# LikeLy-Journey/SegmenTron

Measured on AMD Instinct MI355X. Metric: images/sec fwd+bwd DeepLabv3+_xception65 @1025x2049, higher is better.
Workload: dtype bf16; 1 GPU; DeepLabv3+_xception65 train step (fwd + CE loss + bwd + SGD) @1025x2049, batch 2/GPU (BASELINE.json configs[2]); global_batch=2, bn=BN, parallelism=dp1, full_size=True

## Files before the change

### include/segmentron_hip.h

```cpp
#ifndef SEGMENTRON_HIP_H
#define SEGMENTRON_HIP_H
#ifdef __cplusplus
extern "C" {
#endif

const char* seg_last_error(void);
int seg_version(void);

int seg_conv_gemm_fwd(int dtype, const void* x, long ldx, int N, int Hi, int Wi, int C,
                      const void* w, int O, int KH, int KW, int stride, int pad, int dil,
                      int pro_mode, const float* pro_scale, const float* pro_shift,
                      const float* bias, void* y, long ldy, int Ho, int Wo, int out_H, int out_W,
                      int out_s, float* stat_partial, const void* ep_x, long ldep,
                      const float* ep_c0, const float* ep_c1, int tconv, void* stream);
int seg_conv_gemm_tiles_m(int N, int Ho, int Wo);

int seg_conv_gemm_wgrad(int dtype, const void* x, long ldx, int N, int Hi, int Wi, int C,
                        const void* dy, long lddy, int Ho, int Wo, int O, int KH, int KW,
                        int stride, int pad, int dil, int pro_mode, const float* pro_scale,
                        const float* pro_shift, float* partial, int splits, void* stream);
int seg_conv_gemm_stat_rows(int dtype, int N, int Ho, int Wo, int C, int O, int KH, int KW,
                            int stride, int pad, int dil, int tconv, int has_bias, int pro_mode);
int seg_conv_gemm_wgrad_splits(int dtype, int N, int Ho, int Wo, int C, int O, int KH, int KW,
                               int stride, int pad, int dil, int pro_mode);

int seg_dwconv3x3(int dtype, int mode, const void* x, long ldx, int N, int Hi, int Wi, int C,
                  const float* w9c, int w_layout, int stride, int dil, int pro_mode,
                  const float* pro_scale, const float* pro_shift, void* y, long ldy, int Ho, int Wo,
                  float* stat_partial, int grid_y, void* stream);
int seg_dwconv_grid_y(int dtype, int C, int N, int Ho, int Wo, int stride, int dil, int kind);
int seg_dwconv3x3_wgrad_finalize(const float* partial, int R, int C, float* dw_c9, void* stream);
int seg_dwconv3x3_wgrad(int dtype, const void* x, long ldx, int N, int Hi, int Wi, int C,
                        const void* dy, long lddy, int Ho, int Wo, int stride, int dil,
                        int pro_mode, const float* pro_scale, const float* pro_shift,
                        float* partial, int grid_y, void* stream);

int seg_dwconv3x3_bwd_fused(int dtype, const void* dy, long lddy, const void* x, long ldx, int N,
                            int H, int W, int C, const float* w9c, int w_layout, int dil,
                            int pro_mode, const float* pro_scale, const float* pro_shift, void* g,
                            long ldg, float* partial_w, float* partial_bn, int grid_y,
                            void* stream);
int seg_dwconv3x3_bwd_fused_add_ok(int dil);
int seg_dwconv3x3_bwd_fused_add(int dtype, const void* dy, long lddy, const void* x, long ldx, int N,
                                int H, int W, int C, const float* w9c, int w_layout, int pro_mode,
                                const float* pro_scale, const float* pro_shift, const void* res,
                                long ldr, void* g, long ldg, float* partial_w, float* partial_bn,
                                int grid_y, void* stream);

int seg_colsum(const float* in, long R, int L, double* out_d, float* out_f, double* ws,
               void* stream);
int seg_colsum_count(const float* in, long R, int L, double* out_d, double count, double* ws,
                     void* stream);
int seg_bn_finalize(const double* sums, double count, const double* count_dev,
                    const float* gamma, const float* beta, float eps, float momentum, float* running_mean, float* running_var,
                    float* mean, float* invstd, float* scale, float* shift, int C,
                    const float* mean_offset, void* stream);
int seg_bn_finalize_p(const float* partial, long R, double count, const float* gamma,
                      const float* beta, float eps, float momentum, float* running_mean,
                      float* running_var, float* mean, float* invstd, float* scale, float* shift,
                      int C, const float* mean_offset, double* ws, void* stream);
int seg_bn_finalize_small(int dtype, const void* y, long ldy, long M, int C, const float* gamma,
                          const float* beta, float eps, float momentum, float* running_mean,
                          float* running_var, float* mean, float* invstd, float* scale,
                          float* shift, const float* mean_offset, void* stream);
int seg_bn_moments_small(int dtype, const void* y, long ldy, long M, int C, double* moments,
                         void* stream);
int seg_bn_finalize_small_sync(void* p2p, int dtype, const void* y, long ldy, long M, int C,
                               const float* gamma, const float* beta, float eps, float momentum,
                               float* running_mean, float* running_var, float* mean, float* invstd,
                               float* scale, float* shift, const float* mean_offset,
                               double* count_out, void* stream);
int seg_sum_n(int dtype, int n, const void* const* xs, const long* lds, void* y, long ldy, long M,
              int C, void* stream);
int seg_bn_eval_affine(const float* gamma, const float* beta, const float* rm, const float* rv,
                       float eps, float* scale, float* shift, int C, void* stream);
int seg_bn_eval_affine_multi(int n, const float* const* gamma, const float* const* beta,
                             const float* const* rm, const float* const* rv, const float* eps,
                             float* const* out, const int* C, void* stream);
int seg_bn_apply(int dtype, const void* x, long ldx, int mode_x, const float* sx, const float* tx,
                 const void* r, long ldr, int mode_r, const float* sr, const float* tr,
                 const float* chan_mul, long rows_per_n, const void* elem_mul, long ldm,
                 int post_relu, void* y, long ldy, long M, int C, void* stream);
int seg_bn_bwd_grid_y(int dtype, int C, long M);
int seg_bn_bwd_reduce(int dtype, const void* g, long ldg, const void* x, long ldx, int mode,
                      const float* scale, const float* shift, const float* chan_mul,
                      long rows_per_n, const void* elem_mul, long ldm, long M, int C,
                      float* partial, int grid_y, void* stream);
int seg_bn_bwd_small(int dtype, const void* g, long ldg, const void* x, long ldx, void* dx,
                     long lddx, long M, int C, int mode, const float* scale, const float* shift,
                     const float* mean, const float* invstd, const float* gamma,
                     const float* chan_mul, long rows_per_n, const void* elem_mul, long ldm,
                     double count, int training, float* dgamma, float* dbeta, void* stream);
int seg_bn_bwd_finalize(const double* sums, double count, const double* count_dev,
                        const float* mean, const float* invstd, const float* gamma, float* dgamma, float* dbeta, float* c0, float* c1,
                        int C, void* stream);
int seg_bn_bwd_finalize_s(const double* sums, double count, const double* count_dev,
                          const float* mean, const float* invstd, const float* gamma, float* dgamma,
                          float* dbeta, float* c0, float* c1, int C, double grad_scale, void* stream);
int seg_bn_bwd_finalize_p(const float* partial, long R, double count, const float* mean,
                          const float* invstd, const float* gamma, float* dgamma, float* dbeta,
                          float* c0, float* c1, int C, double* ws, void* stream);
int seg_dw_bwd_finalize(const float* partial_bn, int Rb, double count, const float* mean,
                        const float* invstd, const float* gamma, float* dgamma, float* dbeta,
                        float* c0, float* c1, const float* partial_w, int Rw, float* dw_c9, int C,
                        void* stream);
int seg_bn_bwd_apply(int dtype, const void* g, long ldg, const void* x, long ldx, int mode,
                     const float* scale, const float* shift, const float* c0, const float* c1,
                     const float* chan_mul, long rows_per_n, const void* elem_mul, long ldm,
                     void* dx, long lddx, long M, int C, void* stream);

int seg_gn_chunks(long HW);
int seg_gn_moments(int dtype, const void* u, long ldu, const void* v, long ldv, int N, long HW,
                   int C, float* partial, void* stream);
int seg_gn_fwd_finalize(const float* partial, int N, long HW, int C, int G, const float* gamma,
                        const float* beta, double eps, float* mean_rstd, float* coef,
                        void* stream);
int seg_gn_bwd_finalize(const float* partial, int N, long HW, int C, int G,
                        const float* mean_rstd, const float* gamma, float* coef, float* contrib,
                        void* stream);
int seg_gn_affine(int dtype, const void* u, long ldu, const void* v, long ldv, const float* coef,
                  void* out, long ldo, int N, long HW, int C, void* stream);

int seg_fold_weights(int dtype, const float* W, const float* scale, const float* shift, void* Wp,
                     void* WpT, float* bprime, int O, int C, void* stream);
int seg_fold_bwd_rows(int O);
int seg_fold_bwd_reduce(const float* W, const float* dWp, int splits, const float* scale,
                        const float* shift, const float* db, float* dW, float* dsdt, int O, int C,
                        void* stream);
int seg_fold_bwd_finalize(const float* dsdt, int rows, double count, const double* count_dev,
                          const float* mean, const float* invstd, const float* gamma, const float* scale, float* dgamma, float* dbeta,
                          float* c0, float* c1, int C, void* stream);
int seg_fold_bwd_finalize_s(const float* dsdt, int rows, double count, const double* count_dev,
                            const float* mean, const float* invstd, const float* gamma,
                            const float* scale, float* dgamma, float* dbeta, float* c0, float* c1,
                            int C, double grad_scale, void* stream);

int seg_maxpool_fwd(int dtype, const void* x, long ldx, int N, int Hi, int Wi, int C, int k,
                    int stride, int pad, int pro_mode, const float* pro_scale,
                    const float* pro_shift, void* y, long ldy, int Ho, int Wo, void* idx,
                    void* stream);
int seg_maxpool_bwd(int dtype, void* gx, long ldgx, int N, int Hi, int Wi, int C, int k, int stride,
                    int pad, const void* gy, long ldgy, int Ho, int Wo, const void* idx,
                    void* stream);
int seg_adaptive_avgpool_chunks(int H, int W, int o);
int seg_adaptive_avgpool_partial(int dtype, const void* x, long ldx, int N, int H, int W, int C,
                                 int o, float* partial, int chunks, void* stream);
int seg_adaptive_avgpool_bwd(int dtype, void* gx, long ldgx, int N, int H, int W, int C, int o,
                             const void* gy, long ldgy, void* stream);

int seg_bilinear_fwd(int dtype, const void* x, long ldx, int N, int Hi, int Wi, int C,
                     int pro_mode, const float* pro_scale, const float* pro_shift,
                     const float* chan_mul, void* y, long ldy, int Ho, int Wo, int align_corners,
                     void* stream);
int seg_bilinear_bwd(int dtype, void* gx, long ldgx, int N, int Hi, int Wi, int C, const void* gy,
                     long ldgy, int Ho, int Wo, int align_corners, void* stream);
int seg_nearest_add(int dtype, const void* x, long ldx, int mode_x, const float* sx,
                    const float* tx, const void* r, long ldr, int mode_r, const float* sr,
                    const float* tr, int shift, int post_relu, void* y, long ldy, int N, int H,
                    int W, int C, void* stream);
int seg_nearest_sum_bwd(int dtype, const void* g, long ldg, int N, int H, int W, int C, int shift,
                        void* gr, long ldgr, void* stream);
int seg_upsample_to_nchw(int dtype, const void* x, long ldx, int N, int Hi, int Wi, int C,
                         float* out, int Ho, int Wo, int align_corners, void* stream);
int seg_upsample_to_nchw_bwd(int dtype, void* gx, long ldgx, int N, int Hi, int Wi, int C,
                             const float* gy, int Ho, int Wo, int align_corners, void* stream);
int seg_nchw_to_nhwc_pad(int dtype, const float* x, int N, int Cin, int H, int W, void* y,
                         void* stream);

int seg_upsample_ce_blocks(int N, int H, int W);
int seg_upsample_ce_fwd(int dtype, const void* lo, long ld, int N, int Hi, int Wi, int C,
                        const long* target, int H, int W, long ignore_index, int align_corners,
                        double* ws, float* loss_out, void* stream);
int seg_upsample_ce_bwd(int dtype, const void* lo, long ld, int N, int Hi, int Wi, int C,
                        const long* target, int H, int W, long ignore_index, int align_corners,
                        const float* loss_out, const float* grad_out, void* dlo, long lddlo,
                        void* stream);

int seg_dwconv3x3_s2_grid_y(int C, int N, int H, int W);
int seg_dwconv3x3_s2_bwd_fused(int dtype, const void* dy, long lddy, const void* x, long ldx, int N,
                               int H, int W, int C, const float* w_c9, int pro_mode,
                               const float* pro_scale, const float* pro_shift, void* g, long ldg,
                               float* partial_w, float* partial_bn, int grid_y, void* stream);

int seg_sgd_multi_tensor(int ntensors, const void* const* params, const void* const* grads,
                         const void* const* bufs, const long* numel, const int* group,
                         const float* lr_dev, const float* wd_dev, float momentum, int first,
                         void* stream);
int seg_pack_multi(int dtype, int njobs, const void* const* srcs, const void* const* dsts,
                   const int* O, const int* C, const int* transpose, void* stream);

int seg_metric_update_nchw(const float* logits, int N, int C, int H, int W, const long* target,
                           int nclass, long* counters, void* stream);
int seg_metric_update_upsample(int dtype, const void* lo, long ld, int N, int Hi, int Wi, int C,
                               const long* target, int H, int W, int align_corners, int nclass,
                               long* counters, void* stream);

int seg_cca_attention(int dtype, const void* q, long ldq, const void* k, long ldk, int N, int H,
                      int W, int C, float* att, void* stream);
int seg_cca_attention_bwd(int dtype, const void* dout, long lddo, const void* v, long ldv, int N,
                          int H, int W, int C, const float* att, const float* scale, float* de,
                          void* stream);
int seg_cca_map(int dtype, const float* wt, const void* b, long ldb, int N, int H, int W, int C,
                int transposed, const float* gamma, const void* res, long ldres, void* out,
                long ldo, void* raw, long ldraw, void* stream);

int seg_row_softmax(const void* e, int dt_in, long lde, void* a, int dt_out, long lda, long R,
                    int L, int Lp, float sign, void* stream);
int seg_row_softmax_bwd(const void* a, int dt_a, long lda, const void* g, int dt_g, long ldg,
                        void* de, int dt_out, long ldde, long R, int L, int Lp, float sign,
                        void* stream);
int seg_p2p_create(int rank, int world, long slot_bytes, void** handle_out);
int seg_p2p_ipc_handle(void* handle, void* out64);
int seg_p2p_connect(void* handle, const void* handles);
int seg_p2p_all_reduce_f64(void* handle, void* buf, int n, void* stream);
int seg_p2p_all_reduce_f32(void* handle, void* buf, int n, void* stream);
int seg_p2p_status(void* handle);
int seg_p2p_set_timeout(void* handle, double seconds);
int seg_p2p_destroy(void* handle);
int seg_bn_finalize_p_sync(void* p2p, const float* partial, long R, double local_count,
                           const float* gamma, const float* beta, float eps, float momentum,
                           float* running_mean, float* running_var, float* mean, float* invstd,
                           float* scale, float* shift, int C, const float* mean_offset,
                           double* count_out, double* ws, void* stream);
int seg_bn_bwd_finalize_p_sync(void* p2p, const float* partial, long R, const double* count_dev,
                               const float* mean, const float* invstd, const float* gamma,
                               float* dgamma, float* dbeta, float* c0, float* c1, int C,
                               double grad_scale, double* ws, void* stream);
int seg_dw_bwd_finalize_sync(void* p2p, const float* partial_bn, int Rb, const double* count_dev,
                             const float* mean, const float* invstd, const float* gamma,
                             float* dgamma, float* dbeta, float* c0, float* c1,
                             const float* partial_w, int Rw, float* dw_c9, int C,
                             double grad_scale, void* stream);
int seg_fold_bwd_finalize_sync(void* p2p, const float* dsdt, int rows, const double* count_dev,
                               const float* mean, const float* invstd, const float* gamma,
                               const float* scale, float* dgamma, float* dbeta, float* c0,
                               float* c1, int C, double grad_scale, void* stream);

#ifdef __cplusplus
}
#endif
#endif
```

### segmentron_amd/csrc/conv_gemm_args.h

```cpp
#pragma once
#include <hip/hip_runtime.h>

namespace seg {

struct ConvGemmArgs {
  const void* x;
  const void* w;
  void* y;
  const float* pro_scale;
  const float* pro_shift;
  const float* bias;
  float* stat_partial;
  const void* ep_x;
  const float* ep_c0;
  const float* ep_c1;
  long ldx, ldy, ldep;
  int N, Hi, Wi, C, Ho, Wo, O;
  int KH, KW, stride, pad, dil;
  int pro_mode;
  int tconv;
  int M, K;
  int out_H, out_W, out_s;
  int tiles_m, tiles_n;
};

int px256_tiles_m(long M);
int launch_conv_gemm_px256(int dtype, ConvGemmArgs a, hipStream_t stream);
bool conv_gemm_glds_usable(int dtype, const ConvGemmArgs& a);
int launch_conv_gemm_glds(ConvGemmArgs a, hipStream_t stream);
bool conv_gemm_glds_kxk_usable(int dtype, const ConvGemmArgs& a);
int launch_conv_gemm_glds_kxk(ConvGemmArgs a, hipStream_t stream);

int launch_conv_gemm_glds4(const ConvGemmArgs& a, int rows, hipStream_t stream);

int glds_rows_per_tile(long M, int O, bool kxk);
int glds_tiles_m(long M, int O, bool kxk);

bool conv3x3_direct_usable(int dtype, const ConvGemmArgs& a);
int conv3x3_direct_blocks(int N, int H, int W, int C = 32);
int launch_conv3x3_direct(const ConvGemmArgs& a, hipStream_t stream);

}
```

### segmentron_amd/csrc/conv_gemm_glds.hip

```cpp
#include "conv_gemm.h"
#include "conv_gemm_args.h"
#include "gemm_glds.h"

namespace seg {


template <bool EP, bool STATS, bool KXK = false, int IMS = 4>
__global__ __launch_bounds__(GL_THREADS, 2) void conv_gemm_glds_kernel(const ConvGemmArgs a) {
  typedef bf16_t T;
  constexpr int VEC = 8;
  extern __shared__ __attribute__((aligned(16))) unsigned char smem_raw[];
  lds_byte_t* lds = (lds_byte_t*)smem_raw;

  const int tid = threadIdx.x, lane = tid & 63;
  const int wave = __builtin_amdgcn_readfirstlane(tid >> 6);
  const int wm = wave >> 2, wn = wave & 3;
  const int L = xcd_remap(blockIdx.x, a.tiles_m * a.tiles_n);
  const int tile_m = L / a.tiles_n, tile_n = L - tile_m * a.tiles_n;
  const int m0 = tile_m * (64 * IMS), n0 = tile_n * GL_BN;

  GemmOperand A, B;
  A.base = reinterpret_cast<const unsigned char*>(a.x);
  A.ld_bytes = a.ldx * 2;
  A.rows = a.M;
  B.base = reinterpret_cast<const unsigned char*>(a.w);
  B.ld_bytes = (long)a.K * 2;
  B.rows = a.O;

  f32x16 acc[2][IMS];

  if (KXK) {
    const GlConvA cg = {a.M, a.Hi, a.Wi, a.Ho, a.Wo, a.KW, a.pad, a.dil, a.C / 32};
    gl_mainloop_ring<true, IMS>(A, B, a.K, m0, n0, lds, acc, &cg);
  } else {
    gl_mainloop_ring<false, IMS>(A, B, a.K, m0, n0, lds, acc);
  }

  typedef typename std::conditional<EP, float, T>::type PT;
  constexpr int EP_STRIDE = 64 * (int)sizeof(PT) + 16;
  constexpr int VPR = 64 / VEC;
  unsigned char* ep = smem_raw + wave * 32 * EP_STRIDE;
  T* __restrict__ Y = reinterpret_cast<T*>(a.y);
  const int r32 = lane & 31, hh = lane >> 5;
  const int v = lane & (VPR - 1);
  const int o = n0 + wn * 64 + v * VEC;
  float ssum[VEC], ssq[VEC];
#pragma unroll
  for (int k = 0; k < VEC; ++k) ssum[k] = ssq[k] = 0.f;
  float c0v[VEC], c1v[VEC];
  const bool epc = EP && o < a.O;
  if (epc) {
    load_params<VEC>(a.ep_c0, o, c0v);
    load_params<VEC>(a.ep_c1, o, c1v);
  }
  constexpr int NQ_ALL = (32 * VPR) / 64;
  uint4 xr_all[EP ? IMS : 1][EP ? NQ_ALL : 1];
  if (EP) {
#pragma unroll
    for (int im = 0; im < IMS; ++im)
#pragma unroll
      for (int q = 0; q < NQ_ALL; ++q) {
        const int r = (q * 64 + lane) / VPR;
        const int p = m0 + wm * 32 * IMS + im * 32 + r;
        const long pc = p < a.M ? p : a.M - 1;
        xr_all[im][q] = ldg16(reinterpret_cast<const T*>(a.ep_x) + pc * a.ldep + (epc ? o : 0));
      }
  }
#pragma unroll
  for (int im = 0; im < IMS; ++im) {
#pragma unroll
    for (int jn = 0; jn < 2; ++jn) {
#pragma unroll
      for (int g = 0; g < 4; ++g) {
        const int ch = jn * 32 + 8 * g + 4 * hh;
        float f[4];
#pragma unroll
        for (int k = 0; k < 4; ++k) f[k] = acc[jn][im][4 * g + k];
        HVec<PT>::store(reinterpret_cast<PT*>(ep + r32 * EP_STRIDE) + ch, f);
      }
    }
    __builtin_amdgcn_fence(__ATOMIC_RELEASE, "wavefront");
    __builtin_amdgcn_wave_barrier();
    constexpr int NQ = (32 * VPR) / 64;
    uint4 val[NQ], xr[NQ], vhi[NQ];
#pragma unroll
    for (int q = 0; q < NQ; ++q) {
      const int r = (q * 64 + lane) / VPR;
      if (EP) {
        val[q] = *reinterpret_cast<const uint4*>(ep + r * EP_STRIDE + v * 32);
        vhi[q] = *reinterpret_cast<const uint4*>(ep + r * EP_STRIDE + v * 32 + 16);
      } else {
        val[q] = *reinterpret_cast<const uint4*>(ep + r * EP_STRIDE + v * 16);
      }
      if (EP) xr[q] = xr_all[im][q];
    }
#pragma unroll
    for (int q = 0; q < NQ; ++q) {
      const int r = (q * 64 + lane) / VPR;
      const int p = m0 + wm * 32 * IMS + im * 32 + r;
      if (EP) {
        float f[VEC], xv[VEC];
        Vec<float>::unpack(val[q], f);
        Vec<float>::unpack(vhi[q], f + 4);
        Vec<T>::unpack(xr[q], xv);
        if (epc) {
#pragma unroll
          for (int k = 0; k < VEC; ++k) f[k] = f[k] - c0v[k] - c1v[k] * xv[k];
        }
        val[q] = Vec<T>::pack(f);
      }
      if (STATS && (!EP || p < a.M)) {
        float f[VEC];
        Vec<T>::unpack(val[q], f);
#pragma unroll
        for (int k = 0; k < VEC; ++k) {
          ssum[k] += f[k];
          ssq[k] = fmaf(f[k], f[k], ssq[k]);
        }
      }
      if (p < a.M && o < a.O) stg16(Y + (long)p * a.ldy + o, val[q]);
    }
    __builtin_amdgcn_fence(__ATOMIC_RELEASE, "wavefront");
    __builtin_amdgcn_wave_barrier();
  }
  if (STATS) {
#pragma unroll
    for (int k = 0; k < VEC; ++k) {
#pragma unroll
      for (int m = VPR; m < 64; m <<= 1) {
        ssum[k] += __shfl_xor(ssum[k], m, 64);
        ssq[k] += __shfl_xor(ssq[k], m, 64);
      }
    }
    __syncthreads();
    float* red = reinterpret_cast<float*>(smem_raw);
    if (lane < VPR) {
#pragma unroll
      for (int k = 0; k < VEC; ++k) {
        red[(wm * 2 + 0) * 256 + wn * 64 + v * VEC + k] = ssum[k];
        red[(wm * 2 + 1) * 256 + wn * 64 + v * VEC + k] = ssq[k];
      }
    }
    __syncthreads();
    if (tid < 256) {
      const int oc = n0 + tid;
      if (oc < a.O) {
        float* dst = a.stat_partial + (long)tile_m * 2 * a.O;
        dst[oc] = red[0 * 256 + tid] + red[2 * 256 + tid];
        dst[a.O + oc] = red[1 * 256 + tid] + red[3 * 256 + tid];
      }
    }
  }
}

bool conv_gemm_glds_usable(int dtype, const ConvGemmArgs& a) {
  return dtype == DT_BF16 && a.pro_mode == PRO_NONE && a.bias == nullptr && a.KH == 1 && a.KW == 1 && a.stride == 1 &&
         a.pad == 0 && a.tconv == 0 && a.out_s == 1 && (a.K % 8) == 0 && (a.ldx % 8) == 0 && (a.O % 8) == 0 &&
         (a.ldy % 8) == 0;
}

constexpr int GLDS_FIXED_ROWS = 96;

constexpr long GLDS_W4_MAX_TILES = 512;

static int glds_pick_rows(long M, int O, bool with224) {
  const long tn = (O + GL_BN - 1) / GL_BN;
  int best = 256;
  long best_cost = -1;
  for (int bm = 256; bm >= 192; bm -= 32) {
    const long tiles = ((M + bm - 1) / bm) * tn;
    if (bm == 224 && (!with224 || tiles > GLDS_W4_MAX_TILES)) continue;
    const long cost = ((tiles + 255) / 256) * (bm + GLDS_FIXED_ROWS);
    if (best_cost < 0 || cost < best_cost) {
      best_cost = cost;
      best = bm;
    }
  }
  return best;
}

int glds_rows_per_tile(long M, int O, bool kxk) { return glds_pick_rows(M, O, !kxk); }

int glds_tiles_m(long M, int O, bool kxk) {
  const int bm = glds_rows_per_tile(M, O, kxk);
  return (int)((M + bm - 1) / bm);
}

template <bool EP, bool STATS, bool KXK, int IMS>
static int launch_glds_inst(const ConvGemmArgs& a, hipStream_t stream) {
  static const int once = [] {
    return (int)hipFuncSetAttribute(
        reinterpret_cast<const void*>(&conv_gemm_glds_kernel<EP, STATS, KXK, IMS>),
        hipFuncAttributeMaxDynamicSharedMemorySize, GL_LDS_BYTES);
  }();
  if (once != 0) {
    set_error("conv_gemm_glds: cannot reserve %d bytes of LDS", GL_LDS_BYTES);
    return 2;
  }
  const dim3 grid(a.tiles_m * a.tiles_n), block(GL_THREADS);
  hipLaunchKernelGGL((conv_gemm_glds_kernel<EP, STATS, KXK, IMS>), grid, block, GL_LDS_BYTES,
                     stream, a);
  return check_launch(KXK ? "conv_gemm_fwd (glds KxK)" : "conv_gemm_fwd (glds)");
}

template <bool EP, bool STATS, bool KXK>
static int launch_glds_rows(ConvGemmArgs a, hipStream_t stream) {
  const int bm = glds_pick_rows(a.M, a.O, !KXK && !(EP && !STATS));
  a.tiles_m = (a.M + bm - 1) / bm;
  a.tiles_n = (a.O + GL_BN - 1) / GL_BN;
  if constexpr (!KXK) {
    if (bm == 224) return launch_conv_gemm_glds4(a, bm, stream);
  }
  if (bm == 256) return launch_glds_inst<EP, STATS, KXK, 4>(a, stream);
  if (bm == 192) return launch_glds_inst<EP, STATS, KXK, 3>(a, stream);
  set_error("conv_gemm_glds: no %d-row tile on the eight-wave kernel", bm);
  return 2;
}

int launch_conv_gemm_glds(ConvGemmArgs a, hipStream_t stream) {
  if (a.ep_x != nullptr && a.stat_partial != nullptr)
    return launch_glds_rows<true, true, false>(a, stream);
  if (a.ep_x != nullptr) return launch_glds_rows<true, false, false>(a, stream);
  if (a.stat_partial != nullptr) return launch_glds_rows<false, true, false>(a, stream);
  return launch_glds_rows<false, false, false>(a, stream);
}

bool conv_gemm_glds_kxk_usable(int dtype, const ConvGemmArgs& a) {
  return dtype == DT_BF16 && a.pro_mode == PRO_NONE && a.bias == nullptr && a.ep_x == nullptr &&
         a.KH * a.KW > 1 && a.stride == 1 && a.tconv == 0 && a.out_s == 1 && (a.C % 32) == 0 &&
         (a.ldx % 8) == 0 && (a.O % 8) == 0 && (a.ldy % 8) == 0 &&
         (long)a.N * a.Hi * a.Wi < (1L << 31);
}

int launch_conv_gemm_glds_kxk(ConvGemmArgs a, hipStream_t stream) {
  if (a.stat_partial != nullptr) return launch_glds_rows<false, true, true>(a, stream);
  return launch_glds_rows<false, false, true>(a, stream);
}

}
```

### segmentron_amd/csrc/conv_gemm_wgrad_args.h

```cpp
#pragma once
#include <hip/hip_runtime.h>

namespace seg {

struct WgradArgs {
  const void* x;
  const void* dy;
  float* partial;
  const float* pro_scale;
  const float* pro_shift;
  long ldx, lddy;
  int N, Hi, Wi, C, Ho, Wo, O;
  int KH, KW, stride, pad, dil;
  int pro_mode;
  int M, K;
  int tiles_o, tiles_k, splits;
  int chunk;
};

bool conv_wgrad_glds_usable(int dtype, const WgradArgs& a);
int conv_wgrad_glds_splits(long M, int O, int K);
int launch_conv_wgrad_glds(WgradArgs a, hipStream_t stream);

bool conv3x3_wgrad_direct_usable(int dtype, int C, int O, int KH, int KW, int stride, int pad,
                                 int dil, long M, long ldx, long lddy);
int conv3x3_direct_blocks(int N, int H, int W, int C = 32);
int launch_conv3x3_wgrad_direct(const void* x, long ldx, const void* dy, long lddy, int N, int H,
                                int W, int O, int pro_mode, const float* pro_scale,
                                const float* pro_shift, float* partial, hipStream_t stream);

}
```

### segmentron_amd/csrc/conv_gemm_wgrad_glds.hip

```cpp
#include "conv_gemm.h"
#include "conv_gemm_wgrad_args.h"
#include "gemm_glds.h"

namespace seg {

constexpr int WG_BM = 128, WG_BN = 128, WG_BK = 64;
constexpr int WG_THREADS = 512;
constexpr int WG_SUB = 16 * 1024, WG_SLOT = 32 * 1024, WG_LDS = 4 * WG_SLOT;

typedef unsigned long long u64_t;

__device__ __forceinline__ u64_t tr_read(unsigned addr) {
  u64_t r;
  asm volatile("ds_read_b64_tr_b16 %0, %1" : "=v"(r) : "v"(addr) : "memory");
  return r;
}
template <int OFF>
__device__ __forceinline__ u64_t tr_read_off(unsigned addr) {
  u64_t r;
  asm volatile("ds_read_b64_tr_b16 %0, %1 offset:%2" : "=v"(r) : "v"(addr), "n"(OFF) : "memory");
  return r;
}

struct WgFrags { u64_t a[2], b[2][2]; };

__device__ __forceinline__ bf16x8 wg_join(u64_t lo, u64_t hi) {
  typedef u64_t u64x2 __attribute__((ext_vector_type(2)));
  u64x2 v = {lo, hi};
  return __builtin_bit_cast(bf16x8, v);
}

template <bool KXK>
__global__ __launch_bounds__(WG_THREADS, 2) void conv_wgrad_glds_kernel(const WgradArgs a) {
  extern __shared__ __attribute__((aligned(16))) unsigned char smem_raw[];
  lds_byte_t* lds = (lds_byte_t*)smem_raw;
  const int tid = threadIdx.x, lane = tid & 63;
  const int wave = __builtin_amdgcn_readfirstlane(tid >> 6);
  const int wo = wave >> 1, wc = wave & 1;
  const int tiles = a.tiles_o * a.tiles_k;
  const int L = xcd_remap(blockIdx.x, tiles * a.splits);
  const int tile = L % tiles, split = L / tiles;
  const int o0 = (tile / a.tiles_k) * WG_BM, c0 = (tile % a.tiles_k) * WG_BN;
  const int p0 = split * a.chunk;
  const int p1 = min(a.M, p0 + a.chunk);
  const int nslot = (p1 - p0 + WG_BK - 1) / WG_BK;

  const unsigned char* zero = reinterpret_cast<const unsigned char*>(g_gl_zero);
  const int rr = lane >> 4;
  const int c16 = ((lane & 15) - 4 * rr) & 15;
  const bool ch_dy = o0 + c16 * 8 < a.O, ch_x = c0 + c16 * 8 < (KXK ? a.K : a.C);
  const unsigned char* src[4];
  int prow[2];
  int kdh = 0, kdw = 0, kc0 = c0, pn[2] = {0, 0}, ph[2] = {0, 0}, pw[2] = {0, 0};
  if (KXK) {
    const int tap = c0 / a.C;
    kc0 = c0 - tap * a.C;
    const int kh = tap / a.KW;
    kdh = kh * a.dil - a.pad;
    kdw = (tap - kh * a.KW) * a.dil - a.pad;
  }
#pragma unroll
  for (int j = 0; j < 2; ++j) {
    prow[j] = p0 + (wave * 2 + j) * 4 + rr;
    src[j] = reinterpret_cast<const unsigned char*>(a.dy) +
             ((long)prow[j] * a.lddy + o0 + c16 * 8) * 2;
    src[2 + j] = reinterpret_cast<const unsigned char*>(a.x) +
                 ((long)prow[j] * a.ldx + c0 + c16 * 8) * 2;
    if (KXK) {
      pw[j] = prow[j] % a.Wo;
      const int t = prow[j] / a.Wo;
      ph[j] = t % a.Ho;
      pn[j] = t / a.Ho;
    }
  }
  const long inc_dy = (long)WG_BK * a.lddy * 2, inc_x = (long)WG_BK * a.ldx * 2;
  auto issue = [&](int slot) {
    lds_byte_t* base = lds + (slot & 3) * WG_SLOT + (wave * 2) * 1024;
#pragma unroll
    for (int j = 0; j < 2; ++j) {
      const bool rok = prow[j] + slot * WG_BK < p1;
      const unsigned char* pd = (rok && ch_dy) ? src[j] : zero;
      const unsigned char* px = (rok && ch_x) ? src[2 + j] : zero;
      if (KXK) {
        const int hi = ph[j] + kdh, wi = pw[j] + kdw;
        const bool ok = rok && ch_x && hi >= 0 && hi < a.Hi && wi >= 0 && wi < a.Wi;
        px = ok ? reinterpret_cast<const unsigned char*>(a.x) +
                      ((((long)pn[j] * a.Hi + hi) * a.Wi + wi) * a.ldx + kc0 + c16 * 8) * 2
                : zero;
        pw[j] += WG_BK;
        if (pw[j] >= a.Wo) {
          pw[j] -= a.Wo;
          if (++ph[j] == a.Ho) { ph[j] = 0; ++pn[j]; }
        }
      }
      src[j] += inc_dy;
      src[2 + j] += inc_x;
      __builtin_amdgcn_global_load_lds((glb_byte_t*)pd, base + j * 1024, 16, 0, 0);
      __builtin_amdgcn_global_load_lds((glb_byte_t*)px, base + j * 1024 + WG_SUB, 16, 0, 0);
    }
  };
  issue(0); issue(1); issue(2); issue(3);

  const int g = lane >> 4, i = lane & 15;
  auto lane_base = [&](int cb) {
    const int q = cb * 4 + (g & 1) * 2 + ((i & 3) >> 1);
    const int cpos = (q + 4 * (i >> 2)) & 15;
    return (g >> 1) * 2048 + (i >> 2) * 256 + cpos * 16 + (i & 1) * 8;
  };
  const unsigned lds0 = (unsigned)(unsigned long)lds;
  const unsigned addr_a = lds0 + lane_base(wo);
  const unsigned addr_b0 = lds0 + WG_SUB + lane_base(wc * 2);
  const unsigned addr_b1 = lds0 + WG_SUB + lane_base(wc * 2 + 1);
  auto read = [&](WgFrags& f, int slot, auto step) {
    constexpr int S = decltype(step)::value;
    const unsigned off = (slot & 3) * WG_SLOT;
    f.a[0] = tr_read_off<S * 4096>(addr_a + off);
    f.a[1] = tr_read_off<S * 4096 + 1024>(addr_a + off);
    f.b[0][0] = tr_read_off<S * 4096>(addr_b0 + off);
    f.b[0][1] = tr_read_off<S * 4096 + 1024>(addr_b0 + off);
    f.b[1][0] = tr_read_off<S * 4096>(addr_b1 + off);
    f.b[1][1] = tr_read_off<S * 4096 + 1024>(addr_b1 + off);
  };
  typedef std::integral_constant<int, 0> S0;
  typedef std::integral_constant<int, 1> S1;
  typedef std::integral_constant<int, 2> S2;
  typedef std::integral_constant<int, 3> S3;
  f32x16 acc[2];
#pragma unroll
  for (int e = 0; e < 16; ++e) acc[0][e] = acc[1][e] = 0.f;
  auto mma = [&](const WgFrags& f) {
    const bf16x8 fa = wg_join(f.a[0], f.a[1]);
    acc[0] = __builtin_amdgcn_mfma_f32_32x32x16_bf16(fa, wg_join(f.b[0][0], f.b[0][1]), acc[0], 0,
                                                     0, 0);
    acc[1] = __builtin_amdgcn_mfma_f32_32x32x16_bf16(fa, wg_join(f.b[1][0], f.b[1][1]), acc[1], 0,
                                                     0, 0);
  };
#define WG_WAIT_FRAGS(f, cnt)                                                                  \
  asm volatile("s_waitcnt " cnt                                                               \
               : "+v"(f.a[0]), "+v"(f.a[1]), "+v"(f.b[0][0]), "+v"(f.b[0][1]), "+v"(f.b[1][0]), \
                 "+v"(f.b[1][1])                                                               \
               :                                                                               \
               : "memory")
  WgFrags f0, f1;
  GL_WAIT_VM(12);
  __builtin_amdgcn_s_barrier();
  read(f0, 0, S0{});
  for (int j = 0; j < nslot; ++j) {
    read(f1, j, S1{});
    WG_WAIT_FRAGS(f0, "lgkmcnt(6)");
    mma(f0);
    read(f0, j, S2{});
    WG_WAIT_FRAGS(f1, "lgkmcnt(6)");
    mma(f1);
    read(f1, j, S3{});
    WG_WAIT_FRAGS(f0, "lgkmcnt(6)");
    mma(f0);
    WG_WAIT_FRAGS(f1, "vmcnt(8) lgkmcnt(0)");
    __builtin_amdgcn_s_barrier();
    issue(j + 4);
    read(f0, j + 1, S0{});
    mma(f1);
  }
  asm volatile("s_waitcnt vmcnt(0) lgkmcnt(0)" ::: "memory");
#undef WG_WAIT_FRAGS

  float* __restrict__ P = a.partial + (long)split * a.O * a.K;
  const int r32 = lane & 31, hh = lane >> 5;
#pragma unroll
  for (int jb = 0; jb < 2; ++jb) {
    const int c = c0 + (wc * 2 + jb) * 32 + r32;
#pragma unroll
    for (int e = 0; e < 16; ++e) {
      const int o = o0 + wo * 32 + (e & 3) + 8 * (e >> 2) + 4 * hh;
      if (o < a.O && c < a.K) P[(long)o * a.K + c] = acc[jb][e];
    }
  }
}

bool conv_wgrad_glds_usable(int dtype, const WgradArgs& a) {
  const bool common = dtype == DT_BF16 && a.pro_mode == PRO_NONE && a.stride == 1 &&
                      (a.O % 8) == 0 && (a.ldx % 8) == 0 && (a.lddy % 8) == 0 && a.M >= 2048;
  if (!common) return false;
  if (a.KH == 1 && a.KW == 1)
    return a.pad == 0 && (a.C % 8) == 0 && ((long)a.O * a.C >= 128 * 128 || a.M >= 32768);
  return (a.C % 128) == 0 && a.Wo >= WG_BK && a.O >= 128 &&
         (long)a.N * a.Hi * a.Wi < (1L << 31);
}

int conv_wgrad_glds_splits(long M, int O, int K) {
  const int tiles = ((O + WG_BM - 1) / WG_BM) * ((K + WG_BN - 1) / WG_BN);
  long want = (256 + tiles / 2) / tiles;
  if (want * tiles > 282) want = 256 / tiles;
  const long maxs = (M + 8 * WG_BK - 1) / (8 * WG_BK);
  if (want > maxs) want = maxs;
  if (want < 1) want = 1;
  return (int)want;
}

int launch_conv_wgrad_glds(WgradArgs a, hipStream_t stream) {
  a.tiles_o = (a.O + WG_BM - 1) / WG_BM;
  a.tiles_k = (a.K + WG_BN - 1) / WG_BN;
  const int slots = (a.M + WG_BK - 1) / WG_BK;
  a.chunk = ((slots + a.splits - 1) / a.splits) * WG_BK;
  static const int once = [] {
    int rc = (int)hipFuncSetAttribute(reinterpret_cast<const void*>(&conv_wgrad_glds_kernel<false>),
                                      hipFuncAttributeMaxDynamicSharedMemorySize, WG_LDS);
    rc |= (int)hipFuncSetAttribute(reinterpret_cast<const void*>(&conv_wgrad_glds_kernel<true>),
                                   hipFuncAttributeMaxDynamicSharedMemorySize, WG_LDS);
    return rc;
  }();
  if (once != 0) {
    set_error("conv_wgrad_glds: cannot reserve %d bytes of LDS", WG_LDS);
    return 2;
  }
  const dim3 grid(a.tiles_o * a.tiles_k * a.splits), block(WG_THREADS);
  if (a.KH * a.KW > 1)
    hipLaunchKernelGGL(conv_wgrad_glds_kernel<true>, grid, block, WG_LDS, stream, a);
  else
    hipLaunchKernelGGL(conv_wgrad_glds_kernel<false>, grid, block, WG_LDS, stream, a);
  return check_launch("conv_gemm_wgrad (glds)");
}

}
```

### segmentron_amd/csrc/dwconv.hip

```cpp
#include "common.h"
#include "dwconv_tiled.h"
#include "dwconv_slide.h"
#include <cstdlib>
#include <type_traits>

namespace seg {

constexpr bool g_dw_row = true;

constexpr int DW_TW = 4;
constexpr int DW_THREADS = 256;
enum { MODE_FWD = 0, MODE_DGRAD = 1 };

struct DwArgs {
  const void* x;
  const float* w;
  void* y;
  const float* pro_scale;
  const float* pro_shift;
  float* stat_partial;
  long ldx, ldy;
  int N, Hi, Wi, C;
  int Ho, Wo;
  int stride, pad, dil;
// ... 395 lines not shown
    const int b = 1 << l;
    const double u = (double)CV / (double)(((CV + b - 1) / b) * b);
    if (u > bu + 1e-9) { bu = u; best = l; }
  }
  return best;
}

}

extern "C" int seg_dwconv_grid_y(int dtype, int C, int N, int Ho, int Wo, int stride, int dil,
                                 int kind) {
  using namespace seg;
  const int tiled_stride = kind == 0 ? stride : 1;
  if ((kind == 0 || kind == 1) && dw_slide_supported(stride, dil, C))
    return dw_slide_rows(C, N, Ho, Wo);
  if ((kind == 0 || stride == 1) && dw_tiled_supported(tiled_stride, dil))
    return dw_tiled_grid_y(dtype, C, N, Ho, Wo, kind);
  if (kind == 0 && stride == 2 && dil == 1)
    return dw_tiled_s2_grid_y(dtype, C, N, Ho, Wo);
  if (g_dw_row && (kind == 0 || kind == 1) && dw_row_supported(stride, dil) && C % 4 == 0)
    return dw_row_grid_y(dtype, C, N, Ho, Wo, dil);
  const int vec = dtype == DT_BF16 ? 8 : 4;
  const int CV = C / vec;
  const int l = pick_cvb_log2(CV);
  const int spb = DW_THREADS >> l;
  const long strips = (long)N * Ho * ((Wo + DW_TW - 1) / DW_TW);
  const int gx = (CV + (1 << l) - 1) >> l;
  long gy = (strips + spb - 1) / spb;
  long cap = 1536 / gx;
  if (cap < 1) cap = 1;
  if (gy > cap) gy = cap;
  return (int)gy;
}
extern "C" int seg_dwconv3x3(int dtype, int mode, const void* x, long ldx, int N, int Hi, int Wi,
                             int C, const float* w9c, int w_layout, int stride, int dil, int pro_mode,
                             const float* pro_scale, const float* pro_shift, void* y, long ldy,
                             int Ho, int Wo, float* stat_partial, int grid_y, void* stream) {
  using namespace seg;
  const int vec = dtype == DT_BF16 ? 8 : 4;
  SEG_REQUIRE(dtype == DT_F32 || dtype == DT_BF16, "dwconv3x3: bad dtype %d", dtype);
  SEG_REQUIRE(C % vec == 0 && ldx % vec == 0 && ldy % vec == 0,
              "dwconv3x3: C/ldx/ldy must be multiples of %d", vec);
  SEG_REQUIRE(((pro_mode & PRO_AFFINE) == 0) || (pro_scale && pro_shift),
              "dwconv3x3: affine prologue without scale/shift");
  SEG_REQUIRE(mode == MODE_FWD || stat_partial == nullptr, "dwconv3x3: stats only in forward");
  SEG_REQUIRE(grid_y >= 1, "dwconv3x3: grid_y must be >= 1");
  if (mode == MODE_FWD && dw_slide_supported(stride, dil, C)) {
    SEG_REQUIRE(Ho == Hi && Wo == Wi, "dwconv3x3: stride 1 keeps the size");
    return launch_dw_slide_fwd(dtype, x, ldx, N, Hi, Wi, C, w9c, w_layout, pro_mode, pro_scale,
                               pro_shift, y, ldy, stat_partial, grid_y, (hipStream_t)stream);
  }
  if (mode == MODE_FWD && dw_tiled_supported(stride, dil)) {
    SEG_REQUIRE(Ho == Hi && Wo == Wi, "dwconv3x3: stride 1 keeps the size");
    return launch_dw_tiled(dtype, x, ldx, N, Hi, Wi, C, w9c, w_layout, dil, pro_mode, pro_scale,
                           pro_shift, y, ldy, stat_partial, grid_y, (hipStream_t)stream);
  }
  if (mode == MODE_FWD && stride == 2 && dil == 1) {
    SEG_REQUIRE(Ho == (Hi + 1) / 2 && Wo == (Wi + 1) / 2, "dwconv3x3: stride-2 output size");
    SEG_REQUIRE((long)N * Hi * Wi < (1L << 31), "dwconv3x3: tensor exceeds 32-bit pixel offsets");
    return launch_dw_tiled_s2(dtype, x, ldx, N, Hi, Wi, C, w9c, w_layout, pro_mode, pro_scale,
                              pro_shift, y, ldy, stat_partial, grid_y, (hipStream_t)stream);
  }
  SEG_REQUIRE(w_layout == 0, "dwconv3x3: the strip kernels take tap-major [9][C] weights");
  if (g_dw_row && mode == MODE_FWD && dw_row_supported(stride, dil) && C % 4 == 0) {
    SEG_REQUIRE(Ho == Hi && Wo == Wi, "dwconv3x3: stride 1 keeps the size");
    return launch_dw_row_fwd(dtype, x, ldx, N, Hi, Wi, C, w9c, dil, pro_mode, pro_scale, pro_shift,
                             y, ldy, stat_partial, grid_y, (hipStream_t)stream);
  }
  DwArgs a;
  a.x = x; a.w = w9c; a.y = y; a.pro_scale = pro_scale; a.pro_shift = pro_shift;
  a.stat_partial = stat_partial; a.ldx = ldx; a.ldy = ldy;
  a.N = N; a.Hi = Hi; a.Wi = Wi; a.C = C; a.Ho = Ho; a.Wo = Wo;
  a.stride = stride; a.pad = dil; a.dil = dil; a.pro_mode = pro_mode;
  const int kvec = vec;
  a.CV = C / kvec; a.cvb_log2 = pick_cvb_log2(a.CV);
  a.strips = (long)N * Ho * ((Wo + DW_TW - 1) / DW_TW);
  const int gx = (a.CV + (1 << a.cvb_log2) - 1) >> a.cvb_log2;
  SEG_REQUIRE(grid_y >= 1, "dwconv3x3: grid_y must be >= 1");
  const dim3 grid(gx, grid_y);
  const size_t lds = stat_partial ? (size_t)DW_THREADS * 2 * kvec * sizeof(float) : 0;
  hipStream_t st = (hipStream_t)stream;
  SEG_REQUIRE(a.strips < (1L << 31), "dwconv3x3: too many strips");
  SEG_REQUIRE((long)N * Hi * Wi * ldx < (1L << 31), "dwconv3x3: tensor exceeds 32-bit offsets");
#define SEG_DW_LAUNCH(TT, MM) \
  hipLaunchKernelGGL((dwconv_kernel<TT, MM>), grid, dim3(DW_THREADS), lds, st, a)
  if (dtype == DT_BF16) {
    if (mode == MODE_FWD) SEG_DW_LAUNCH(bf16_t, MODE_FWD); else SEG_DW_LAUNCH(bf16_t, MODE_DGRAD);
  } else {
    if (mode == MODE_FWD) SEG_DW_LAUNCH(float, MODE_FWD); else SEG_DW_LAUNCH(float, MODE_DGRAD);
  }
#undef SEG_DW_LAUNCH
  return check_launch("dwconv3x3");
}

extern "C" int seg_dwconv3x3_wgrad(int dtype, const void* x, long ldx, int N, int Hi, int Wi,
                                   int C, const void* dy, long lddy, int Ho, int Wo, int stride,
                                   int dil, int pro_mode, const float* pro_scale,
                                   const float* pro_shift, float* partial, int grid_y,
                                   void* stream) {
  using namespace seg;
  const int vec = dtype == DT_BF16 ? 8 : 4;
  SEG_REQUIRE(dtype == DT_F32 || dtype == DT_BF16, "dwconv3x3_wgrad: bad dtype %d", dtype);
  SEG_REQUIRE(C % vec == 0 && ldx % vec == 0 && lddy % vec == 0,
              "dwconv3x3_wgrad: C/ldx/lddy must be multiples of %d", vec);
  SEG_REQUIRE(grid_y >= 1, "dwconv3x3_wgrad: grid_y must be >= 1");
  if (dw_tiled_supported(stride, dil)) {
    SEG_REQUIRE(Ho == Hi && Wo == Wi, "dwconv3x3_wgrad: stride 1 keeps the size");
    return launch_dw_wgrad_tiled(dtype, x, ldx, N, Hi, Wi, C, dy, lddy, dil, pro_mode, pro_scale,
                                 pro_shift, partial, grid_y, (hipStream_t)stream);
  }
  DwWgradArgs a;
  a.x = x; a.dy = dy; a.partial = partial; a.pro_scale = pro_scale; a.pro_shift = pro_shift;
  a.ldx = ldx; a.lddy = lddy; a.N = N; a.Hi = Hi; a.Wi = Wi; a.C = C; a.Ho = Ho; a.Wo = Wo;
  a.stride = stride; a.pad = dil; a.dil = dil; a.pro_mode = pro_mode;
  a.CV = C / vec; a.cvb_log2 = pick_cvb_log2(a.CV);
  a.strips = (long)N * Ho * ((Wo + DW_TW - 1) / DW_TW);
  const int gx = (a.CV + (1 << a.cvb_log2) - 1) >> a.cvb_log2;
  SEG_REQUIRE(grid_y >= 1, "dwconv3x3_wgrad: grid_y must be >= 1");
  const dim3 grid(gx, grid_y);
  const size_t lds = (size_t)DW_THREADS * 3 * vec * sizeof(float);
  hipStream_t st = (hipStream_t)stream;
  SEG_REQUIRE(a.strips < (1L << 31), "dwconv3x3_wgrad: too many strips");
  if (dtype == DT_BF16)
    hipLaunchKernelGGL((dwconv_wgrad_kernel<bf16_t>), grid, dim3(DW_THREADS), lds, st, a);
  else
    hipLaunchKernelGGL((dwconv_wgrad_kernel<float>), grid, dim3(DW_THREADS), lds, st, a);
  return check_launch("dwconv3x3_wgrad");
}

extern "C" int seg_dwconv3x3_bwd_fused_add_ok(int dil) { return dil == 1 ? 1 : 0; }

extern "C" int seg_dwconv3x3_bwd_fused_add(int dtype, const void* dy, long lddy, const void* x,
                                           long ldx, int N, int H, int W, int C, const float* w9c,
                                           int w_layout, int pro_mode, const float* pro_scale,
                                           const float* pro_shift, const void* res, long ldr,
                                           void* g, long ldg, float* partial_w, float* partial_bn,
                                           int grid_y, void* stream) {
  using namespace seg;
  SEG_REQUIRE(dtype == DT_F32 || dtype == DT_BF16, "dwconv3x3_bwd_fused_add: bad dtype %d", dtype);
  const int tvec = dtype == DT_BF16 ? 8 : 4;
  SEG_REQUIRE(C % tvec == 0 && ldx % tvec == 0 && lddy % tvec == 0 && ldg % tvec == 0 &&
                  ldr % 4 == 0 && res != nullptr,
              "dwconv3x3_bwd_fused_add: C/ld must be multiples of %d, res non-null", tvec);
  SEG_REQUIRE(((pro_mode & PRO_AFFINE) == 0) || (pro_scale && pro_shift),
              "dwconv3x3_bwd_fused_add: affine prologue without scale/shift");
  SEG_REQUIRE(grid_y >= 1 && partial_w != nullptr, "dwconv3x3_bwd_fused_add: bad grid/partials");
  if (dw_slide_supported(1, 1, C))
    return launch_dw_slide_bwd(dtype, dy, lddy, x, ldx, N, H, W, C, w9c, w_layout, pro_mode,
                               pro_scale, pro_shift, g, ldg, partial_w, partial_bn, grid_y,
                               (hipStream_t)stream, res, ldr);
  return launch_dw_bwd_tiled(dtype, dy, lddy, x, ldx, N, H, W, C, w9c, w_layout, 1, pro_mode,
                             pro_scale, pro_shift, g, ldg, partial_w, partial_bn, grid_y,
                             (hipStream_t)stream, res, ldr);
}

extern "C" int seg_dwconv3x3_bwd_fused(int dtype, const void* dy, long lddy, const void* x,
                                       long ldx, int N, int H, int W, int C, const float* w9c,
                                       int w_layout, int dil, int pro_mode, const float* pro_scale,
                                       const float* pro_shift, void* g, long ldg,
                                       float* partial_w, float* partial_bn, int grid_y,
                                       void* stream) {
  using namespace seg;
  const int vec = 4;
  SEG_REQUIRE(dtype == DT_F32 || dtype == DT_BF16, "dwconv3x3_bwd_fused: bad dtype %d", dtype);
  SEG_REQUIRE(C % vec == 0 && ldx % vec == 0 && lddy % vec == 0 && ldg % vec == 0,
              "dwconv3x3_bwd_fused: C/ld must be multiples of %d", vec);
  SEG_REQUIRE(((pro_mode & PRO_AFFINE) == 0) || (pro_scale && pro_shift),
              "dwconv3x3_bwd_fused: affine prologue without scale/shift");
  SEG_REQUIRE(grid_y >= 1 && partial_w != nullptr, "dwconv3x3_bwd_fused: bad grid/partials");
  if (dw_slide_supported(1, dil, C))
    return launch_dw_slide_bwd(dtype, dy, lddy, x, ldx, N, H, W, C, w9c, w_layout, pro_mode,
                               pro_scale, pro_shift, g, ldg, partial_w, partial_bn, grid_y,
                               (hipStream_t)stream);
  if (dw_tiled_supported(1, dil)) {
    const int tvec = dtype == DT_BF16 ? 8 : 4;
    SEG_REQUIRE(C % tvec == 0 && ldx % tvec == 0 && lddy % tvec == 0 && ldg % tvec == 0,
                "dwconv3x3_bwd_fused: C/ld must be multiples of %d", tvec);
    return launch_dw_bwd_tiled(dtype, dy, lddy, x, ldx, N, H, W, C, w9c, w_layout, dil, pro_mode,
                               pro_scale, pro_shift, g, ldg, partial_w, partial_bn, grid_y,
                               (hipStream_t)stream);
  }
  SEG_REQUIRE(w_layout == 0, "dwconv3x3_bwd_fused: the strip kernel takes tap-major weights");
  if (g_dw_row && dw_row_supported(1, dil))
    return launch_dw_row_bwd(dtype, dy, lddy, x, ldx, N, H, W, C, w9c, dil, pro_mode, pro_scale,
                             pro_shift, g, ldg, partial_w, partial_bn, grid_y, (hipStream_t)stream);
  DwBwdArgs a;
  a.dy = dy; a.x = x; a.g = g; a.w = w9c; a.pro_scale = pro_scale; a.pro_shift = pro_shift;
  a.partial_w = partial_w; a.partial_bn = partial_bn;
  a.lddy = lddy; a.ldx = ldx; a.ldg = ldg; a.N = N; a.H = H; a.W = W; a.C = C; a.dil = dil;
  a.pro_mode = pro_mode; a.CV = C / vec; a.cvb_log2 = pick_cvb_log2(a.CV);
  a.strips = (long)N * H * ((W + DW_TW - 1) / DW_TW);
  SEG_REQUIRE(a.strips < (1L << 31), "dwconv3x3_bwd_fused: too many strips");
  SEG_REQUIRE((long)N * H * W * lddy < (1L << 31), "dwconv3x3_bwd_fused: 32-bit offsets");
  const int gx = (a.CV + (1 << a.cvb_log2) - 1) >> a.cvb_log2;
  const dim3 grid(gx, grid_y);
  const size_t lds = (size_t)DW_THREADS * 3 * vec * sizeof(float);
  hipStream_t st = (hipStream_t)stream;
  if (dtype == DT_BF16)
    hipLaunchKernelGGL((dwconv_bwd_fused_kernel<bf16_t>), grid, dim3(DW_THREADS), lds, st, a);
  else
    hipLaunchKernelGGL((dwconv_bwd_fused_kernel<float>), grid, dim3(DW_THREADS), lds, st, a);
  return check_launch("dwconv3x3_bwd_fused");
}

extern "C" int seg_dwconv3x3_wgrad_finalize(const float* partial, int R, int C, float* dw_c9,
                                            void* stream) {
  using namespace seg;
  SEG_REQUIRE(R >= 1 && C >= 1, "dwconv3x3_wgrad_finalize: bad R/C");
  return launch_dw_wgrad_finalize(partial, R, C, dw_c9, (hipStream_t)stream);
}
```

### segmentron_amd/csrc/dwconv_slide.h

```cpp
#pragma once
#include <hip/hip_runtime.h>

namespace seg {
bool dw_slide_supported(int stride, int dil, int C);
int dw_slide_rows(int C, int N, int H, int W);
int launch_dw_slide_fwd(int dtype, const void* x, long ldx, int N, int H, int W, int C,
                        const float* w, int w_layout, int pro_mode, const float* sc,
                        const float* sh, void* y, long ldy, float* stat_partial, int rows,
                        hipStream_t st);
int launch_dw_slide_bwd(int dtype, const void* dy, long lddy, const void* x, long ldx, int N, int H,
                        int W, int C, const float* w, int w_layout, int pro_mode, const float* sc,
                        const float* sh, void* g, long ldg, float* partial_w, float* partial_bn,
                        int rows, hipStream_t st, const void* res = nullptr, long ldr = 0);
}
```

### segmentron_amd/csrc/dwconv_slide.hip

```cpp
#include <type_traits>
#include "common.h"
#include "dwconv_slide.h"

namespace seg {

constexpr int SL_THREADS = 256, SL_CQ = 16, SL_WL = 16;
constexpr int SL_DEPTH_F = 2, SL_OCC_F = 4, SL_DEPTH_B = 2;
#define SL_SCHED_BARRIER() __builtin_amdgcn_sched_barrier(0)

struct DwSlideArgs {
  const void* x;
  const void* dy;
  const void* res;
  void* y;
  const float* w;
  int w_layout;
  const float* sc; const float* sh;
  float* partial;
  float* partial_bn;
  long ldx, lddy, ldy, ldr;
  int N, H, W, C, pro_mode, rs, nstrips, nwblk, ncblk;
};

struct SlBlock { int n, strip, wblk, cblk, prow; };
__device__ __forceinline__ SlBlock sl_block(const DwSlideArgs& a) {
  const int nblk = a.ncblk * a.nwblk * a.nstrips * a.N;
  int L = xcd_remap(blockIdx.x, nblk);
  SlBlock b;
  b.cblk = L % a.ncblk;
  L /= a.ncblk;
  b.prow = L;
  b.wblk = L % a.nwblk;
  L /= a.nwblk;
  b.strip = L % a.nstrips;
  b.n = L / a.nstrips;
  return b;
}

typedef float f32x2 __attribute__((ext_vector_type(2)));
typedef short s16x2 __attribute__((ext_vector_type(2)));
struct Q4 { f32x2 lo, hi; };
__device__ __forceinline__ Q4 q4_zero() { Q4 q; q.lo = q.hi = (f32x2){0.f, 0.f}; return q; }
__device__ __forceinline__ void q4_fma(Q4& acc, const Q4& a, const Q4& b) {
  acc.lo = __builtin_elementwise_fma(a.lo, b.lo, acc.lo);
  acc.hi = __builtin_elementwise_fma(a.hi, b.hi, acc.hi);
}
template <typename T> struct SlIO;
template <> struct SlIO<bf16_t> {
  typedef uint2 raw_t;
  static constexpr int BYTES = 8;
  __device__ static __forceinline__ Q4 unpack(const raw_t& r) {
    Q4 q;
    q.lo = (f32x2){__uint_as_float(r.x << 16), __uint_as_float(r.x & 0xFFFF0000u)};
    q.hi = (f32x2){__uint_as_float(r.y << 16), __uint_as_float(r.y & 0xFFFF0000u)};
    return q;
  }
  __device__ static __forceinline__ raw_t relu_raw(const raw_t& r) {
    const s16x2 z = {0, 0};
    raw_t o;
    o.x = __builtin_bit_cast(unsigned, __builtin_elementwise_max(__builtin_bit_cast(s16x2, r.x), z));
    o.y = __builtin_bit_cast(unsigned, __builtin_elementwise_max(__builtin_bit_cast(s16x2, r.y), z));
    return o;
  }
  static constexpr bool RAW_RELU = true;
  __device__ static __forceinline__ raw_t pack(const Q4& q) {
    return make_uint2(pack_bf16x2(q.lo.x, q.lo.y), pack_bf16x2(q.hi.x, q.hi.y));
  }
};
template <> struct SlIO<float> {
  typedef uint4 raw_t;
  static constexpr int BYTES = 16;
  __device__ static __forceinline__ Q4 unpack(const raw_t& r) {
    Q4 q;
    q.lo = (f32x2){__uint_as_float(r.x), __uint_as_float(r.y)};
    q.hi = (f32x2){__uint_as_float(r.z), __uint_as_float(r.w)};
    return q;
  }
  __device__ static __forceinline__ raw_t relu_raw(const raw_t& r) { return r; }
  static constexpr bool RAW_RELU = false;
  __device__ static __forceinline__ raw_t pack(const Q4& q) {
    return make_uint4(__float_as_uint(q.lo.x), __float_as_uint(q.lo.y), __float_as_uint(q.hi.x),
                      __float_as_uint(q.hi.y));
  }
};
template <typename R>
__device__ __forceinline__ R sl_ld(const unsigned char* __restrict__ base, unsigned off) {
  return *reinterpret_cast<const R*>(base + off);
}
template <typename R>
__device__ __forceinline__ void sl_st(unsigned char* __restrict__ base, unsigned off, const R& v) {
  *reinterpret_cast<R*>(base + off) = v;
}

__device__ __forceinline__ void sl_load_taps(const DwSlideArgs& a, int c, Q4 (&wt)[9]) {
  float f[36];
  if (a.w_layout & 1) {
    const float4* p = reinterpret_cast<const float4*>(a.w + (long)c * 9);
#pragma unroll
    for (int j = 0; j < 9; ++j) {
      const float4 v = p[j];
      f[4 * j] = v.x; f[4 * j + 1] = v.y; f[4 * j + 2] = v.z; f[4 * j + 3] = v.w;
    }
#pragma unroll
    for (int k = 0; k < 9; ++k) {
      const int tap = (a.w_layout & 2) ? 8 - k : k;
      wt[k].lo = (f32x2){(a.w_layout & 2) ? f[8 - k] : f[k], (a.w_layout & 2) ? f[9 + 8 - k] : f[9 + k]};
      wt[k].hi = (f32x2){(a.w_layout & 2) ? f[18 + 8 - k] : f[18 + k],
                         (a.w_layout & 2) ? f[27 + 8 - k] : f[27 + k]};
      (void)tap;
    }
  } else {
#pragma unroll
    for (int k = 0; k < 9; ++k) {
      const int tap = (a.w_layout & 2) ? 8 - k : k;
      const float4 v = *reinterpret_cast<const float4*>(a.w + (long)tap * a.C + c);
      wt[k].lo = (f32x2){v.x, v.y};
      wt[k].hi = (f32x2){v.z, v.w};
    }
  }
}

template <int MODE, bool RELU_DONE>
__device__ __forceinline__ void sl_act(Q4& q, const Q4& sc, const Q4& sh) {
  const f32x2 z = {0.f, 0.f}, six = {6.f, 6.f};
  if (MODE & PRO_AFFINE) {
    q.lo = __builtin_elementwise_fma(q.lo, sc.lo, sh.lo);
    q.hi = __builtin_elementwise_fma(q.hi, sc.hi, sh.hi);
  }
  if ((MODE & PRO_RELU) && !RELU_DONE) {
    q.lo = __builtin_elementwise_max(q.lo, z);
    q.hi = __builtin_elementwise_max(q.hi, z);
  }
  if (MODE & PRO_CLAMP6) {
    q.lo = __builtin_elementwise_min(q.lo, six);
    q.hi = __builtin_elementwise_min(q.hi, six);
  }
}

struct SlThread {
  int c, w, r0, r1, rlast;
  bool live, lm, rm;
  unsigned off_m, off_0, off_p;
  bool edge, first, last;
  unsigned off_e;
  int bp_up, bp_dn;
};
template <int ESIZE>
__device__ __forceinline__ SlThread sl_thread(const DwSlideArgs& a, const SlBlock& b, long ld) {
  const int tid = threadIdx.x, cq = tid & (SL_CQ - 1), wl = tid >> 4;
  SlThread t;
  const int cfull = (b.cblk * SL_CQ + cq) * 4, wfull = b.wblk * SL_WL + wl;
  t.c = min(cfull, a.C - 4);
  t.w = min(wfull, a.W - 1);
  t.live = wfull < a.W && cfull < a.C;
  t.lm = t.w >= 1;
  t.rm = t.w + 1 < a.W;
  t.r0 = b.strip * a.rs;
  t.r1 = min(a.H, t.r0 + a.rs);
  t.rlast = min(t.r1, a.H - 1);
  t.off_m = (unsigned)((max(t.w - 1, 0) * ld + t.c) * ESIZE);
  t.off_0 = (unsigned)((t.w * ld + t.c) * ESIZE);
  t.off_p = (unsigned)((min(t.w + 1, a.W - 1) * ld + t.c) * ESIZE);
  const int lane = tid & 63, col = lane >> 4;
  t.first = col == 0;
  t.last = col == 3;
  t.edge = t.first || t.last;
  t.off_e = t.first ? t.off_m : (t.last ? t.off_p : 0xFFFFFFFFu);
  t.bp_up = ((lane - 16) & 63) * 4;
  t.bp_dn = ((lane + 16) & 63) * 4;
  return t;
}

typedef unsigned int sl_u32x2 __attribute__((ext_vector_type(2)));
// ... 22 lines not shown
}
template <typename R> __device__ __forceinline__ R sl_bperm(int addr, const R& v);
template <> __device__ __forceinline__ uint2 sl_bperm<uint2>(int addr, const uint2& v) {
  return make_uint2((unsigned)__builtin_amdgcn_ds_bpermute(addr, (int)v.x),
                    (unsigned)__builtin_amdgcn_ds_bpermute(addr, (int)v.y));
}
template <> __device__ __forceinline__ uint4 sl_bperm<uint4>(int addr, const uint4& v) {
  return make_uint4((unsigned)__builtin_amdgcn_ds_bpermute(addr, (int)v.x),
                    (unsigned)__builtin_amdgcn_ds_bpermute(addr, (int)v.y),
                    (unsigned)__builtin_amdgcn_ds_bpermute(addr, (int)v.z),
                    (unsigned)__builtin_amdgcn_ds_bpermute(addr, (int)v.w));
}
__device__ __forceinline__ uint2 sl_sel(bool c, const uint2& a, const uint2& b) {
  return make_uint2(c ? a.x : b.x, c ? a.y : b.y);
}
__device__ __forceinline__ uint4 sl_sel(bool c, const uint4& a, const uint4& b) {
  return make_uint4(c ? a.x : b.x, c ? a.y : b.y, c ? a.z : b.z, c ? a.w : b.w);
}
template <typename R>
__device__ __forceinline__ void sl_neighbours(const SlThread& t, const R (&raw)[3], R& left, R& right) {
  const R up = sl_bperm<R>(t.bp_up, raw[0]), dn = sl_bperm<R>(t.bp_dn, raw[0]);
  left = sl_sel(t.first, raw[1], up);
  right = sl_sel(t.last, raw[1], dn);
}

template <typename T, int MODE, bool XCHG>
__global__ __launch_bounds__(SL_THREADS, SL_OCC_F) void dwconv_slide_fwd_kernel(const DwSlideArgs a) {
  using IO = SlIO<T>;
  using raw_t = typename IO::raw_t;
  constexpr int ES = sizeof(T);
  constexpr bool RAWRELU = IO::RAW_RELU && MODE == PRO_RELU;
  const int tid = threadIdx.x, cq = tid & (SL_CQ - 1);
  const SlBlock b = sl_block(a);
  const SlThread t = sl_thread<ES>(a, b, a.ldx);
  const int r0 = t.r0, r1 = t.r1;

  Q4 wt[9], sc, sh;
  sc = sh = q4_zero();
  const unsigned char* __restrict__ Xb = reinterpret_cast<const unsigned char*>(a.x) +
                                         (long)b.n * a.H * a.W * a.ldx * ES;
  unsigned char* __restrict__ Yb = reinterpret_cast<unsigned char*>(a.y) +
                                   (long)b.n * a.H * a.W * a.ldy * ES;
  const long xpitch = (long)a.W * a.ldx * ES, ypitch = (long)a.W * a.ldy * ES;
  const unsigned rowbytes = (unsigned)xpitch;
  const unsigned yoff = t.live ? (unsigned)((t.w * a.ldy + t.c) * ES) : 0xFFFFFFFFu;

  auto issue = [&](int r, raw_t (&raw)[3]) {
    const unsigned char* __restrict__ row = Xb + (long)min(max(r, 0), t.rlast) * xpitch;
    if (XCHG) {
      raw[0] = sl_ld<raw_t>(row, t.off_0);
      raw[1] = sl_ld_edge<raw_t>(row, rowbytes, t.off_e);
    } else {
      raw[0] = sl_ld<raw_t>(row, t.off_0);
      raw[1] = sl_ld<raw_t>(row, t.off_m);
      raw[2] = sl_ld<raw_t>(row, t.off_p);
    }
  };
  auto commit = [&](int r, const raw_t (&raw)[3], Q4 (&row)[3], auto check) {
    constexpr bool CHECK = decltype(check)::value;
    const bool rv = !CHECK || (r >= 0 && r < a.H);
    raw_t r3[3];
    r3[1] = raw[0];
    if (XCHG) {
      sl_neighbours<raw_t>(t, raw, r3[0], r3[2]);
    } else {
      r3[0] = raw[1];
      r3[2] = raw[2];
    }
#pragma unroll
    for (int k = 0; k < 3; ++k) {
      row[k] = IO::unpack(RAWRELU ? IO::relu_raw(r3[k]) : r3[k]);
      sl_act<MODE, RAWRELU>(row[k], sc, sh);
      if (CHECK && !rv) row[k] = q4_zero();
    }
  };
  Q4 ssum = q4_zero(), ssq = q4_zero();
  auto compute = [&](int ro, const Q4 (&ra)[3], const Q4 (&rb)[3], const Q4 (&rc)[3]) {
    Q4 acc = q4_zero();
#pragma unroll
    for (int kw = 0; kw < 3; ++kw) q4_fma(acc, ra[kw], wt[kw]);
#pragma unroll
    for (int kw = 0; kw < 3; ++kw) q4_fma(acc, rb[kw], wt[3 + kw]);
#pragma unroll
    for (int kw = 0; kw < 3; ++kw) q4_fma(acc, rc[kw], wt[6 + kw]);
    sl_st_row<raw_t>(Yb + (long)ro * ypitch, (unsigned)ypitch, yoff, IO::pack(acc));
    ssum.lo += acc.lo; ssum.hi += acc.hi;
    q4_fma(ssq, acc, acc);
  };

  constexpr int D = SL_DEPTH_F, U = (D % 3 == 0) ? D : 3 * D;
  Q4 win[3][3];
  raw_t ring[D][3];
#pragma unroll
  for (int j = 0; j < D; ++j) issue(r0 - 1 + j, ring[j]);
  sl_load_taps(a, t.c, wt);
  if (MODE & PRO_AFFINE) {
    const float4 s4 = *reinterpret_cast<const float4*>(a.sc + t.c);
    const float4 t4 = *reinterpret_cast<const float4*>(a.sh + t.c);
    sc.lo = (f32x2){s4.x, s4.y}; sc.hi = (f32x2){s4.z, s4.w};
    sh.lo = (f32x2){t4.x, t4.y}; sh.hi = (f32x2){t4.z, t4.w};
  }
#pragma unroll
  for (int kh = 0; kh < 3; ++kh) {
    if (!t.lm) wt[kh * 3] = q4_zero();
    if (!t.rm) wt[kh * 3 + 2] = q4_zero();
  }
  commit(r0 - 1, ring[0], win[0], std::true_type{});
  issue(r0 - 1 + D, ring[0]);
  commit(r0, ring[1 % D], win[1], std::false_type{});
  issue(r0 + D, ring[1 % D]);
  int ro = r0;
  for (; ro + U < r1; ro += U) {
#pragma unroll
    for (int k = 0; k < U; ++k) {
      commit(ro + k + 1, ring[(k + 2) % D], win[(k + 2) % 3], std::false_type{});
      issue(ro + k + 1 + D, ring[(k + 2) % D]);
      SL_SCHED_BARRIER();
      compute(ro + k, win[k % 3], win[(k + 1) % 3], win[(k + 2) % 3]);
      SL_SCHED_BARRIER();
    }
  }
#pragma unroll
  for (int k = 0; k < U; ++k) {
    if (ro + k < r1) {
      commit(ro + k + 1, ring[(k + 2) % D], win[(k + 2) % 3], std::true_type{});
      issue(ro + k + 1 + D, ring[(k + 2) % D]);
      compute(ro + k, win[k % 3], win[(k + 1) % 3], win[(k + 2) % 3]);
    }
  }

  if (a.partial != nullptr) {
    __shared__ float red[4][SL_CQ][8];
    float v[8] = {ssum.lo.x, ssum.lo.y, ssum.hi.x, ssum.hi.y, ssq.lo.x, ssq.lo.y, ssq.hi.x, ssq.hi.y};
#pragma unroll
    for (int i = 0; i < 8; ++i) {
      v[i] = t.live ? v[i] : 0.f;
      v[i] += __shfl_xor(v[i], 16, 64);
      v[i] += __shfl_xor(v[i], 32, 64);
    }
    if ((tid & 63) < SL_CQ) {
#pragma unroll
      for (int i = 0; i < 8; ++i) red[tid >> 6][cq][i] = v[i];
    }
    __syncthreads();
    if (tid < SL_CQ * 8) {
      const int q = tid >> 3, k = tid & 7;
      const float tot = red[0][q][k] + red[1][q][k] + red[2][q][k] + red[3][q][k];
      const int ch = (b.cblk * SL_CQ + q) * 4 + (k & 3);
      if (ch < a.C) a.partial[((long)b.prow * 2 + (k >> 2)) * a.C + ch] = tot;
    }
  }
}

template <typename T, int MODE, bool RES, bool XCHG>
__global__ __launch_bounds__(SL_THREADS, 2) void dwconv_slide_bwd_kernel(const DwSlideArgs a) {
  using IO = SlIO<T>;
  using raw_t = typename IO::raw_t;
  constexpr int ES = sizeof(T);
  const int tid = threadIdx.x, cq = tid & (SL_CQ - 1);
  const SlBlock b = sl_block(a);
  const SlThread t = sl_thread<ES>(a, b, a.lddy);
  const int r0 = t.r0, r1 = t.r1;

  Q4 wt[9], sc, sh;
  sc = sh = q4_zero();
  const long img = (long)b.n * a.H * a.W;
  const unsigned char* __restrict__ Db = reinterpret_cast<const unsigned char*>(a.dy) + img * a.lddy * ES;
  const unsigned char* __restrict__ Xb = reinterpret_cast<const unsigned char*>(a.x) + img * a.ldx * ES;
  const unsigned char* __restrict__ Rb =
      RES ? reinterpret_cast<const unsigned char*>(a.res) + img * a.ldr * ES : nullptr;
  unsigned char* __restrict__ Gb = reinterpret_cast<unsigned char*>(a.y) + img * a.ldy * ES;
  const long dpitch = (long)a.W * a.lddy * ES, xpitch = (long)a.W * a.ldx * ES;
  const long rpitch = (long)a.W * a.ldr * ES, gpitch = (long)a.W * a.ldy * ES;
  const unsigned rowbytes = (unsigned)dpitch;
  const unsigned xoff = (unsigned)((t.w * a.ldx + t.c) * ES), roff = (unsigned)((t.w * a.ldr + t.c) * ES);
  const unsigned goff = t.live ? (unsigned)((t.w * a.ldy + t.c) * ES) : 0xFFFFFFFFu;

  auto issue = [&](int r, raw_t (&raw)[3]) {
    const unsigned char* __restrict__ row = Db + (long)min(max(r, 0), t.rlast) * dpitch;
    if (XCHG) {
      raw[0] = sl_ld<raw_t>(row, t.off_0);
      raw[1] = sl_ld_edge<raw_t>(row, rowbytes, t.off_e);
    } else {
      raw[0] = sl_ld<raw_t>(row, t.off_0);
      raw[1] = sl_ld<raw_t>(row, t.off_m);
      raw[2] = sl_ld<raw_t>(row, t.off_p);
    }
  };
  auto issue_x = [&](int r, raw_t& xr, raw_t& rr) {
    const int rcl = min(r, r1 - 1);
    xr = sl_ld<raw_t>(Xb + (long)rcl * xpitch, xoff);
    if (RES) rr = sl_ld<raw_t>(Rb + (long)rcl * rpitch, roff);
  };
  auto commit = [&](int r, const raw_t (&raw)[3], Q4 (&row)[3], auto check) {
    constexpr bool CHECK = decltype(check)::value;
    const bool rv = !CHECK || (r >= 0 && r < a.H);
    raw_t r3[3];
    r3[1] = raw[0];
    if (XCHG) {
      sl_neighbours<raw_t>(t, raw, r3[0], r3[2]);
    } else {
      r3[0] = raw[1];
      r3[2] = raw[2];
    }
#pragma unroll
    for (int k = 0; k < 3; ++k) {
      row[k] = IO::unpack(r3[k]);
      if (CHECK && !rv) row[k] = q4_zero();
    }
  };
  Q4 accw[9], s1 = q4_zero(), s2 = q4_zero();
#pragma unroll
  for (int k = 0; k < 9; ++k) accw[k] = q4_zero();

  auto compute = [&](int ro, const raw_t& xraw, const raw_t& rraw, const Q4 (&ra)[3],
                     const Q4 (&rb)[3], const Q4 (&rcw)[3]) {
    const Q4 xr = IO::unpack(xraw);
    Q4 xa = xr;
    sl_act<MODE, false>(xa, sc, sh);
    Q4 g = q4_zero();
#pragma unroll
    for (int bq = 0; bq < 3; ++bq) { q4_fma(g, ra[bq], wt[8 - bq]); q4_fma(accw[8 - bq], ra[bq], xa); }
#pragma unroll
    for (int bq = 0; bq < 3; ++bq) { q4_fma(g, rb[bq], wt[5 - bq]); q4_fma(accw[5 - bq], rb[bq], xa); }
#pragma unroll
    for (int bq = 0; bq < 3; ++bq) { q4_fma(g, rcw[bq], wt[2 - bq]); q4_fma(accw[2 - bq], rcw[bq], xa); }
    if (MODE & PRO_RELU) {
      auto on = [&](float v) { return v > 0.f && (!(MODE & PRO_CLAMP6) || v < 6.f); };
      g.lo.x = on(xa.lo.x) ? g.lo.x : 0.f; g.lo.y = on(xa.lo.y) ? g.lo.y : 0.f;
      g.hi.x = on(xa.hi.x) ? g.hi.x : 0.f; g.hi.y = on(xa.hi.y) ? g.hi.y : 0.f;
    }
    if (RES) {
      const Q4 rr = IO::unpack(rraw);
      Q4 o;
      o.lo = g.lo + rr.lo;
      o.hi = g.hi + rr.hi;
      sl_st_row<raw_t>(Gb + (long)ro * gpitch, (unsigned)gpitch, goff, IO::pack(o));
    } else {
      sl_st_row<raw_t>(Gb + (long)ro * gpitch, (unsigned)gpitch, goff, IO::pack(g));
    }
    s1.lo += g.lo; s1.hi += g.hi;
    q4_fma(s2, g, xr);
  };

  constexpr int D = SL_DEPTH_B, U = (D % 3 == 0) ? D : 3 * D;
  Q4 win[3][3];
  raw_t ring[D][3], xring[D], rring[D];
#pragma unroll
  for (int j = 0; j < D; ++j) {
    issue(r0 - 1 + j, ring[j]);
    rring[j] = xring[j] = sl_ld<raw_t>(Xb + (long)min(r0 + j, r1 - 1) * xpitch, xoff);
    if (RES) rring[j] = sl_ld<raw_t>(Rb + (long)min(r0 + j, r1 - 1) * rpitch, roff);
  }
  sl_load_taps(a, t.c, wt);
  if (MODE & PRO_AFFINE) {
    const float4 s4 = *reinterpret_cast<const float4*>(a.sc + t.c);
    const float4 t4 = *reinterpret_cast<const float4*>(a.sh + t.c);
    sc.lo = (f32x2){s4.x, s4.y}; sc.hi = (f32x2){s4.z, s4.w};
    sh.lo = (f32x2){t4.x, t4.y}; sh.hi = (f32x2){t4.z, t4.w};
  }
#pragma unroll
  for (int kh = 0; kh < 3; ++kh) {
    if (!t.lm) wt[kh * 3 + 2] = q4_zero();
    if (!t.rm) wt[kh * 3] = q4_zero();
  }
  commit(r0 - 1, ring[0], win[0], std::true_type{});
  issue(r0 - 1 + D, ring[0]);
  commit(r0, ring[1 % D], win[1], std::false_type{});
  issue(r0 + D, ring[1 % D]);
  int ro = r0;
  for (; ro + U < r1; ro += U) {
#pragma unroll
    for (int k = 0; k < U; ++k) {
      commit(ro + k + 1, ring[(k + 2) % D], win[(k + 2) % 3], std::false_type{});
      issue(ro + k + 1 + D, ring[(k + 2) % D]);
      const raw_t xraw = xring[k % D], rraw = rring[k % D];
      issue_x(ro + k + D, xring[k % D], rring[k % D]);
      SL_SCHED_BARRIER();
      compute(ro + k, xraw, rraw, win[k % 3], win[(k + 1) % 3], win[(k + 2) % 3]);
      SL_SCHED_BARRIER();
    }
  }
#pragma unroll
  for (int k = 0; k < U; ++k) {
    if (ro + k < r1) {
      commit(ro + k + 1, ring[(k + 2) % D], win[(k + 2) % 3], std::true_type{});
      issue(ro + k + 1 + D, ring[(k + 2) % D]);
      const raw_t xraw = xring[k % D], rraw = rring[k % D];
      issue_x(ro + k + D, xring[k % D], rring[k % D]);
      compute(ro + k, xraw, rraw, win[k % 3], win[(k + 1) % 3], win[(k + 2) % 3]);
    }
  }

  float v[44];
#pragma unroll
  for (int k = 0; k < 9; ++k) {
    const int kw = k % 3;
    const bool keep = t.live && (kw != 2 || t.lm) && (kw != 0 || t.rm);
    v[k * 4] = keep ? accw[k].lo.x : 0.f; v[k * 4 + 1] = keep ? accw[k].lo.y : 0.f;
    v[k * 4 + 2] = keep ? accw[k].hi.x : 0.f; v[k * 4 + 3] = keep ? accw[k].hi.y : 0.f;
  }
  v[36] = s1.lo.x; v[37] = s1.lo.y; v[38] = s1.hi.x; v[39] = s1.hi.y;
  v[40] = s2.lo.x; v[41] = s2.lo.y; v[42] = s2.hi.x; v[43] = s2.hi.y;
#pragma unroll
  for (int i = 36; i < 44; ++i) v[i] = t.live ? v[i] : 0.f;
#pragma unroll
  for (int i = 0; i < 44; ++i) {
    v[i] += __shfl_xor(v[i], 16, 64);
    v[i] += __shfl_xor(v[i], 32, 64);
  }
  __shared__ float red[4][SL_CQ][44];
  if ((tid & 63) < SL_CQ) {
#pragma unroll
    for (int i = 0; i < 44; ++i) red[tid >> 6][cq][i] = v[i];
  }
  __syncthreads();
  for (int e = tid; e < SL_CQ * 44; e += SL_THREADS) {
    const int q = e / 44, k = e - q * 44;
    const float tot = red[0][q][k] + red[1][q][k] + red[2][q][k] + red[3][q][k];
    const int ch = (b.cblk * SL_CQ + q) * 4 + (k & 3), r = k >> 2;
    if (ch < a.C) {
      if (r < 9) a.partial[((long)b.prow * 9 + r) * a.C + ch] = tot;
      else if (a.partial_bn != nullptr) a.partial_bn[((long)b.prow * 2 + (r - 9)) * a.C + ch] = tot;
    }
  }
}

bool dw_slide_supported(int stride, int dil, int C) { return stride == 1 && dil == 1 && C % 4 == 0; }

static void slide_geom(DwSlideArgs& a, int N, int H, int W, int C) {
  a.ncblk = (C / 4 + SL_CQ - 1) / SL_CQ;
  a.nwblk = (W + SL_WL - 1) / SL_WL;
  long ns = (H + 21) / 43;
  const long per_strip = (long)N * a.nwblk * a.ncblk;
  const long want = (400 + per_strip - 1) / per_strip;
  if (ns < want) ns = want;
  if (ns > H / 8) ns = H / 8;
  const long cap = 1024 / ((long)N * a.nwblk);
  if (ns > cap) ns = cap;
  if (ns < 1) ns = 1;
  a.rs = (int)((H + ns - 1) / ns);
  a.nstrips = (H + a.rs - 1) / a.rs;
}

int dw_slide_rows(int C, int N, int H, int W) {
  DwSlideArgs a;
  slide_geom(a, N, H, W, C);
  return N * a.nstrips * a.nwblk;
}

static bool slide_exchange(const DwSlideArgs& a, int esize) {
  return (long)a.N * a.H * a.W * a.C * esize >= (30L << 20);
}
template <typename T>
static void slide_launch_fwd(const DwSlideArgs& a, dim3 grid, hipStream_t st) {
  const bool xc = slide_exchange(a, (int)sizeof(T));
  switch (a.pro_mode) {
#define SL_CASE(M)                                                                                  \
  case M:                                                                                           \
    if (xc) hipLaunchKernelGGL((dwconv_slide_fwd_kernel<T, M, true>), grid, dim3(SL_THREADS), 0, st, a);  \
    else hipLaunchKernelGGL((dwconv_slide_fwd_kernel<T, M, false>), grid, dim3(SL_THREADS), 0, st, a);    \
    break;
    SL_CASE(0) SL_CASE(1) SL_CASE(2) SL_CASE(3) SL_CASE(5) SL_CASE(7)
#undef SL_CASE
    default: break;
  }
}
template <typename T, bool RES>
static void slide_launch_bwd(const DwSlideArgs& a, dim3 grid, hipStream_t st) {
  const bool xc = slide_exchange(a, (int)sizeof(T));
  switch (a.pro_mode) {
#define SL_CASE(M)                                                                                       \
  case M:                                                                                                \
    if (xc) hipLaunchKernelGGL((dwconv_slide_bwd_kernel<T, M, RES, true>), grid, dim3(SL_THREADS), 0, st, a);  \
    else hipLaunchKernelGGL((dwconv_slide_bwd_kernel<T, M, RES, false>), grid, dim3(SL_THREADS), 0, st, a);    \
    break;
    SL_CASE(0) SL_CASE(1) SL_CASE(2) SL_CASE(3) SL_CASE(5) SL_CASE(7)
#undef SL_CASE
    default: break;
  }
}
static bool slide_mode_ok(int m) { return m == 0 || m == 1 || m == 2 || m == 3 || m == 5 || m == 7; }

int launch_dw_slide_fwd(int dtype, const void* x, long ldx, int N, int H, int W, int C,
                        const float* w, int w_layout, int pro_mode, const float* sc,
                        const float* sh, void* y, long ldy, float* stat_partial, int rows,
                        hipStream_t st) {
  DwSlideArgs a;
  a.x = x; a.dy = nullptr; a.res = nullptr; a.y = y; a.w = w; a.w_layout = w_layout;
  a.sc = sc; a.sh = sh; a.partial = stat_partial; a.partial_bn = nullptr;
  a.ldx = ldx; a.lddy = 0; a.ldy = ldy; a.ldr = 0;
  a.N = N; a.H = H; a.W = W; a.C = C; a.pro_mode = pro_mode;
  slide_geom(a, N, H, W, C);
  SEG_REQUIRE(slide_mode_ok(pro_mode), "dwconv (slide): unsupported prologue mode %d", pro_mode);
  SEG_REQUIRE(C % 4 == 0 && ldx % 4 == 0 && ldy % 4 == 0,
              "dwconv (slide): C/ldx/ldy must be multiples of 4");
  SEG_REQUIRE(stat_partial == nullptr || rows == N * a.nstrips * a.nwblk,
              "dwconv (slide): %d partial rows, the launch writes %d (seg_dwconv_grid_y)", rows,
              N * a.nstrips * a.nwblk);
  const dim3 grid((unsigned)((long)a.ncblk * a.nwblk * a.nstrips * N));
  if (dtype == DT_BF16) slide_launch_fwd<bf16_t>(a, grid, st);
  else slide_launch_fwd<float>(a, grid, st);
  return check_launch("dwconv3x3 (slide)");
}

int launch_dw_slide_bwd(int dtype, const void* dy, long lddy, const void* x, long ldx, int N, int H,
                        int W, int C, const float* w, int w_layout, int pro_mode, const float* sc,
                        const float* sh, void* g, long ldg, float* partial_w, float* partial_bn,
                        int rows, hipStream_t st, const void* res, long ldr) {
  DwSlideArgs a;
  a.x = x; a.dy = dy; a.res = res; a.y = g; a.w = w; a.w_layout = w_layout & 1;
  a.sc = sc; a.sh = sh; a.partial = partial_w; a.partial_bn = partial_bn;
  a.ldx = ldx; a.lddy = lddy; a.ldy = ldg; a.ldr = ldr;
  a.N = N; a.H = H; a.W = W; a.C = C; a.pro_mode = pro_mode;
  slide_geom(a, N, H, W, C);
  SEG_REQUIRE(slide_mode_ok(pro_mode), "dwconv bwd (slide): unsupported prologue mode %d", pro_mode);
  SEG_REQUIRE(C % 4 == 0 && ldx % 4 == 0 && lddy % 4 == 0 && ldg % 4 == 0 &&
                  (res == nullptr || ldr % 4 == 0),
              "dwconv bwd (slide): C/ldx/lddy/ldg/ldr must be multiples of 4");
  SEG_REQUIRE(rows == N * a.nstrips * a.nwblk,
              "dwconv bwd (slide): %d partial rows, the launch writes %d (seg_dwconv_grid_y)", rows,
              N * a.nstrips * a.nwblk);
  const dim3 grid((unsigned)((long)a.ncblk * a.nwblk * a.nstrips * N));
  if (dtype == DT_BF16) {
    if (res) slide_launch_bwd<bf16_t, true>(a, grid, st);
    else slide_launch_bwd<bf16_t, false>(a, grid, st);
  } else {
    if (res) slide_launch_bwd<float, true>(a, grid, st);
    else slide_launch_bwd<float, false>(a, grid, st);
  }
  return check_launch("dwconv3x3_bwd_fused (slide)");
}

}
```

### segmentron_amd/functional.py

```python
import contextlib
import dataclasses
import os
import weakref

import torch
import torch.distributed as dist
import torch.nn as nn

from . import hip_ops as K
from . import parallel
from .hip_ops import PRO_AFFINE, PRO_NONE, PRO_RELU


class BNState:
    __slots__ = ("gamma", "beta", "mean", "invstd", "scale", "shift", "count", "training", "group")

    def __init__(self, gamma, beta, mean, invstd, scale, shift, count, training, group=None):
        self.gamma, self.beta = gamma, beta
        self.mean, self.invstd, self.scale, self.shift = mean, invstd, scale, shift
        self.count, self.training, self.group = count, training, group


RELU, RELU6 = 1, 5


class Act:
    __slots__ = ("t", "bn", "relu")

    def __init__(self, t, bn=None, relu=False):
        self.t, self.bn, self.relu = t, bn, relu

    @property
    def pro(self):
        mode = (PRO_AFFINE if self.bn is not None else PRO_NONE) | int(self.relu)
        if self.bn is None:
            return (mode, None, None)
        return (mode, self.bn.scale, self.bn.shift)

    @property
    def params(self):
        if self.bn is None:
            return None, None
        return self.bn.gamma, self.bn.beta

    def with_relu(self):
        return Act(self.t, self.bn, self.relu or True)

    @property
    def shape(self):
        return self.t.shape


_sync_group = parallel.sync_group


class GradFork:
    __slots__ = ("g",)

    def __init__(self):
        self.g = None

    def take(self):
        g, self.g = self.g, None
        return g


def uses_batch_stats(bn):
    return not getattr(bn, "frozen", False) and (bn.training or bn.running_mean is None)


def finish_bn(bn, partial, count, mean_offset=None, y=None):
    use_batch = uses_batch_stats(bn)
    if not use_batch:
        scale, shift = eval_affine(bn)
        invstd = mean = None
        if torch.is_grad_enabled():
            mean = bn.running_mean
            invstd = torch.rsqrt(bn.running_var + bn.eps)
        return BNState(bn.weight, bn.bias, mean, invstd, scale, shift, count, False)
    if count <= 1 and _sync_group(bn) is None:
        raise ValueError("Expected more than 1 value per channel when training, got count=%d"
                         % count)
    group = _sync_group(bn)
    cnt = float(count)
    momentum = bn.momentum if bn.momentum is not None else 0.1
    track = bn.training and getattr(bn, "track_running_stats", False) \
        and bn.running_mean is not None
    rm, rv = (bn.running_mean, bn.running_var) if track else (None, None)
    if track:
        note_running_stats_changed()
    if group is None and y is not None and count <= K.SMALL_BN_ROWS:
        mean, invstd, scale, shift = K.bn_finalize_small(y, bn.weight, bn.bias, bn.eps, momentum,
                                                         rm, rv, mean_offset)
    elif group is None:
        mean, invstd, scale, shift = K.bn_finalize_p(partial, cnt, bn.weight, bn.bias, bn.eps,
                                                     momentum, rm, rv, mean_offset)
    else:
        C = partial.shape[-1]
        naive = parallel.is_naive_sync(bn)
        if naive:
            rm = rv = None
        box = parallel.mailbox(group)
        small = y is not None and count * dist.get_world_size(group) <= K.SMALL_BN_ROWS
        if box is not None and small:
            mean, invstd, scale, shift, cnt = K.bn_finalize_small_sync(
                box, y, bn.weight, bn.bias, bn.eps, momentum, rm, rv, mean_offset)
        elif box is not None:
            mean, invstd, scale, shift, cnt = K.bn_finalize_p_sync(
                box, partial, cnt, bn.weight, bn.bias, bn.eps, momentum, rm, rv, mean_offset)
        elif small:
            sums, cnt = parallel.allreduce_moments(K.bn_moments_small(y), group)
            mean, invstd, scale, shift = K.bn_finalize(sums, cnt, bn.weight, bn.bias, bn.eps,
                                                       momentum, rm, rv, mean_offset)
        else:
            sums, cnt = parallel.allreduce_forward_sums(partial.view(partial.shape[0], 2 * C),
                                                        cnt, group)
            mean, invstd, scale, shift = K.bn_finalize(sums, cnt, bn.weight, bn.bias, bn.eps,
                                                       momentum, rm, rv, mean_offset)
        if naive and track:
            mo = mean if mean_offset is None else mean + mean_offset
            parallel.naive_running_update(bn, mo, invstd)
            track = False
    if track and bn.num_batches_tracked is not None:
        if _COUNTER_SCOPE[0] > 0:
            _PENDING_COUNTERS.append(bn.num_batches_tracked)
        else:
            bn.num_batches_tracked.add_(1)
    return BNState(bn.weight, bn.bias, mean, invstd, scale, shift, cnt, True, group)


_PENDING_COUNTERS = []
_COUNTER_SCOPE = [0]


class bn_counter_scope:
    def __enter__(self):
        _COUNTER_SCOPE[0] += 1
        return self

    def __exit__(self, exc_type, exc, tb):
        _COUNTER_SCOPE[0] -= 1
        if _COUNTER_SCOPE[0] == 0:
            flush_bn_counters()
        return False


def flush_bn_counters():
    if _PENDING_COUNTERS:
        torch._foreach_add_(_PENDING_COUNTERS, 1)
        del _PENDING_COUNTERS[:]


def _sync_bwd_finalize(partial, bn):
    box = parallel.mailbox(bn.group)
    scale = parallel.grad_scale(bn.group)
    if box is not None and isinstance(bn.count, torch.Tensor):
        return K.bn_bwd_finalize_p_sync(box, partial, bn.count, bn.mean, bn.invstd, bn.gamma, scale)
    sums = parallel.allreduce_backward_sums(K.colsum(partial), bn.group)
    return K.bn_bwd_finalize(sums, bn.count, bn.mean, bn.invstd, bn.gamma, scale)


def bn_input_backward(g, x, bn, relu, chan_mul=None, inplace=False, elem_mul=None):
    mode = (PRO_AFFINE if bn is not None else PRO_NONE) | int(relu)
    if bn is None:
        if not relu and chan_mul is None and elem_mul is None:
            return g, None, None
        dx = K.bn_bwd_apply(g, x, (mode, None, None), chan_mul=chan_mul,
                            out=g if inplace else None, elem_mul=elem_mul)
        return dx, None, None
    pro = (mode, bn.scale, bn.shift)
    if (bn.group is None and not isinstance(bn.count, torch.Tensor) and bn.mean is not None
            and bn.count <= K.SMALL_BN_ROWS and g.dim() == 4
            and g.shape[0] * g.shape[1] * g.shape[2] <= K.SMALL_BN_ROWS):
        return K.bn_bwd_small(g, x, pro, bn.count, bn.mean, bn.invstd, bn.gamma, chan_mul,
                              elem_mul, bn.training, out=g if inplace else None)
    partial = K.bn_bwd_reduce_partial(g, x, pro, chan_mul, elem_mul)
    if bn.group is None:
        dgamma, dbeta, c0, c1 = K.bn_bwd_finalize_p(partial, bn.count, bn.mean, bn.invstd,
                                                    bn.gamma)
    else:
        dgamma, dbeta, c0, c1 = _sync_bwd_finalize(partial, bn)
    if not bn.training:
        c0 = c1 = None
    dx = K.bn_bwd_apply(g, x, pro, c0, c1, chan_mul, out=g if inplace else None,
                        elem_mul=elem_mul)
    return dx, dgamma, dbeta


_WCACHE = {}
_EPOCH = [1]


def _scope():
    return _EPOCH[0] if (torch.cuda.is_available() and torch.cuda.is_current_stream_capturing()) \
        else 0


def _hit(ent, param, scope):
    return (ent is not None and ent[0] == param._version and ent[1] == param.data_ptr()
            and ent[2]() is param and ent[4] == scope)


def cached_pack(param, kind, builder):
    key = (id(param), kind)
    ent = _WCACHE.get(key)
    scope = _scope()
    if _hit(ent, param, scope):
        return ent[3]
    val = builder()
    _WCACHE[key] = (param._version, param.data_ptr(), weakref.ref(param), val, scope)
    _note_miss()
    return val


_MISSES = [0]


# ... 14 lines not shown


@contextlib.contextmanager
def restrict_pack_plan(params):
    prev = _PLAN_FILTER[0]
    _PLAN_FILTER[0] = {id(p) for p in params}
    try:
        yield
    finally:
        _PLAN_FILTER[0] = prev
_PARAM_ALIAS = {}


def packed_pointwise(param, transpose, dtype):
    param = _PARAM_ALIAS.get(id(param), param)
    key = (id(param), ("pw", bool(transpose), dtype))
    scope = _scope()
    ent = _WCACHE.get(key)
    if _hit(ent, param, scope):
        return ent[3]
    _PACK_PLAN[(id(param), bool(transpose), dtype)] = weakref.ref(param)
    todo = []
    for (pid, tr, dt), ref in list(_PACK_PLAN.items()):
        p = ref()
        if p is None or id(p) != pid:
            del _PACK_PLAN[(pid, tr, dt)]
            continue
        if dt != dtype or p.device != param.device:
            continue
        if _PLAN_FILTER[0] is not None and pid not in _PLAN_FILTER[0] and p is not param:
            continue
        if _hit(_WCACHE.get((pid, ("pw", tr, dt))), p, scope):
            continue
        todo.append((p, tr))
    outs = K.pack_multi([(p.detach().view(p.shape[0], p.shape[1]), tr) for p, tr in todo], dtype)
    for (p, tr), val in zip(todo, outs):
        _WCACHE[(id(p), ("pw", tr, dtype))] = (p._version, p.data_ptr(), weakref.ref(p), val, scope)
        _note_miss()
    return _WCACHE[key][3]


_EVAL_PLAN = {}
EVAL_AFFINE_MAX_C = 2048


_STATS_EPOCH = [0]


def note_running_stats_changed():
    _STATS_EPOCH[0] += 1


def _eval_versions(bn):
    ts = (bn.weight, bn.bias, bn.running_mean, bn.running_var)
    return tuple(-1 if t is None else t._version for t in ts) \
        + tuple(0 if t is None else t.data_ptr() for t in ts) \
        + tuple(0 if t is None else id(t) for t in ts) \
        + (float(bn.eps), 0 if getattr(bn, "frozen", False) else _STATS_EPOCH[0])


def eval_affine(bn):
    key = (id(bn), "eval_affine")
    scope = _scope()

    def hit(m, k):
        ent = _WCACHE.get(k)
        return ent is not None and ent[0] == _eval_versions(m) and ent[2]() is m and ent[4] == scope \
            and ent[1] == m.running_mean.data_ptr()

    if hit(bn, key):
        return _WCACHE[key][3]
    if bn.running_mean.numel() > EVAL_AFFINE_MAX_C:
        val = K.bn_eval_affine(bn.weight, bn.bias, bn.running_mean, bn.running_var, bn.eps)
        _WCACHE[key] = (_eval_versions(bn), bn.running_mean.data_ptr(), weakref.ref(bn), val, scope)
        return val
    _EVAL_PLAN[id(bn)] = weakref.ref(bn)
    todo = []
    for mid, ref in list(_EVAL_PLAN.items()):
        m = ref()
        if m is None or id(m) != mid or m.running_mean is None:
            del _EVAL_PLAN[mid]
            continue
        if m is not bn:
            if m.running_mean.device != bn.running_mean.device or uses_batch_stats(m):
                continue
            if _PLAN_FILTER[0] is not None and (m.weight is None or id(m.weight) not in _PLAN_FILTER[0]):
                continue
            if hit(m, (mid, "eval_affine")):
                continue
        todo.append(m)
    outs = K.bn_eval_affine_multi([(m.weight, m.bias, m.running_mean, m.running_var, m.eps)
                                   for m in todo])
    for m, val in zip(todo, outs):
        _WCACHE[(id(m), "eval_affine")] = (_eval_versions(m), m.running_mean.data_ptr(),
                                           weakref.ref(m), val, scope)
        _note_miss()
    return _WCACHE[key][3]


def pack_conv_weight(w, cx, dtype):
    O, Cw, KH, KW = w.shape
    if KH == 1 and KW == 1 and cx == Cw:
        return w.detach().reshape(O, Cw).to(dtype)
    p = w.detach().permute(0, 2, 3, 1)
    if cx != Cw:
        p = torch.nn.functional.pad(p, (0, cx - Cw))
    return p.reshape(O, KH * KW * cx).to(dtype).contiguous()


def pack_conv_weight_dgrad(w, opad, dtype):
    O, Cw, KH, KW = w.shape
    if KH == 1 and KW == 1 and opad == O:
        out = torch.empty((Cw, O), dtype=dtype, device=w.device)
        out.copy_(w.detach().reshape(O, Cw).t())
        return out
    p = w.detach().flip(2, 3).permute(1, 2, 3, 0)
    if opad != O:
        p = torch.nn.functional.pad(p, (0, opad - O))
    return p.reshape(Cw, KH * KW * opad).to(dtype).contiguous()


def pack_conv_weight_tconv(w, opad, dtype):
    O, Cw, KH, KW = w.shape
    p = w.detach().permute(1, 2, 3, 0)
    if opad != O:
        p = torch.nn.functional.pad(p, (0, opad - O))
    return p.reshape(Cw, KH * KW * opad).to(dtype).contiguous()


def pack_dw_weight(w, flipped=False):
    C = w.shape[0]
    t = w.detach().reshape(C, 9)
    if flipped:
        t = t.flip(1)
    out = torch.empty((9, C), dtype=torch.float32, device=w.device)
    out.copy_(t.t())
    return out


def _round_up(v, m):
    return (v + m - 1) // m * m


class ConvSpec:

    def __init__(self, act, stride=1, pad=0, dil=1, out=None, want_stats=True):
        self.bn_in, self.relu = act.bn, act.relu
        self.pro = act.pro
        self.stride, self.pad, self.dil = stride, pad, dil
        self.out, self.want_stats = out, want_stats
        self.partial = None
        self.drop_bias = False
        self.fork = None


class _ConvFn(torch.autograd.Function):

    @staticmethod
    def forward(ctx, x, in_gamma, in_beta, weight, bias, spec):
        O, Cw, KH, KW = weight.shape
        cx, dt = x.shape[-1], x.dtype
        if KH == 1 and KW == 1 and cx == Cw and weight.dtype == torch.float32:
            wp = packed_pointwise(weight, False, dt)
        else:
            wp = cached_pack(weight, ("fwd", cx, dt), lambda: pack_conv_weight(weight, cx, dt))
        y, spec.partial = K.conv_gemm(x, wp, O, KH, KW, spec.stride, spec.pad, spec.dil, spec.pro,
                                      None if spec.drop_bias else bias, spec.out, spec.want_stats)
        spec.out = None
        ctx.spec = spec
        ctx.save_for_backward(x, weight)
        ctx.has_bias = bias is not None
        return y

    @staticmethod
    def backward(ctx, dy):
        x, weight = ctx.saved_tensors
        s = ctx.spec
        O, Cw, KH, KW = weight.shape
        vec = K.vec_of(x.dtype)
        N, Ho, Wo, _ = dy.shape
        if O % vec != 0 or K.nhwc(dy)[4] % vec != 0:
            dyp = torch.zeros((N, Ho, Wo, _round_up(O, vec)), dtype=dy.dtype, device=dy.device)
            dyp[..., :O] = dy
            dy_full, dy = dyp, dyp[..., :O]
        else:
            dy_full = dy
        Cx = x.shape[-1]
        Ow = dy_full.shape[-1]
        dWp = K.conv_wgrad(x, dy_full, Ow, KH, KW, s.stride, s.pad, s.dil, s.pro)[:O]
        if KH == 1 and KW == 1 and Cx == Cw:
            dW = dWp.view(O, Cw, 1, 1)
        else:
            dW = dWp.view(O, KH, KW, Cx)[..., :Cw].permute(0, 3, 1, 2).contiguous()
        dbias = None
        if ctx.has_bias and s.drop_bias:
            dbias = torch.zeros(O, dtype=torch.float32, device=dy.device)
        elif ctx.has_bias:
            dbias = K.bn_bwd_reduce(dy_full, dy_full, (PRO_NONE, None, None))[:O].float()
        dx = dgamma = dbeta = None
        if ctx.needs_input_grad[0]:
            Op, dt = dy_full.shape[-1], x.dtype
            if KH == 1 and KW == 1 and Op == O and weight.dtype == torch.float32:
                wt = packed_pointwise(weight, True, dt)
            else:
                wt = cached_pack(weight, ("dgrad", Op, dt),
                                 lambda: pack_conv_weight_dgrad(weight, Op, dt))
            res = None
            if s.fork is not None and s.fork.g is not None:
                res = s.fork.take()
            if s.stride == 1 and res is not None and KH == 1 and KW == 1 and s.bn_in is None \
                    and not s.relu and Cw % K.vec_of(dt) == 0 and res.dtype == dt:
                g, _ = K.conv_gemm(dy_full, wt, Cw, 1, 1, 1, 0, 1,
                                   ep=(res, _const(Cw, x.device, 0.0), _const(Cw, x.device, -1.0)))
                res = None
            elif s.stride == 1:
                g, _ = K.conv_gemm(dy_full, wt, Cw, KH, KW, 1, s.dil * (KH - 1) - s.pad, s.dil)
            elif KH == 1 and KW == 1 and s.pad == 0:
                g, _ = K.conv_gemm(dy_full, wt, Cw, 1, 1, 1, 0, 1,
                                   scatter=(x.shape[1], x.shape[2], s.stride))
            else:
                wt = cached_pack(weight, ("tconv", Op, dt),
                                 lambda: pack_conv_weight_tconv(weight, Op, dt))
                g, _ = K.conv_gemm(dy_full, wt, Cw, KH, KW, s.stride, s.pad, s.dil,
                                   tconv_out_hw=(x.shape[1], x.shape[2]))
            dx, dgamma, dbeta = bn_input_backward(g, x, s.bn_in, s.relu, inplace=True)
            if res is not None:
                dx = dx + res
        elif s.fork is not None:
            s.fork.g = None
        return dx, dgamma, dbeta, dW, dbias, None


_ONES = {}


def _const(c, device, value):
    key = (c, str(device), float(value))
    if key not in _ONES:
        _ONES[key] = torch.full((c,), float(value), dtype=torch.float32, device=device)
    return _ONES[key]


def _ones(c, device):
    return _const(c, device, 1.0)


class _FoldConvFn(torch.autograd.Function):

    @staticmethod
    def forward(ctx, x, in_gamma, in_beta, weight, spec):
        O, C = weight.shape[0], weight.shape[1]
        bn = spec.bn_in
        w2d = weight.detach().view(O, C)
        wp, wpt, bp = K.fold_weights(w2d, bn.scale, bn.shift, x.dtype,
                                     want_transpose=ctx.needs_input_grad[0])
        spec.mean_offset = bp
        bias = None if spec.drop_const else bp
        y, spec.partial = K.conv_gemm(x, wp, O, 1, 1, spec.stride, 0, 1, None, bias, spec.out,
                                      spec.want_stats)
        spec.out = None
        ctx.spec = spec
        ctx.wpt = wpt
        ctx.save_for_backward(x, weight)
        return y

    @staticmethod
    def backward(ctx, dy):
        x, weight = ctx.saved_tensors
        s = ctx.spec
        bn = s.bn_in
        O, C = weight.shape[0], weight.shape[1]
        if K.nhwc(dy)[4] % K.vec_of(dy.dtype) != 0:
            dy = dy.contiguous()
        dwp = K.conv_wgrad(x, dy, O, 1, 1, s.stride, 0, 1, None, raw_partial=True)
        db = None
        if not s.drop_const:
            db = K.bn_bwd_reduce(dy, dy, (PRO_NONE, None, None))[:O].float()
        dW, dsdt = K.fold_bwd_reduce(weight.detach().view(O, C), dwp, bn.scale, bn.shift, db)
        box = parallel.mailbox(bn.group) if bn.group is not None else None
        if box is not None and isinstance(bn.count, torch.Tensor):
            dgamma, dbeta, c0, c1 = K.fold_bwd_finalize_sync(
                box, dsdt, bn.count, bn.mean, bn.invstd, bn.gamma, bn.scale,
                parallel.grad_scale(bn.group))
        else:
            if bn.group is not None:
                dsdt = K.colsum(dsdt, f64=False)
                parallel.allreduce_backward_sums(dsdt, bn.group)
            dgamma, dbeta, c0, c1 = K.fold_bwd_finalize(
                dsdt, bn.count, bn.mean, bn.invstd, bn.gamma, bn.scale,
                parallel.grad_scale(bn.group) if bn.group is not None else 1.0)
        dx = None
        if ctx.needs_input_grad[0]:
            if s.stride == 1:
                dx, _ = K.conv_gemm(dy, ctx.wpt, C, 1, 1, 1, 0, 1,
                                    ep=(x, c0, c1) if bn.training else None)
            else:
                g, _ = K.conv_gemm(dy, ctx.wpt, C, 1, 1, 1, 0, 1,
                                   scatter=(x.shape[1], x.shape[2], s.stride))
                if bn.training:
                    ones = _ones(C, x.device)
                    dx = K.bn_bwd_apply(g, x, (PRO_AFFINE, ones, ones), c0, c1, out=g)
                else:
                    dx = g
        return dx, dgamma, dbeta, dW.view_as(weight), None


class _DwFn(torch.autograd.Function):

    @staticmethod
    def forward(ctx, x, in_gamma, in_beta, weight, spec):
        if K.dw_tiled(spec.stride, spec.dil):
            w = weight.detach()
        else:
            w = cached_pack(weight, "dw", lambda: pack_dw_weight(weight))
        y, spec.partial = K.dwconv(x, w, spec.stride, spec.dil, spec.pro, spec.out,
                                   spec.want_stats)
        spec.out = None
        ctx.spec = spec
        ctx.save_for_backward(x, weight)
        return y

    @staticmethod
    def backward(ctx, dy):
        x, weight = ctx.saved_tensors
        s = ctx.spec
        C = weight.shape[0]
        if K.nhwc(dy)[4] % K.vec_of(dy.dtype) != 0:
            dy = dy.contiguous()
        dx = dgamma = dbeta = None
        tiled = K.dw_tiled(s.stride, s.dil)
        big = x.numel() * x.element_size() >= (40 << 20)
        strided = s.stride == 2 and s.dil == 1 and C % 4 == 0 and weight.dtype == torch.float32
        if ctx.needs_input_grad[0] and ((s.stride == 1 and (tiled or big or s.dil > 2)) or strided):
            bn = s.bn_in
            box = parallel.mailbox(bn.group) if (bn is not None and bn.group is not None) else None
            both = bn is not None and (strided or tiled) and \
                (bn.group is None or (box is not None and isinstance(bn.count, torch.Tensor)))
            if strided:
                g, dW, pb = K.dwconv_bwd_fused_s2(x, dy, weight.detach().contiguous(), s.pro,
                                                  want_bn=bn is not None, raw_dw=both)
            elif tiled:
                res = None
                if bn is None and s.fork is not None and s.fork.g is not None \
                        and K.dwconv_bwd_fused_add_ok(x, s.dil):
                    res = s.fork.take()
                    if res.dtype != x.dtype or tuple(res.shape) != tuple(x.shape):
                        s.fork.g, res = res, None
                g, dW, pb = K.dwconv_bwd_fused(x, dy, weight.detach(), s.dil, s.pro,
                                               want_bn=bn is not None, torch_layout=True,
                                               raw_dw=both, res=res)
            else:
                w9c = cached_pack(weight, "dw", lambda: pack_dw_weight(weight))
                g, dW9c, pb = K.dwconv_bwd_fused(x, dy, w9c, s.dil, s.pro, want_bn=bn is not None)
                dW = dW9c.t().reshape(C, 1, 3, 3).contiguous()
            if bn is None:
                dx = g
            else:
                if both and pb.shape[0] <= 1024 and bn.group is None:
                    dgamma, dbeta, c0, c1, dW = K.dw_bwd_finalize(pb, dW, bn.count, bn.mean,
                                                                  bn.invstd, bn.gamma)
                elif both and pb.shape[0] <= 1024:
                    dgamma, dbeta, c0, c1, dW = K.dw_bwd_finalize_sync(
                        box, pb, dW, bn.count, bn.mean, bn.invstd, bn.gamma,
                        parallel.grad_scale(bn.group))
                elif both:
                    dW = K.dw_wgrad_finalize(dW, C)
                    if bn.group is None:
                        dgamma, dbeta, c0, c1 = K.bn_bwd_finalize_p(pb, bn.count, bn.mean,
                                                                    bn.invstd, bn.gamma)
                    else:
                        dgamma, dbeta, c0, c1 = _sync_bwd_finalize(pb, bn)
                elif bn.group is None:
                    dgamma, dbeta, c0, c1 = K.bn_bwd_finalize_p(pb, bn.count, bn.mean, bn.invstd,
                                                                bn.gamma)
                else:
                    dgamma, dbeta, c0, c1 = _sync_bwd_finalize(pb, bn)
                if not bn.training:
                    c0 = c1 = None
                dx = K.bn_bwd_apply(g, x, (PRO_AFFINE, bn.scale, bn.shift), c0, c1, out=g)
        else:
            tiled = K.dw_tiled(s.stride, s.dil)
            if tiled:
                dW = K.dwconv_wgrad(x, dy, s.stride, s.dil, s.pro, torch_layout=True)
            else:
                dW9c = K.dwconv_wgrad(x, dy, s.stride, s.dil, s.pro)
                dW = dW9c.t().reshape(C, 1, 3, 3).contiguous()
            if ctx.needs_input_grad[0]:
                if tiled:
                    w = weight.detach()
                elif s.stride == 1:
                    w = cached_pack(weight, "dw_flip", lambda: pack_dw_weight(weight, True))
                else:
                    w = cached_pack(weight, "dw", lambda: pack_dw_weight(weight))
                g = K.dwconv_dgrad(dy, w, s.stride, s.dil, (x.shape[1], x.shape[2]))
                dx, dgamma, dbeta = bn_input_backward(g, x, s.bn_in, s.relu, inplace=True)
        if s.fork is not None and s.fork.g is not None and dx is not None:
            dx = dx + s.fork.take()
        return dx, dgamma, dbeta, dW, None


class ApplySpec:
    def __init__(self, a, r=None, chan_mul=None, post_relu=False, out=None, elem_mul=None,
                 fork=None):
        self.elem_mul = elem_mul
        self.fork = fork
        self.bn_x, self.relu_x, self.pro_x = a.bn, a.relu, a.pro
        if r is not None:
            self.bn_r, self.relu_r, self.pro_r = r.bn, r.relu, r.pro
        else:
            self.bn_r, self.relu_r, self.pro_r = None, False, None
        self.chan_mul, self.post_relu, self.out = chan_mul, post_relu, out


class _ApplyFn(torch.autograd.Function):

    @staticmethod
    def forward(ctx, x, gx, bx, r, gr, br, spec):
        y = K.bn_apply(x, spec.pro_x, r, spec.pro_r, spec.chan_mul, spec.post_relu, spec.out,
                       spec.elem_mul)
        spec.out = None
        ctx.spec = spec
        ctx.has_r = r is not None
        if spec.post_relu:
            ctx.save_for_backward(x, r, y)
        else:
            ctx.save_for_backward(x, r)
        return y

    @staticmethod
    def backward(ctx, g):
        s = ctx.spec
        if s.post_relu:
            x, r, y = ctx.saved_tensors
            g = K.bn_bwd_apply(g, y, (PRO_RELU, None, None))
        else:
            x, r = ctx.saved_tensors
        dx, dgx, dbx = bn_input_backward(g, x, s.bn_x, s.relu_x, s.chan_mul, inplace=False,
                                         elem_mul=s.elem_mul)
        dr = dgr = dbr = None
        if ctx.has_r and ctx.needs_input_grad[3]:
            if s.fork is not None and s.bn_r is None and not s.relu_r:
                s.fork.g = g
            else:
                dr, dgr, dbr = bn_input_backward(g, r, s.bn_r, s.relu_r, None, inplace=False)
        return dx, dgx, dbx, dr, dgr, dbr, None


class AddUpSpec:
    def __init__(self, a, r, shift, post_relu, out=None):
        self.bn_x, self.relu_x, self.pro_x = a.bn, a.relu, a.pro
        self.bn_r, self.relu_r, self.pro_r = r.bn, r.relu, r.pro
        self.shift, self.post_relu, self.out = shift, post_relu, out


class _AddUpFn(torch.autograd.Function):

    @staticmethod
    def forward(ctx, x, gx, bx, r, gr, br, spec):
        y = K.nearest_add(x, spec.pro_x, r, spec.pro_r, spec.shift, spec.post_relu, spec.out)
        spec.out = None
        ctx.spec = spec
        if spec.post_relu:
            ctx.save_for_backward(x, r, y)
        else:
            ctx.save_for_backward(x, r)
        return y

    @staticmethod
    def backward(ctx, g):
        s = ctx.spec
        if s.post_relu:
            x, r, y = ctx.saved_tensors
            g = K.bn_bwd_apply(g, y, (PRO_RELU, None, None))
        else:
            x, r = ctx.saved_tensors
        dx = dgx = dbx = dr = dgr = dbr = None
        if ctx.needs_input_grad[3]:
            g_r = K.nearest_sum_bwd(g, s.shift)
            dr, dgr, dbr = bn_input_backward(g_r, r, s.bn_r, s.relu_r, inplace=True)
        if ctx.needs_input_grad[0]:
            dx, dgx, dbx = bn_input_backward(g, x, s.bn_x, s.relu_x, inplace=False)
        return dx, dgx, dbx, dr, dgr, dbr, None
# ... 269 lines not shown


def fork(t, n):
    if n <= 1 or not (torch.is_grad_enabled() and t.requires_grad):
        return (t,) * n
    return _ForkFn.apply(t, n)


def _scaled(t, gamma32, residual=None):
    C = t.shape[-1]
    sc = gamma32.expand(C).contiguous()
    zero = torch.zeros(C, dtype=torch.float32, device=t.device)
    return K.bn_apply(t, (PRO_AFFINE, sc, zero), residual, None if residual is None
                      else (PRO_NONE, None, None))


def _dot(a, b):
    C = a.shape[-1]
    return K.bn_bwd_reduce(a, b, (PRO_NONE, None, None))[C:2 * C].sum().float().view(1)


class _PAMFn(torch.autograd.Function):

    @staticmethod
    def forward(ctx, q, k, v, x, gamma):
        N, H, W, C = x.shape
        P, dt = H * W, x.dtype
        vec = K.vec_of(dt)
        Pp = _round_up(P, vec)
        g32 = gamma.detach().float().contiguous()
        raw = torch.empty((N, H, W, C), dtype=dt, device=x.device)
        atts = []
        for n in range(N):
            kp = torch.zeros((Pp, k.shape[-1]), dtype=dt, device=x.device)
            kp[:P] = k[n].reshape(P, -1)
            e = K.gemm_nt(q[n].reshape(P, -1).contiguous(), kp)
            a = K.row_softmax(e, P, dt)
            vt = torch.zeros((C, Pp), dtype=dt, device=x.device)
            vt[:, :P] = v[n].reshape(P, C).t()
            raw[n] = K.gemm_nt(a, vt).view(H, W, C)
            atts.append(a)
        ctx.save_for_backward(q, k, v, raw, g32, *atts)
        return _scaled(raw, g32, x)

    @staticmethod
    def backward(ctx, dout):
        q, k, v, raw, g32 = ctx.saved_tensors[:5]
        atts = ctx.saved_tensors[5:]
        N, H, W, C = raw.shape
        P, dt = H * W, raw.dtype
        Pp = atts[0].shape[1]
        dout = dout.contiguous()
        dgamma = _dot(dout, raw) if ctx.needs_input_grad[4] else None
        do = _scaled(dout, g32)
        dq, dk, dv = torch.empty_like(q), torch.empty_like(k), torch.empty_like(v)
        for n in range(N):
            a, don = atts[n], do[n].reshape(P, C)
            dv[n] = K.gemm_tn(a, don)[:P].to(dt).view(H, W, C)
            vp = torch.zeros((Pp, C), dtype=dt, device=raw.device)
            vp[:P] = v[n].reshape(P, C)
            de = K.row_softmax_bwd(a, K.gemm_nt(don, vp), P, dt)
            kt = torch.zeros((k.shape[-1], Pp), dtype=dt, device=raw.device)
            kt[:, :P] = k[n].reshape(P, -1).t()
            dq[n] = K.gemm_nt(de, kt).view(H, W, -1)
            dk[n] = K.gemm_tn(de, q[n].reshape(P, -1).contiguous())[:P].to(dt).view(H, W, -1)
        return dq, dk, dv, dout, dgamma


class _CAMFn(torch.autograd.Function):

    @staticmethod
    def forward(ctx, x, gamma):
        N, H, W, C = x.shape
        P, dt = H * W, x.dtype
        g32 = gamma.detach().float().contiguous()
        raw = torch.empty_like(x)
        atts = []
        for n in range(N):
            xn = x[n].reshape(P, C).contiguous()
            a = K.row_softmax(K.gemm_tn(xn, xn), C, dt, sign=-1.0)
            raw[n] = K.gemm_nt(xn, a).view(H, W, C)
            atts.append(a)
        ctx.save_for_backward(x, raw, g32, *atts)
        return _scaled(raw, g32, x)

    @staticmethod
    def backward(ctx, dout):
        x, raw, g32 = ctx.saved_tensors[:3]
        atts = ctx.saved_tensors[3:]
        N, H, W, C = x.shape
        P, dt = H * W, x.dtype
        dout = dout.contiguous()
        dgamma = _dot(dout, raw) if ctx.needs_input_grad[1] else None
        do = _scaled(dout, g32)
        dx = torch.empty_like(x)
        for n in range(N):
            a, xn, don = atts[n], x[n].reshape(P, C).contiguous(), do[n].reshape(P, C)
            de = K.row_softmax_bwd(a, K.gemm_tn(don, xn), C, torch.float32, sign=-1.0)
            sym = (de + de.t()).to(dt)
            g1 = K.gemm_nt(don, a.t().contiguous()).view(1, H, W, C)
            g2 = K.gemm_nt(xn, sym).view(1, H, W, C)
            K.bn_apply(g1, None, g2, None, out=dx[n:n + 1])
        dx = K.bn_apply(dx, None, dout, None)
        return dx, dgamma


def position_attention(q, k, v, x, gamma):
    return _PAMFn.apply(q, k, v, x, gamma)


def channel_attention(x, gamma):
    return _CAMFn.apply(x, gamma)


_NO_FOLD = os.environ.get("SEG_NO_FOLD") == "1"


class _GroupNormFn(torch.autograd.Function):

    @staticmethod
    def forward(ctx, y, weight, bias, groups, eps, out):
        N, H, W, C = y.shape
        mean_rstd, coef = K.gn_fwd_finalize(K.gn_moments(y), H * W, groups, weight, bias, eps)
        ctx.save_for_backward(y, weight, mean_rstd)
        ctx.groups, ctx.has_bias = groups, bias is not None
        return K.gn_affine(y, None, coef, out=out)

    @staticmethod
    def backward(ctx, dz):
        y, weight, mean_rstd = ctx.saved_tensors
        N, H, W, C = y.shape
        if dz.dtype != y.dtype:
            dz = dz.to(y.dtype)
        if not _sum_n_operand_ok(dz, K.vec_of(y.dtype)):
            dz = dz.contiguous()
        coef, contrib = K.gn_bwd_finalize(K.gn_moments(dz, y), H * W, ctx.groups, mean_rstd, weight)
        dx = K.gn_affine(dz, y, coef) if ctx.needs_input_grad[0] else None
        dw = db = None
        if weight is not None and (ctx.needs_input_grad[1] or ctx.needs_input_grad[2]):
            sums = K.colsum(contrib.view(N, 2 * C), f64=False)
            dw = sums[:C].to(weight.dtype) if ctx.needs_input_grad[1] else None
            db = sums[C:].to(weight.dtype) if ctx.has_bias and ctx.needs_input_grad[2] else None
        return dx, dw, db, None, None, None


def is_group_norm(norm):
    return isinstance(norm, torch.nn.GroupNorm)


def group_norm(y, gn, out=None):
    return Act(_GroupNormFn.apply(y, gn.weight, gn.bias, gn.num_groups, gn.eps, out))


def conv_bn(act, conv, bn=None, out=None, fork=None):
    x = act.t
    gn = bn if is_group_norm(bn) else None
    if gn is not None:
        bn = None
    batch_stats = bn is not None and uses_batch_stats(bn)
    spec = ConvSpec(act, conv.stride[0], conv.padding[0], conv.dilation[0],
                    None if gn is not None else out, want_stats=batch_stats)
    g, b = act.params
    foldable = (act.bn is not None and not act.relu and conv.kernel_size == (1, 1)
                and conv.padding[0] == 0 and conv.bias is None and not _NO_FOLD)
    if not foldable and (act.bn is not None or act.relu) and conv.out_channels >= 256:
        act = Act(materialize(act))
        x = act.t
        spec = ConvSpec(act, conv.stride[0], conv.padding[0], conv.dilation[0], out,
                        want_stats=batch_stats)
        g, b = act.params
    if foldable:
        spec.drop_const = batch_stats
        y = _FoldConvFn.apply(x, g, b, conv.weight, spec)
        offset = spec.mean_offset if batch_stats else None
    else:
        spec.drop_bias = batch_stats and conv.bias is not None
        spec.fork = fork
        y = _ConvFn.apply(x, g, b, conv.weight, conv.bias, spec)
        offset = conv.bias.detach() if spec.drop_bias else None
    if gn is not None:
        return group_norm(y, gn, out)
    if bn is None:
        return Act(y)
    N, Ho, Wo, _ = y.shape
    return Act(y, finish_bn(bn, spec.partial, N * Ho * Wo, offset, y=y))


def dwconv_bn(act, conv, bn, out=None, fork=None):
    gn = bn if is_group_norm(bn) else None
    spec = ConvSpec(act, conv.stride[0], conv.padding[0], conv.dilation[0],
                    None if gn is not None else out,
                    want_stats=gn is None and uses_batch_stats(bn))
    spec.fork = fork
    assert conv.padding[0] == conv.dilation[0] and conv.kernel_size[0] == 3
    g, b = act.params
    y = _DwFn.apply(act.t, g, b, conv.weight, spec)
    if gn is not None:
        return group_norm(y, gn, out)
    N, Ho, Wo, _ = y.shape
    return Act(y, finish_bn(bn, spec.partial, N * Ho * Wo, y=y))


def materialize(act, residual=None, chan_mul=None, post_relu=False, out=None, elem_mul=None,
                force=False, fork=None):
    if act.bn is None and not act.relu and residual is None and chan_mul is None and out is None \
            and not post_relu and elem_mul is None and not force:
        return act.t
    spec = ApplySpec(act, residual, chan_mul, post_relu, out, elem_mul, fork)
    gx, bx = act.params
    if residual is None:
        return _ApplyFn.apply(act.t, gx, bx, None, None, None, spec)
    gr, br = residual.params
    return _ApplyFn.apply(act.t, gx, bx, residual.t, gr, br, spec)


def add_upsampled(act, up, shift, post_relu=False, out=None):
    gx, bx = act.params
    gr, br = up.params
    return _AddUpFn.apply(act.t, gx, bx, up.t, gr, br, AddUpSpec(act, up, shift, post_relu, out))


def bilinear(act, out_hw, chan_mul=None, align_corners=True, out=None):
    spec = ResizeSpec(act, tuple(out_hw), chan_mul, align_corners, out)
    g, b = act.params
    return _BilinearFn.apply(act.t, g, b, spec)


_LAZY_EVAL = [os.environ.get("SEG_LAZY_EVAL_LOGITS") == "1"]


def criss_cross_attention(q, k, v, x, gamma):
    return _CCAFn.apply(q, k, v, x, gamma)


def lazy_eval_logits(enable=None):
    prev = _LAZY_EVAL[0]
    if enable is not None:
        _LAZY_EVAL[0] = bool(enable)
    return prev


def want_lazy_logits(training):
    if training:
        return torch.is_grad_enabled()
    return _LAZY_EVAL[0] and not torch.is_grad_enabled()


def logits_to_nchw(x, out_hw, align_corners=True, lazy=False):
    if lazy and align_corners:
        return LogitsView(x, out_hw, align_corners)
    return _LogitsFn.apply(x, tuple(out_hw), align_corners)


def global_avg_pool(x, keep_fp32=False):
    return _GapFn.apply(x, torch.float32 if keep_fp32 else x.dtype)


def max_pool(act, k, stride, pad):
    g, b = act.params
    return _MaxPoolFn.apply(act.t, g, b, PoolSpec(act, k, stride, pad))


def adaptive_avg_pool(x, o, keep_fp32=False):
    return _AdaptivePoolFn.apply(x, o, torch.float32 if keep_fp32 else x.dtype)


def dropout_mask(shape, p, dtype, device):
    keep = torch.rand(shape, device=device) >= p
    return (keep.to(torch.float32) / (1.0 - p)).to(dtype)


def concat_alias(buf, parts):
    return _CatFn.apply(buf, *parts)


def image_to_nhwc(x, dtype):
    return K.nchw_to_nhwc_pad(x, dtype)
```

### segmentron_amd/hip_ops.py

```python
import torch

from ._lib import LIB

PRO_NONE, PRO_RELU, PRO_AFFINE, PRO_AFFINE_RELU = 0, 1, 2, 3
_DT = {torch.float32: 0, torch.bfloat16: 1}


def vec_of(dtype):
    return 8 if dtype == torch.bfloat16 else 4


_raw_stream = getattr(torch._C, "_cuda_getCurrentRawStream", None)


def _stream():
    if _raw_stream is not None:
        return _raw_stream(torch.cuda.current_device())
    return torch.cuda.current_stream().cuda_stream


def _p(t):
    return 0 if t is None else t.data_ptr()


# ... 114 lines not shown
def gn_bwd_finalize(partial, HW, G, mean_rstd, gamma):
    N, _, _, C = partial.shape
    coef = torch.empty((N, 3, C), dtype=torch.float32, device=partial.device)
    contrib = torch.empty((N, 2, C), dtype=torch.float32, device=partial.device)
    LIB.call("seg_gn_bwd_finalize", _p(partial), N, HW, C, G, _p(mean_rstd), _p(gamma), _p(coef),
             _p(contrib), _stream())
    return coef, contrib


def gn_affine(u, v, coef, out=None):
    N, H, W, C, ldu = nhwc(u)
    ldv = 0 if v is None else nhwc(v)[4]
    if out is None:
        out = torch.empty((N, H, W, C), dtype=u.dtype, device=u.device)
    LIB.call("seg_gn_affine", _DT[u.dtype], _p(u), ldu, _p(v), ldv, _p(coef), _p(out),
             nhwc(out)[4], N, H * W, C, _stream())
    return out


def colsum_count(partial2d, count):
    R, L = partial2d.shape
    dev = partial2d.device
    out = torch.empty(L + 1, dtype=torch.float64, device=dev)
    ws = torch.empty(64 * L, dtype=torch.float64, device=dev) if R > 128 else None
    LIB.call("seg_colsum_count", _p(partial2d), R, L, _p(out), float(count), _p(ws), _stream())
    return out


def conv_wgrad(x, dy, O, KH, KW, stride, pad, dil, pro=None, raw_partial=False):
    N, Hi, Wi, C, ldx = nhwc(x)
    Nd, Ho, Wo, Od, lddy = nhwc(dy)
    assert Nd == N and Od == O
    mode, ps, pt = _pro(pro)
    K = KH * KW * C
    splits = LIB.query("seg_conv_gemm_wgrad_splits", _DT[x.dtype], N, Ho, Wo, C, O, KH, KW,
                       stride, pad, dil, mode)
    partial = torch.empty((splits, O * K), dtype=torch.float32, device=x.device)
    LIB.call("seg_conv_gemm_wgrad", _DT[x.dtype], _p(x), ldx, N, Hi, Wi, C, _p(dy), lddy, Ho, Wo,
             O, KH, KW, stride, pad, dil, mode, _p(ps), _p(pt), _p(partial), splits, _stream())
    if raw_partial:
        return partial
    if splits == 1:
        return partial.view(O, K)
    return colsum(partial, f64=False).view(O, K)


def dw_tiled(stride, dil):
    return stride == 1 and dil in (1, 2)


def _dw_weight_arg(w, C, stride, dil, flip):
    if w.dim() == 4 or (w.dim() == 2 and w.shape == (C, 9) and C != 9):
        if not dw_tiled(stride, dil):
            raise ValueError("depthwise strip kernels need tap-major [9, C] weights")
        return w, 1 | (2 if flip else 0)
    return w, (2 if flip else 0) if dw_tiled(stride, dil) else 0


def dwconv(x, w9c, stride, dil, pro=None, out=None, want_stats=False):
    N, Hi, Wi, C, ldx = nhwc(x)
    Ho, Wo = conv_out_size(Hi, 3, stride, dil, dil), conv_out_size(Wi, 3, stride, dil, dil)
    mode, ps, pt = _pro(pro)
    if out is None:
        out = torch.empty((N, Ho, Wo, C), dtype=x.dtype, device=x.device)
    ldy = nhwc(out)[4]
    w, layout = _dw_weight_arg(w9c, C, stride, dil, False)
    gy = LIB.query("seg_dwconv_grid_y", _DT[x.dtype], C, N, Ho, Wo, stride, dil, 0)
    partial = torch.empty((gy, 2, C), dtype=torch.float32, device=x.device) if want_stats else None
    LIB.call("seg_dwconv3x3", _DT[x.dtype], 0, _p(x), ldx, N, Hi, Wi, C, _p(w), layout, stride,
             dil, mode, _p(ps), _p(pt), _p(out), ldy, Ho, Wo, _p(partial), gy, _stream())
    return out, partial


def dwconv_dgrad(dy, w9c, stride, dil, in_hw, flipped=True):
    N, Ho, Wo, C, lddy = nhwc(dy)
    Hi, Wi = in_hw
    dx = torch.empty((N, Hi, Wi, C), dtype=dy.dtype, device=dy.device)
    gy = LIB.query("seg_dwconv_grid_y", _DT[dy.dtype], C, N, Hi, Wi, stride, dil, 0)
    if stride == 1:
        if w9c.dim() == 4:
            w, layout = w9c, 3
        elif dw_tiled(stride, dil):
            w, layout = w9c, 0 if flipped else 2
        else:
            w, layout = (w9c if flipped else w9c.flip(0).contiguous()), 0
        LIB.call("seg_dwconv3x3", _DT[dy.dtype], 0, _p(dy), lddy, N, Ho, Wo, C, _p(w), layout, 1,
                 dil, PRO_NONE, 0, 0, _p(dx), C, Hi, Wi, 0, gy, _stream())
    else:
        LIB.call("seg_dwconv3x3", _DT[dy.dtype], 1, _p(dy), lddy, N, Ho, Wo, C, _p(w9c), 0, stride,
                 dil, PRO_NONE, 0, 0, _p(dx), C, Hi, Wi, 0, gy, _stream())
    return dx


def dw_wgrad_finalize(pw, C):
    dW = torch.empty((C, 1, 3, 3), dtype=torch.float32, device=pw.device)
    LIB.call("seg_dwconv3x3_wgrad_finalize", _p(pw), pw.shape[0], C, _p(dW), _stream())
    return dW


def dw_bwd_finalize(pb, pw, count, mean, invstd, gamma):
    C = mean.numel()
    out = torch.empty((4, C), dtype=torch.float32, device=mean.device)
    dW = torch.empty((C, 1, 3, 3), dtype=torch.float32, device=mean.device)
    LIB.call("seg_dw_bwd_finalize", _p(pb), pb.shape[0], float(count), _p(mean), _p(invstd),
             _p(gamma), _p(out[0]), _p(out[1]), _p(out[2]), _p(out[3]), _p(pw), pw.shape[0],
             _p(dW), C, _stream())
    return out[0], out[1], out[2], out[3], dW


def dw_bwd_finalize_sync(box, pb, pw, count_dev, mean, invstd, gamma, grad_scale):
    C = mean.numel()
    out = torch.empty((4, C), dtype=torch.float32, device=mean.device)
    dW = torch.empty((C, 1, 3, 3), dtype=torch.float32, device=mean.device)
    LIB.call("seg_dw_bwd_finalize_sync", box.handle, _p(pb), pb.shape[0], _p(count_dev), _p(mean),
             _p(invstd), _p(gamma), _p(out[0]), _p(out[1]), _p(out[2]), _p(out[3]), _p(pw),
             pw.shape[0], _p(dW), C, float(grad_scale), _stream())
    return out[0], out[1], out[2], out[3], dW


def dwconv_bwd_fused_add_ok(x, dil):
    return bool(LIB.query("seg_dwconv3x3_bwd_fused_add_ok", int(dil)))


def dwconv_bwd_fused(x, dy, w, dil, pro=None, want_bn=False, torch_layout=False, raw_dw=False,
                     res=None):
    N, H, W, C, ldx = nhwc(x)
    lddy = nhwc(dy)[4]
    mode, ps, pt = _pro(pro)
    g = torch.empty((N, H, W, C), dtype=x.dtype, device=x.device)
    tiled = dw_tiled(1, dil)
    layout = 1 if w.dim() == 4 else 0
    if layout and not tiled:
        raise ValueError("depthwise strip kernels need tap-major [9, C] weights")
    gy = LIB.query("seg_dwconv_grid_y", _DT[x.dtype], C, N, H, W, 1, dil, 1)
    pw = torch.empty((gy, 9 * C), dtype=torch.float32, device=x.device)
    pb = torch.empty((gy, 2 * C), dtype=torch.float32, device=x.device) if want_bn else None
    if res is not None:
        assert dil == 1 and tuple(res.shape) == (N, H, W, C) and res.dtype == x.dtype
        LIB.call("seg_dwconv3x3_bwd_fused_add", _DT[x.dtype], _p(dy), lddy, _p(x), ldx, N, H, W,
                 C, _p(w), layout, mode, _p(ps), _p(pt), _p(res), nhwc(res)[4], _p(g), C, _p(pw),
                 _p(pb), gy, _stream())
    else:
        LIB.call("seg_dwconv3x3_bwd_fused", _DT[x.dtype], _p(dy), lddy, _p(x), ldx, N, H, W, C,
                 _p(w), layout, dil, mode, _p(ps), _p(pt), _p(g), C, _p(pw), _p(pb), gy, _stream())
    if raw_dw:
        return g, pw, pb
    if torch_layout:
        dW = torch.empty((C, 1, 3, 3), dtype=torch.float32, device=x.device)
        LIB.call("seg_dwconv3x3_wgrad_finalize", _p(pw), gy, C, _p(dW), _stream())
        return g, dW, pb
    return g, colsum(pw, f64=False).view(9, C), pb


def dwconv_bwd_fused_s2(x, dy, w, pro=None, want_bn=False, raw_dw=False):
    N, H, W, C, ldx = nhwc(x)
    Nd, Ho, Wo, Cd, lddy = nhwc(dy)
    assert (Nd, Ho, Wo, Cd) == (N, (H + 1) // 2, (W + 1) // 2, C) and tuple(w.shape) == (C, 1, 3, 3)
    mode, ps, pt = _pro(pro)
    g = torch.empty((N, H, W, C), dtype=x.dtype, device=x.device)
    gy = LIB.query("seg_dwconv3x3_s2_grid_y", C, N, H, W)
    pw = torch.empty((gy, 9 * C), dtype=torch.float32, device=x.device)
    pb = torch.empty((gy, 2 * C), dtype=torch.float32, device=x.device) if want_bn else None
    LIB.call("seg_dwconv3x3_s2_bwd_fused", _DT[x.dtype], _p(dy), lddy, _p(x), ldx, N, H, W, C,
             _p(w), mode, _p(ps), _p(pt), _p(g), C, _p(pw), _p(pb), gy, _stream())
    if raw_dw:
        return g, pw, pb
    dW = torch.empty((C, 1, 3, 3), dtype=torch.float32, device=x.device)
    LIB.call("seg_dwconv3x3_wgrad_finalize", _p(pw), gy, C, _p(dW), _stream())
    return g, dW, pb


def dwconv_wgrad(x, dy, stride, dil, pro=None, torch_layout=False):
    N, Hi, Wi, C, ldx = nhwc(x)
    _, Ho, Wo, _, lddy = nhwc(dy)
    mode, ps, pt = _pro(pro)
    gy = LIB.query("seg_dwconv_grid_y", _DT[x.dtype], C, N, Ho, Wo, stride, dil, 2)
    partial = torch.empty((gy, 9 * C), dtype=torch.float32, device=x.device)
    LIB.call("seg_dwconv3x3_wgrad", _DT[x.dtype], _p(x), ldx, N, Hi, Wi, C, _p(dy), lddy, Ho, Wo,
             stride, dil, mode, _p(ps), _p(pt), _p(partial), gy, _stream())
    if torch_layout:
        out = torch.empty((C, 1, 3, 3), dtype=torch.float32, device=x.device)
        LIB.call("seg_dwconv3x3_wgrad_finalize", _p(partial), gy, C, _p(out), _stream())
        return out
    return colsum(partial, f64=False).view(9, C)


def bn_finalize(sums, count, gamma, beta, eps, momentum, running_mean, running_var,
                mean_offset=None):
    C = sums.numel() // 2
    dev = sums.device
    out = torch.empty((4, C), dtype=torch.float32, device=dev)
    LIB.call("seg_bn_finalize", _p(sums), *_count(count), _p(gamma), _p(beta), float(eps),
             float(momentum), _p(running_mean), _p(running_var), _p(out[0]), _p(out[1]),
             _p(out[2]), _p(out[3]), C, _p(mean_offset), _stream())
    return out[0], out[1], out[2], out[3]


def bn_eval_affine(gamma, beta, rm, rv, eps):
    C = rm.numel()
    out = torch.empty((2, C), dtype=torch.float32, device=rm.device)
    LIB.call("seg_bn_eval_affine", _p(gamma), _p(beta), _p(rm), _p(rv), float(eps), _p(out[0]),
             _p(out[1]), C, _stream())
    return out[0], out[1]


def bn_eval_affine_multi(jobs):
    import ctypes
    n = len(jobs)
    outs = [torch.empty((2, j[2].numel()), dtype=torch.float32, device=j[2].device) for j in jobs]
    vp, fp, ip = ctypes.c_void_p * n, ctypes.c_float * n, ctypes.c_int * n
    LIB.call("seg_bn_eval_affine_multi", n, vp(*[_p(j[0]) for j in jobs]),
             vp(*[_p(j[1]) for j in jobs]), vp(*[_p(j[2]) for j in jobs]),
             vp(*[_p(j[3]) for j in jobs]), fp(*[float(j[4]) for j in jobs]),
             vp(*[o.data_ptr() for o in outs]), ip(*[j[2].numel() for j in jobs]), _stream())
    return [(o[0], o[1]) for o in outs]


def bn_apply(x, pro_x=None, r=None, pro_r=None, chan_mul=None, post_relu=False, out=None,
             elem_mul=None):
    N, H, W, C, ldx = nhwc(x)
    mx, sx, tx = _pro(pro_x)
    mr, sr, tr = _pro(pro_r)
    if out is None:
        out = torch.empty((N, H, W, C), dtype=x.dtype, device=x.device)
    ldy = nhwc(out)[4]
    ldr = nhwc(r)[4] if r is not None else 0
    ldm = nhwc(elem_mul)[4] if elem_mul is not None else 0
    LIB.call("seg_bn_apply", _DT[x.dtype], _p(x), ldx, mx, _p(sx), _p(tx), _p(r), ldr, mr, _p(sr),
             _p(tr), _p(chan_mul), H * W, _p(elem_mul), ldm, int(post_relu), _p(out), ldy,
             N * H * W, C, _stream())
    return out


def sum_n(tensors):
    import ctypes
    ts = list(tensors)
    while len(ts) > 1:
        group, ts = ts[:8], ts[8:]
        N, H, W, C, _ = nhwc(group[0])
        lds = [nhwc(t)[4] for t in group]
        assert all(t.shape == group[0].shape and t.dtype == group[0].dtype for t in group)
        out = torch.empty((N, H, W, C), dtype=group[0].dtype, device=group[0].device)
        n = len(group)
        LIB.call("seg_sum_n", _DT[out.dtype], n, (ctypes.c_void_p * n)(*[t.data_ptr() for t in group]),
                 (ctypes.c_long * n)(*lds), _p(out), C, N * H * W, C, _stream())
        ts.insert(0, out)
    return ts[0]


def nearest_add(x, pro_x, r, pro_r, shift, post_relu=False, out=None):
    N, H, W, C, ldx = nhwc(x)
    Nr, Hr, Wr, Cr, ldr = nhwc(r)
    if (Nr, Hr << shift, Wr << shift, Cr) != (N, H, W, C):
        raise ValueError("nearest_add: %s is not %s upsampled by 2^%d"
                         % (tuple(x.shape), tuple(r.shape), shift))
    mx, sx, tx = _pro(pro_x)
    mr, sr, tr = _pro(pro_r)
    if out is None:
        out = torch.empty((N, H, W, C), dtype=x.dtype, device=x.device)
    LIB.call("seg_nearest_add", _DT[x.dtype], _p(x), ldx, mx, _p(sx), _p(tx), _p(r), ldr, mr,
             _p(sr), _p(tr), shift, int(post_relu), _p(out), nhwc(out)[4], N, H, W, C, _stream())
    return out


def nearest_sum_bwd(g, shift):
    N, H, W, C, ldg = nhwc(g)
    out = torch.empty((N, H >> shift, W >> shift, C), dtype=g.dtype, device=g.device)
    LIB.call("seg_nearest_sum_bwd", _DT[g.dtype], _p(g), ldg, N, H, W, C, shift, _p(out), C,
             _stream())
    return out


def bn_bwd_reduce_partial(g, x, pro, chan_mul=None, elem_mul=None):
    N, H, W, C, ldg = nhwc(g)
    ldx = nhwc(x)[4]
    mode, s, t = _pro(pro)
    M = N * H * W
    gy = LIB.query("seg_bn_bwd_grid_y", _DT[g.dtype], C, M)
    partial = torch.empty((gy, 2 * C), dtype=torch.float32, device=g.device)
    ldm = nhwc(elem_mul)[4] if elem_mul is not None else 0
    LIB.call("seg_bn_bwd_reduce", _DT[g.dtype], _p(g), ldg, _p(x), ldx, mode, _p(s), _p(t),
             _p(chan_mul), H * W, _p(elem_mul), ldm, M, C, _p(partial), gy, _stream())
    return partial


def bn_bwd_small(g, x, pro, count, mean, invstd, gamma, chan_mul=None, elem_mul=None,
                 training=True, out=None):
    N, H, W, C, ldg = nhwc(g)
    ldx = nhwc(x)[4]
    mode, s, t = _pro(pro)
    if out is None:
        out = torch.empty((N, H, W, C), dtype=g.dtype, device=g.device)
    lddx = nhwc(out)[4]
    dgb = torch.empty((2, C), dtype=torch.float32, device=g.device)
    ldm = nhwc(elem_mul)[4] if elem_mul is not None else 0
    LIB.call("seg_bn_bwd_small", _DT[g.dtype], _p(g), ldg, _p(x), ldx, _p(out), lddx, N * H * W, C,
             mode, _p(s), _p(t), _p(mean), _p(invstd), _p(gamma), _p(chan_mul), H * W,
             _p(elem_mul), ldm, float(count), 1 if training else 0, _p(dgb[0]), _p(dgb[1]),
             _stream())
    return out, dgb[0], dgb[1]


def bn_bwd_reduce(g, x, pro, chan_mul=None):
    return colsum(bn_bwd_reduce_partial(g, x, pro, chan_mul), f64=True)


def _ws(R, C, dev):
    return torch.empty(128 * C, dtype=torch.float64, device=dev) if R > 1024 else None


def bn_finalize_p(partial, count, gamma, beta, eps, momentum, running_mean, running_var,
                  mean_offset=None):
    R = partial.shape[0]
    C = partial.numel() // (2 * R)
    out = torch.empty((4, C), dtype=torch.float32, device=partial.device)
    ws = _ws(R, C, partial.device)
    LIB.call("seg_bn_finalize_p", _p(partial), R, float(count), _p(gamma), _p(beta), float(eps),
             float(momentum), _p(running_mean), _p(running_var), _p(out[0]), _p(out[1]),
             _p(out[2]), _p(out[3]), C, _p(mean_offset), _p(ws), _stream())
    return out[0], out[1], out[2], out[3]


SMALL_BN_ROWS = 1024


def bn_finalize_small(y, gamma, beta, eps, momentum, running_mean, running_var, mean_offset=None):
    N, H, W, C, ldy = nhwc(y)
    out = torch.empty((4, C), dtype=torch.float32, device=y.device)
    LIB.call("seg_bn_finalize_small", _DT[y.dtype], _p(y), ldy, N * H * W, C, _p(gamma), _p(beta),
             float(eps), float(momentum), _p(running_mean), _p(running_var), _p(out[0]),
             _p(out[1]), _p(out[2]), _p(out[3]), _p(mean_offset), _stream())
    return out[0], out[1], out[2], out[3]


def bn_moments_small(y):
    N, H, W, C, ldy = nhwc(y)
    out = torch.empty(2 * C + 1, dtype=torch.float64, device=y.device)
    LIB.call("seg_bn_moments_small", _DT[y.dtype], _p(y), ldy, N * H * W, C, _p(out), _stream())
    return out


def bn_finalize_small_sync(box, y, gamma, beta, eps, momentum, running_mean, running_var,
                           mean_offset=None):
    N, H, W, C, ldy = nhwc(y)
    out = torch.empty((4, C), dtype=torch.float32, device=y.device)
    cnt = torch.empty(1, dtype=torch.float64, device=y.device)
    LIB.call("seg_bn_finalize_small_sync", box.handle, _DT[y.dtype], _p(y), ldy, N * H * W, C,
             _p(gamma), _p(beta), float(eps), float(momentum), _p(running_mean), _p(running_var),
             _p(out[0]), _p(out[1]), _p(out[2]), _p(out[3]), _p(mean_offset), _p(cnt), _stream())
    return out[0], out[1], out[2], out[3], cnt


def bn_finalize_p_sync(box, partial, local_count, gamma, beta, eps, momentum, running_mean,
                       running_var, mean_offset=None):
    R = partial.shape[0]
    C = partial.numel() // (2 * R)
    out = torch.empty((4, C), dtype=torch.float32, device=partial.device)
    cnt = torch.empty(1, dtype=torch.float64, device=partial.device)
    ws = _ws(R, C, partial.device)
    LIB.call("seg_bn_finalize_p_sync", box.handle, _p(partial), R, float(local_count), _p(gamma),
             _p(beta), float(eps), float(momentum), _p(running_mean), _p(running_var), _p(out[0]),
             _p(out[1]), _p(out[2]), _p(out[3]), C, _p(mean_offset), _p(cnt), _p(ws), _stream())
    return out[0], out[1], out[2], out[3], cnt


def bn_bwd_finalize_p_sync(box, partial, count_dev, mean, invstd, gamma, grad_scale):
    C = mean.numel()
    out = torch.empty((4, C), dtype=torch.float32, device=mean.device)
    ws = _ws(partial.shape[0], C, mean.device)
    LIB.call("seg_bn_bwd_finalize_p_sync", box.handle, _p(partial), partial.shape[0], _p(count_dev),
             _p(mean), _p(invstd), _p(gamma), _p(out[0]), _p(out[1]), _p(out[2]), _p(out[3]), C,
             float(grad_scale), _p(ws), _stream())
    return out[0], out[1], out[2], out[3]


def bn_bwd_finalize_p(partial, count, mean, invstd, gamma):
    R = partial.shape[0]
    C = mean.numel()
    out = torch.empty((4, C), dtype=torch.float32, device=mean.device)
    ws = _ws(R, C, mean.device)
    LIB.call("seg_bn_bwd_finalize_p", _p(partial), R, float(count), _p(mean), _p(invstd),
             _p(gamma), _p(out[0]), _p(out[1]), _p(out[2]), _p(out[3]), C, _p(ws), _stream())
    return out[0], out[1], out[2], out[3]


def bn_bwd_finalize(sums, count, mean, invstd, gamma, grad_scale=1.0):
    C = mean.numel()
    out = torch.empty((4, C), dtype=torch.float32, device=mean.device)
    LIB.call("seg_bn_bwd_finalize_s", _p(sums), *_count(count), _p(mean), _p(invstd), _p(gamma),
             _p(out[0]), _p(out[1]), _p(out[2]), _p(out[3]), C, float(grad_scale), _stream())
    return out[0], out[1], out[2], out[3]


def bn_bwd_apply(g, x, pro, c0=None, c1=None, chan_mul=None, out=None, elem_mul=None):
    N, H, W, C, ldg = nhwc(g)
    ldx = nhwc(x)[4]
    mode, s, t = _pro(pro)
    if out is None:
        out = torch.empty((N, H, W, C), dtype=g.dtype, device=g.device)
    lddx = nhwc(out)[4]
    ldm = nhwc(elem_mul)[4] if elem_mul is not None else 0
    LIB.call("seg_bn_bwd_apply", _DT[g.dtype], _p(g), ldg, _p(x), ldx, mode, _p(s), _p(t), _p(c0),
             _p(c1), _p(chan_mul), H * W, _p(elem_mul), ldm, _p(out), lddx, N * H * W, C,
             _stream())
    return out


def fold_weights(w2d, scale, shift, dtype, want_transpose=False, want_bias=True):
    O, C = w2d.shape
    dev = w2d.device
    wp = torch.empty((O, C), dtype=dtype, device=dev)
    wpt = torch.empty((C, O), dtype=dtype, device=dev) if want_transpose else None
    bp = torch.empty(O, dtype=torch.float32, device=dev) if want_bias else None
    LIB.call("seg_fold_weights", _DT[dtype], _p(w2d), _p(scale), _p(shift), _p(wp), _p(wpt),
             _p(bp), O, C, _stream())
    return wp, wpt, bp


def fold_bwd_reduce(w2d, dwp, scale, shift, db=None):
    O, C = w2d.shape
    S = 1 if tuple(dwp.shape) == (O, C) else dwp.shape[0]
    assert dwp.numel() == S * O * C and dwp.is_contiguous()
    R = LIB.query("seg_fold_bwd_rows", O)
    if S > 8 and R == 1:
        dwp = colsum(dwp.view(S, O * C), f64=False).view(O, C)
        S = 1
    dW = torch.empty((O, C), dtype=torch.float32, device=w2d.device)
    dsdt = torch.empty((R, 2 * C), dtype=torch.float32, device=w2d.device)
    LIB.call("seg_fold_bwd_reduce", _p(w2d), _p(dwp), S, _p(scale), _p(shift), _p(db), _p(dW),
             _p(dsdt), O, C, _stream())
    return dW, dsdt


def fold_bwd_finalize(dsdt, count, mean, invstd, gamma, scale, grad_scale=1.0):
    C = mean.numel()
    out = torch.empty((4, C), dtype=torch.float32, device=mean.device)
    dsdt = dsdt.view(-1, 2 * C)
    LIB.call("seg_fold_bwd_finalize_s", _p(dsdt), dsdt.shape[0], *_count(count), _p(mean),
             _p(invstd), _p(gamma), _p(scale), _p(out[0]), _p(out[1]), _p(out[2]), _p(out[3]), C,
             float(grad_scale), _stream())
    return out[0], out[1], out[2], out[3]


def fold_bwd_finalize_sync(box, dsdt, count_dev, mean, invstd, gamma, scale, grad_scale):
    C = mean.numel()
    out = torch.empty((4, C), dtype=torch.float32, device=mean.device)
    dsdt = dsdt.view(-1, 2 * C)
    LIB.call("seg_fold_bwd_finalize_sync", box.handle, _p(dsdt), dsdt.shape[0], _p(count_dev),
             _p(mean), _p(invstd), _p(gamma), _p(scale), _p(out[0]), _p(out[1]), _p(out[2]),
             _p(out[3]), C, float(grad_scale), _stream())
    return out[0], out[1], out[2], out[3]


def maxpool(x, k, stride, pad, pro=None):
    N, Hi, Wi, C, ldx = nhwc(x)
    Ho, Wo = (Hi + 2 * pad - k) // stride + 1, (Wi + 2 * pad - k) // stride + 1
    mode, ps, pt = _pro(pro)
    y = torch.empty((N, Ho, Wo, C), dtype=x.dtype, device=x.device)
    idx = torch.empty((N, Ho, Wo, C), dtype=torch.uint8, device=x.device)
    LIB.call("seg_maxpool_fwd", _DT[x.dtype], _p(x), ldx, N, Hi, Wi, C, k, stride, pad, mode,
             _p(ps), _p(pt), _p(y), C, Ho, Wo, _p(idx), _stream())
    return y, idx


def maxpool_bwd(gy, idx, in_hw, k, stride, pad):
    N, Ho, Wo, C, ldgy = nhwc(gy)
    Hi, Wi = in_hw
    gx = torch.empty((N, Hi, Wi, C), dtype=gy.dtype, device=gy.device)
    LIB.call("seg_maxpool_bwd", _DT[gy.dtype], _p(gx), C, N, Hi, Wi, C, k, stride, pad, _p(gy),
             ldgy, Ho, Wo, _p(idx), _stream())
    return gx


def adaptive_avgpool_sums(x, o):
    N, H, W, C, ldx = nhwc(x)
    chunks = LIB.query("seg_adaptive_avgpool_chunks", H, W, o)
    partial = torch.empty((chunks, N * o * o * C), dtype=torch.float32, device=x.device)
    LIB.call("seg_adaptive_avgpool_partial", _DT[x.dtype], _p(x), ldx, N, H, W, C, o, _p(partial),
             chunks, _stream())
    sums = partial[0] if chunks == 1 else colsum(partial, f64=False)
    return sums.view(N, o, o, C)


def adaptive_avgpool_bwd(gy, in_hw):
    N, o, _, C, ldgy = nhwc(gy)
    H, W = in_hw
    gx = torch.empty((N, H, W, C), dtype=gy.dtype, device=gy.device)
    LIB.call("seg_adaptive_avgpool_bwd", _DT[gy.dtype], _p(gx), C, N, H, W, C, o, _p(gy), ldgy,
             _stream())
    return gx


_BIN_AREAS = {}


def adaptive_bin_areas(H, W, o, device):
    key = (H, W, o, str(device))
    if key not in _BIN_AREAS:
        _BIN_AREAS[key] = _adaptive_bin_areas(H, W, o, device)
    return _BIN_AREAS[key]


def _adaptive_bin_areas(H, W, o, device):
    import math
    hs = [math.ceil((i + 1) * H / o) - (i * H) // o for i in range(o)]
    ws = [math.ceil((j + 1) * W / o) - (j * W) // o for j in range(o)]
    return torch.tensor([[float(a * b) for b in ws] for a in hs], device=device)


def bilinear(x, out_hw, pro=None, chan_mul=None, align_corners=True, out=None):
    N, Hi, Wi, C, ldx = nhwc(x)
    Ho, Wo = out_hw
    mode, s, t = _pro(pro)
    if out is None:
        out = torch.empty((N, Ho, Wo, C), dtype=x.dtype, device=x.device)
    ldy = nhwc(out)[4]
    LIB.call("seg_bilinear_fwd", _DT[x.dtype], _p(x), ldx, N, Hi, Wi, C, mode, _p(s), _p(t),
             _p(chan_mul), _p(out), ldy, Ho, Wo, int(align_corners), _stream())
    return out


def bilinear_bwd(gy, in_hw, align_corners=True):
    N, Ho, Wo, C, ldgy = nhwc(gy)
    Hi, Wi = in_hw
    gx = torch.empty((N, Hi, Wi, C), dtype=gy.dtype, device=gy.device)
    LIB.call("seg_bilinear_bwd", _DT[gy.dtype], _p(gx), C, N, Hi, Wi, C, _p(gy), ldgy, Ho, Wo,
             int(align_corners), _stream())
    return gx


def upsample_to_nchw(x, C, out_hw, align_corners=True):
    N, Hi, Wi, _, ldx = nhwc(x)
    Ho, Wo = out_hw
    out = torch.empty((N, C, Ho, Wo), dtype=torch.float32, device=x.device)
    LIB.call("seg_upsample_to_nchw", _DT[x.dtype], _p(x), ldx, N, Hi, Wi, C, _p(out), Ho, Wo,
             int(align_corners), _stream())
    return out


def upsample_to_nchw_bwd(gy, in_hw, dtype, pitch, align_corners=True):
    if not gy.is_cuda or gy.dtype != torch.float32:
        raise RuntimeError("upsample_to_nchw_bwd needs a float32 HIP device tensor")
    N, C, Ho, Wo = gy.shape
    Hi, Wi = in_hw
    gy = gy.contiguous()
    gx = torch.empty((N, Hi, Wi, pitch), dtype=dtype, device=gy.device)
    LIB.call("seg_upsample_to_nchw_bwd", _DT[dtype], _p(gx), pitch, N, Hi, Wi, C, _p(gy), Ho, Wo,
             int(align_corners), _stream())
    return gx


def nchw_to_nhwc_pad(x, dtype):
    if not x.is_cuda:
        raise RuntimeError("segmentron_amd ops need HIP device tensors (no CPU fallback)")
    N, Cin, H, W = x.shape
    x = x.contiguous().float()
    y = torch.empty((N, H, W, vec_of(dtype)), dtype=dtype, device=x.device)
    LIB.call("seg_nchw_to_nhwc_pad", _DT[dtype], _p(x), N, Cin, H, W, _p(y), _stream())
    return y


def upsample_ce_fwd(lo, target, out_hw, ignore_index, align_corners=True):
    N, Hi, Wi, C, ld = nhwc(lo)
    H, W = out_hw
    if not target.is_cuda or target.dtype != torch.int64 or tuple(target.shape) != (N, H, W):
        raise RuntimeError("upsample_ce: target must be an int64 HIP tensor [N, H, W] = %s, got %s"
                           % ((N, H, W), tuple(target.shape)))
    target = target.contiguous()
    blocks = LIB.query("seg_upsample_ce_blocks", N, H, W)
    ws = torch.empty(2 * blocks, dtype=torch.float64, device=lo.device)
    out = torch.empty(2, dtype=torch.float32, device=lo.device)
    LIB.call("seg_upsample_ce_fwd", _DT[lo.dtype], _p(lo), ld, N, Hi, Wi, C, _p(target), H, W,
             int(ignore_index), int(align_corners), _p(ws), _p(out), _stream())
    return out


def upsample_ce_bwd(lo, target, out_hw, ignore_index, loss_out, grad_out, pitch,
                    align_corners=True):
    N, Hi, Wi, C, ld = nhwc(lo)
    H, W = out_hw
    grad_out = grad_out.reshape(1).to(torch.float32).contiguous()
    dlo = torch.empty((N, Hi, Wi, pitch), dtype=lo.dtype, device=lo.device)
    LIB.call("seg_upsample_ce_bwd", _DT[lo.dtype], _p(lo), ld, N, Hi, Wi, C,
             _p(target.contiguous()), H, W, int(ignore_index), int(align_corners), _p(loss_out),
             _p(grad_out), _p(dlo), pitch, _stream())
    return dlo
# ... 130 lines not shown
```

### segmentron_amd/models/backbones/xception.py

```python
import torch
import torch.nn as nn

from ... import functional as F
from ...config import cfg
from ...modules import SeparableConv2d
from .build import BACKBONE_REGISTRY

__all__ = ["Xception65", "XceptionBlock", "xception65"]


class XceptionBlock(nn.Module):

    def __init__(self, channel_list, stride=1, dilation=1, skip_connection_type="conv",
                 relu_first=True, low_feat=False, norm_layer=nn.BatchNorm2d):
        super().__init__()
        assert len(channel_list) == 4
        if skip_connection_type not in ("conv", "sum", "none"):
            raise ValueError("Unsupported skip connection type.")
        self.skip_connection_type = skip_connection_type
        self.relu_first = relu_first
        self.low_feat = low_feat
        c = channel_list
        if skip_connection_type == "conv":
            self.conv = nn.Conv2d(c[0], c[3], 1, stride=stride, bias=False)
            self.bn = norm_layer(c[3])
        self.sep_conv1 = SeparableConv2d(c[0], c[1], dilation=dilation, relu_first=relu_first,
                                         norm_layer=norm_layer)
        self.sep_conv2 = SeparableConv2d(c[1], c[2], dilation=dilation, relu_first=relu_first,
                                         norm_layer=norm_layer)
        self.sep_conv3 = SeparableConv2d(c[2], c[3], dilation=dilation, relu_first=relu_first,
                                         stride=stride, norm_layer=norm_layer)
        self.last_inp_channels = c[3]

    def forward(self, inputs):
        fork = None
        if (self.skip_connection_type == "sum" and self.relu_first and inputs.bn is None
                and not inputs.relu and torch.is_grad_enabled() and inputs.t.requires_grad):
            fork = F.GradFork()
        skip_in = inputs
        if self.skip_connection_type == "conv":
            t = F.fork(inputs.t, 2)
            inputs, skip_in = F.Act(t[0], inputs.bn, inputs.relu), F.Act(t[1], inputs.bn, inputs.relu)
        sc1 = self.sep_conv1(inputs, fork=fork) if fork is not None else self.sep_conv1(inputs)
        sc2 = self.sep_conv2(sc1)
        low = sc2
        if self.low_feat:
            t = F.fork(sc2.t, 2)
            sc2, low = F.Act(t[0], sc2.bn, sc2.relu), F.Act(t[1], sc2.bn, sc2.relu)
        residual = self.sep_conv3(sc2)
        if self.skip_connection_type == "conv":
            shortcut = F.conv_bn(skip_in, self.conv, self.bn)
            outputs = F.Act(F.materialize(residual, residual=shortcut))
        elif self.skip_connection_type == "sum":
            outputs = F.Act(F.materialize(residual, residual=inputs, fork=fork))
        else:
            outputs = residual
        return (outputs, low) if self.low_feat else outputs


class Xception65(nn.Module):

    def __init__(self, norm_layer=nn.BatchNorm2d):
        super().__init__()
        os_ = cfg.MODEL.OUTPUT_STRIDE
        if os_ == 32:
            b3_stride, mid_dil, exit_dil, exit_stride = 2, 1, (1, 1), 2
        elif os_ == 16:
            b3_stride, mid_dil, exit_dil, exit_stride = 2, 1, (1, 2), 1
        elif os_ == 8:
            b3_stride, mid_dil, exit_dil, exit_stride = 1, 2, (2, 4), 1
        else:
            raise NotImplementedError
        self.conv1 = nn.Conv2d(3, 32, 3, stride=2, padding=1, bias=False)
        self.bn1 = norm_layer(32)
        self.relu = nn.ReLU()
        self.conv2 = nn.Conv2d(32, 64, 3, stride=1, padding=1, bias=False)
        self.bn2 = norm_layer(64)
        self.block1 = XceptionBlock([64, 128, 128, 128], stride=2, norm_layer=norm_layer)
        self.block2 = XceptionBlock([128, 256, 256, 256], stride=2, low_feat=True,
                                    norm_layer=norm_layer)
        self.block3 = XceptionBlock([256, 728, 728, 728], stride=b3_stride, low_feat=True,
                                    norm_layer=norm_layer)
        for i in range(4, 20):
            setattr(self, "block%d" % i,
                    XceptionBlock([728] * 4, dilation=mid_dil, skip_connection_type="sum",
                                  norm_layer=norm_layer))
        self.block20 = XceptionBlock([728, 728, 1024, 1024], stride=exit_stride,
                                     dilation=exit_dil[0], norm_layer=norm_layer)
        self.block21 = XceptionBlock([1024, 1536, 1536, 2048], dilation=exit_dil[1],
                                     skip_connection_type="none", relu_first=False,
                                     norm_layer=norm_layer)

    def forward(self, x):
        from ... import compute_dtype
        a = F.Act(F.image_to_nhwc(x, compute_dtype()))
        a = F.conv_bn(a, self.conv1, self.bn1)
        a.relu = True
        a = F.conv_bn(a, self.conv2, self.bn2)
        a.relu = True
        a = self.block1(a)
        a, c1 = self.block2(a)
        a, c2 = self.block3(a)
        for i in range(4, 20):
            a = getattr(self, "block%d" % i)(a)
        c3 = a
        a = self.block20(c3)
        c4 = self.block21(a)
        return c1, c2, c3, c4


@BACKBONE_REGISTRY.register()
def xception65(norm_layer=nn.BatchNorm2d):
    return Xception65(norm_layer=norm_layer)
```

### segmentron_amd/modules/basic.py

```python
from collections import OrderedDict

import torch.nn as nn

from .. import functional as F

__all__ = ["SeparableConv2d", "_ConvBNReLU", "InvertedResidual"]


class SeparableConv2d(nn.Module):

    def __init__(self, inplanes, planes, kernel_size=3, stride=1, dilation=1, relu_first=True,
                 bias=False, norm_layer=nn.BatchNorm2d):
        super().__init__()
        assert kernel_size == 3 and not bias
        self.relu_first = relu_first
        layers = [
            ("depthwise", nn.Conv2d(inplanes, inplanes, kernel_size, stride=stride,
                                    padding=dilation, dilation=dilation, groups=inplanes,
                                    bias=bias)),
            ("bn_depth", norm_layer(inplanes)),
            ("pointwise", nn.Conv2d(inplanes, planes, 1, bias=bias)),
            ("bn_point", norm_layer(planes)),
        ]
        if relu_first:
            layers.insert(0, ("relu", nn.ReLU()))
        else:
            layers.insert(2, ("relu1", nn.ReLU(inplace=True)))
            layers.append(("relu2", nn.ReLU(inplace=True)))
        self.block = nn.Sequential(OrderedDict(layers))

    def forward(self, act, fork=None):
        b = self.block
        if self.relu_first:
            d = F.dwconv_bn(act.with_relu(), b.depthwise, b.bn_depth, fork=fork)
            return F.conv_bn(d, b.pointwise, b.bn_point)
        assert fork is None
        d = F.dwconv_bn(act, b.depthwise, b.bn_depth)
        d.relu = True
        p = F.conv_bn(d, b.pointwise, b.bn_point)
        p.relu = True
        return p


class _ConvBNReLU(nn.Module):

    def __init__(self, in_channels, out_channels, kernel_size, stride=1, padding=0, dilation=1,
                 groups=1, relu6=False, norm_layer=nn.BatchNorm2d):
        super().__init__()
        if groups not in (1, in_channels) or (groups != 1 and in_channels != out_channels):
            raise NotImplementedError("only dense and depthwise convolutions are on the HIP path")
        self.conv = nn.Conv2d(in_channels, out_channels, kernel_size, stride, padding, dilation,
                              groups, bias=False)
        self.bn = norm_layer(out_channels)
        self.relu = nn.ReLU6(True) if relu6 else nn.ReLU(True)
        self.relu6 = relu6
        self.depthwise = groups != 1

    def forward(self, act, out=None):
        if self.depthwise:
            a = F.dwconv_bn(act, self.conv, self.bn, out=out)
        else:
            a = F.conv_bn(act, self.conv, self.bn, out=out)
        a.relu = F.RELU6 if self.relu6 else F.RELU
        return a


class InvertedResidual(nn.Module):

    def __init__(self, in_channels, out_channels, stride, expand_ratio, dilation=1,
                 norm_layer=nn.BatchNorm2d):
        super().__init__()
        assert stride in [1, 2]
        self.use_res_connect = stride == 1 and in_channels == out_channels
        inter = int(round(in_channels * expand_ratio))
        layers = []
        if expand_ratio != 1:
            layers.append(_ConvBNReLU(in_channels, inter, 1, relu6=True, norm_layer=norm_layer))
        layers.extend([
            _ConvBNReLU(inter, inter, 3, stride, dilation, dilation, groups=inter, relu6=True,
                        norm_layer=norm_layer),
            nn.Conv2d(inter, out_channels, 1, bias=False),
            norm_layer(out_channels)])
        self.conv = nn.Sequential(*layers)

    def forward(self, x):
        a = x
        mods = list(self.conv)
        for m in mods[:-2]:
            a = m(a)
        a = F.conv_bn(a, mods[-2], mods[-1])
        if self.use_res_connect:
            return F.Act(F.materialize(a, residual=x))
        return a
```

Baseline: 90.40 images/sec.

## Fuse pointwise BN-fold backward correction into depthwise bwd and group middle-flow wgrads

Adds a dgrad GEMM variant that accumulates the BN-fold dscale/dshift sums in its epilogue and defers the BN correction (c0, c1) to the following depthwise backward kernel, which applies it on the fly. Separately, the pointwise weight gradients of the 48 middle-flow separable convs are batched into one grouped wgrad launch through a per-layer pointer table, with each layer's scale applied as its result is written. Together these are meant to remove one full elementwise pass per separable conv and many small wgrad launches. In exchange they add complex cross-layer state (CorrLink, weight groups) and fallback paths when shape or dtype conditions are not met.

New measurement: 90.39 images/sec (median of 6 runs). No clear change (-0.0%).

```diff
diff --git a/include/segmentron_hip.h b/include/segmentron_hip.h
--- a/include/segmentron_hip.h
+++ b/include/segmentron_hip.h
@@ -46,6 +46,13 @@
                                 const float* pro_scale, const float* pro_shift, const void* res,
                                 long ldr, void* g, long ldg, float* partial_w, float* partial_bn,
                                 int grid_y, void* stream);
+
+int seg_dwconv3x3_bwd_fused_corr(int dtype, const void* dy, long lddy, const void* x, long ldx,
+                                 int N, int H, int W, int C, const float* w9c, int w_layout,
+                                 int pro_mode, const float* pro_scale, const float* pro_shift,
+                                 const void* res, long ldr, const void* d, long ldd,
+                                 const float* c0, const float* c1, void* g, long ldg,
+                                 float* partial_w, float* partial_bn, int grid_y, void* stream);
 
 int seg_colsum(const float* in, long R, int L, double* out_d, float* out_f, double* ws,
                void* stream);
@@ -123,6 +130,11 @@
 
 int seg_fold_weights(int dtype, const float* W, const float* scale, const float* shift, void* Wp,
                      void* WpT, float* bprime, int O, int C, void* stream);
+int seg_conv_gemm_dgrad_sums_rows(long M, int C);
+int seg_conv_gemm_dgrad_sums(const void* dy, long lddy, int M, int O, const void* wt, int C,
+                             const float* scale, const void* x, long ldx, void* y, long ldy,
+                             float* dsdt, int rows, int want_dt, void* stream);
+int seg_conv_wgrad_grouped(const long* table, int L, int M, int O, int C, void* stream);
 int seg_fold_bwd_rows(int O);
 int seg_fold_bwd_reduce(const float* W, const float* dWp, int splits, const float* scale,
                         const float* shift, const float* db, float* dW, float* dsdt, int O, int C,
diff --git a/segmentron_amd/csrc/conv_gemm_args.h b/segmentron_amd/csrc/conv_gemm_args.h
--- a/segmentron_amd/csrc/conv_gemm_args.h
+++ b/segmentron_amd/csrc/conv_gemm_args.h
@@ -22,12 +22,15 @@
   int M, K;
   int out_H, out_W, out_s;
   int tiles_m, tiles_n;
+  int sums_dt;
 };
 
 int px256_tiles_m(long M);
 int launch_conv_gemm_px256(int dtype, ConvGemmArgs a, hipStream_t stream);
 bool conv_gemm_glds_usable(int dtype, const ConvGemmArgs& a);
 int launch_conv_gemm_glds(ConvGemmArgs a, hipStream_t stream);
+int glds_sums_rows_per_tile(long M, int O);
+int launch_conv_gemm_glds_sums(ConvGemmArgs a, hipStream_t stream);
 bool conv_gemm_glds_kxk_usable(int dtype, const ConvGemmArgs& a);
 int launch_conv_gemm_glds_kxk(ConvGemmArgs a, hipStream_t stream);
 
diff --git a/segmentron_amd/csrc/conv_gemm_glds.hip b/segmentron_amd/csrc/conv_gemm_glds.hip
--- a/segmentron_amd/csrc/conv_gemm_glds.hip
+++ b/segmentron_amd/csrc/conv_gemm_glds.hip
@@ -5,7 +5,7 @@
 namespace seg {
 
 
-template <bool EP, bool STATS, bool KXK = false, int IMS = 4>
+template <bool EP, bool STATS, bool KXK = false, int IMS = 4, bool SUMS = false>
 __global__ __launch_bounds__(GL_THREADS, 2) void conv_gemm_glds_kernel(const ConvGemmArgs a) {
   typedef bf16_t T;
   constexpr int VEC = 8;
@@ -49,7 +49,11 @@
   for (int k = 0; k < VEC; ++k) ssum[k] = ssq[k] = 0.f;
   float c0v[VEC], c1v[VEC];
   const bool epc = EP && o < a.O;
-  if (epc) {
+  if (SUMS) {
+#pragma unroll
+    for (int k = 0; k < VEC; ++k) c0v[k] = 0.f;
+    if (epc) load_params<VEC>(a.ep_c0, o, c0v);
+  } else if (epc) {
     load_params<VEC>(a.ep_c0, o, c0v);
     load_params<VEC>(a.ep_c1, o, c1v);
   }
@@ -103,13 +107,23 @@
         Vec<float>::unpack(val[q], f);
         Vec<float>::unpack(vhi[q], f + 4);
         Vec<T>::unpack(xr[q], xv);
-        if (epc) {
+        if (SUMS) {
+          if (p < a.M) {
+#pragma unroll
+            for (int k = 0; k < VEC; ++k) {
+              ssum[k] = fmaf(f[k], xv[k], ssum[k]);
+              ssq[k] += f[k];
+            }
+          }
+#pragma unroll
+          for (int k = 0; k < VEC; ++k) f[k] *= c0v[k];
+        } else if (epc) {
 #pragma unroll
           for (int k = 0; k < VEC; ++k) f[k] = f[k] - c0v[k] - c1v[k] * xv[k];
         }
         val[q] = Vec<T>::pack(f);
       }
-      if (STATS && (!EP || p < a.M)) {
+      if (STATS && !SUMS && (!EP || p < a.M)) {
         float f[VEC];
         Vec<T>::unpack(val[q], f);
 #pragma unroll
@@ -147,7 +161,7 @@
       if (oc < a.O) {
         float* dst = a.stat_partial + (long)tile_m * 2 * a.O;
         dst[oc] = red[0 * 256 + tid] + red[2 * 256 + tid];
-        dst[a.O + oc] = red[1 * 256 + tid] + red[3 * 256 + tid];
+        dst[a.O + oc] = (SUMS && !a.sums_dt) ? 0.f : red[1 * 256 + tid] + red[3 * 256 + tid];
       }
     }
   }
@@ -186,11 +200,11 @@
   return (int)((M + bm - 1) / bm);
 }
 
-template <bool EP, bool STATS, bool KXK, int IMS>
+template <bool EP, bool STATS, bool KXK, int IMS, bool SUMS = false>
 static int launch_glds_inst(const ConvGemmArgs& a, hipStream_t stream) {
   static const int once = [] {
     return (int)hipFuncSetAttribute(
-        reinterpret_cast<const void*>(&conv_gemm_glds_kernel<EP, STATS, KXK, IMS>),
+        reinterpret_cast<const void*>(&conv_gemm_glds_kernel<EP, STATS, KXK, IMS, SUMS>),
         hipFuncAttributeMaxDynamicSharedMemorySize, GL_LDS_BYTES);
   }();
   if (once != 0) {
@@ -198,8 +212,8 @@
     return 2;
   }
   const dim3 grid(a.tiles_m * a.tiles_n), block(GL_THREADS);
-  hipLaunchKernelGGL((conv_gemm_glds_kernel<EP, STATS, KXK, IMS>), grid, block, GL_LDS_BYTES,
-                     stream, a);
+  hipLaunchKernelGGL((conv_gemm_glds_kernel<EP, STATS, KXK, IMS, SUMS>), grid, block,
+                     GL_LDS_BYTES, stream, a);
   return check_launch(KXK ? "conv_gemm_fwd (glds KxK)" : "conv_gemm_fwd (glds)");
 }
 
@@ -225,6 +239,18 @@
   return launch_glds_rows<false, false, false>(a, stream);
 }
 
+int glds_sums_rows_per_tile(long M, int O) { return glds_pick_rows(M, O, false); }
+
+int launch_conv_gemm_glds_sums(ConvGemmArgs a, hipStream_t stream) {
+  const int bm = glds_sums_rows_per_tile(a.M, a.O);
+  a.tiles_m = (a.M + bm - 1) / bm;
+  a.tiles_n = (a.O + GL_BN - 1) / GL_BN;
+  if (bm == 256) return launch_glds_inst<true, true, false, 4, true>(a, stream);
+  if (bm == 192) return launch_glds_inst<true, true, false, 3, true>(a, stream);
+  set_error("conv_gemm_glds (sums): no %d-row tile on the eight-wave kernel", bm);
+  return 2;
+}
+
 bool conv_gemm_glds_kxk_usable(int dtype, const ConvGemmArgs& a) {
   return dtype == DT_BF16 && a.pro_mode == PRO_NONE && a.bias == nullptr && a.ep_x == nullptr &&
          a.KH * a.KW > 1 && a.stride == 1 && a.tconv == 0 && a.out_s == 1 && (a.C % 32) == 0 &&
@@ -238,3 +264,29 @@
 }
 
 }
+
+extern "C" int seg_conv_gemm_dgrad_sums_rows(long M, int C) {
+  const int bm = seg::glds_sums_rows_per_tile(M, C);
+  return (int)((M + bm - 1) / bm);
+}
+
+extern "C" int seg_conv_gemm_dgrad_sums(const void* dy, long lddy, int M, int O, const void* wt,
+                                        int C, const float* scale, const void* x, long ldx,
+                                        void* y, long ldy, float* dsdt, int rows, int want_dt,
+                                        void* stream) {
+  using namespace seg;
+  ConvGemmArgs a = {};
+  a.x = dy; a.w = wt; a.y = y; a.stat_partial = dsdt;
+  a.ep_x = x; a.ep_c0 = scale; a.ldep = ldx;
+  a.ldx = lddy; a.ldy = ldy;
+  a.N = 1; a.Hi = 1; a.Wi = M; a.C = O; a.Ho = 1; a.Wo = M; a.O = C;
+  a.KH = a.KW = a.stride = a.dil = 1; a.pad = 0; a.out_s = 1;
+  a.pro_mode = PRO_NONE; a.M = M; a.K = O; a.sums_dt = want_dt;
+  SEG_REQUIRE(M > 0 && dy && wt && scale && x && y && dsdt, "conv_gemm_dgrad_sums: bad arguments");
+  SEG_REQUIRE(conv_gemm_glds_usable(DT_BF16, a) && (ldx % 8) == 0,
+              "conv_gemm_dgrad_sums: bf16 with O, C and pitches multiples of 8");
+  SEG_REQUIRE(rows == seg_conv_gemm_dgrad_sums_rows(M, C),
+              "conv_gemm_dgrad_sums: %d partial rows, the launch writes %d", rows,
+              seg_conv_gemm_dgrad_sums_rows(M, C));
+  return launch_conv_gemm_glds_sums(a, (hipStream_t)stream);
+}
diff --git a/segmentron_amd/csrc/conv_gemm_wgrad_args.h b/segmentron_amd/csrc/conv_gemm_wgrad_args.h
--- a/segmentron_amd/csrc/conv_gemm_wgrad_args.h
+++ b/segmentron_amd/csrc/conv_gemm_wgrad_args.h
@@ -18,6 +18,20 @@
   int chunk;
 };
 
+constexpr int WG_GROUP_MAX = 64;
+struct WgGroupEntry {
+  const void* dy;
+  const void* x;
+  const float* s;
+  float* dw;
+  int lddy, ldx;
+};
+struct WgGroup {
+  WgGroupEntry e[WG_GROUP_MAX];
+  int n;
+};
+int launch_conv_wgrad_grouped(WgradArgs a, const WgGroup& gt, hipStream_t stream);
+
 bool conv_wgrad_glds_usable(int dtype, const WgradArgs& a);
 int conv_wgrad_glds_splits(long M, int O, int K);
 int launch_conv_wgrad_glds(WgradArgs a, hipStream_t stream);
diff --git a/segmentron_amd/csrc/conv_gemm_wgrad_glds.hip b/segmentron_amd/csrc/conv_gemm_wgrad_glds.hip
--- a/segmentron_amd/csrc/conv_gemm_wgrad_glds.hip
+++ b/segmentron_amd/csrc/conv_gemm_wgrad_glds.hip
@@ -30,8 +30,8 @@
   return __builtin_bit_cast(bf16x8, v);
 }
 
-template <bool KXK>
-__global__ __launch_bounds__(WG_THREADS, 2) void conv_wgrad_glds_kernel(const WgradArgs a) {
+template <bool KXK, bool GROUPED>
+__device__ __forceinline__ void conv_wgrad_glds_body(const WgradArgs& a, const WgGroup* gt) {
   extern __shared__ __attribute__((aligned(16))) unsigned char smem_raw[];
   lds_byte_t* lds = (lds_byte_t*)smem_raw;
   const int tid = threadIdx.x, lane = tid & 63;
@@ -41,9 +41,19 @@
   const int L = xcd_remap(blockIdx.x, tiles * a.splits);
   const int tile = L % tiles, split = L / tiles;
   const int o0 = (tile / a.tiles_k) * WG_BM, c0 = (tile % a.tiles_k) * WG_BN;
-  const int p0 = split * a.chunk;
-  const int p1 = min(a.M, p0 + a.chunk);
+  const int p0 = GROUPED ? 0 : split * a.chunk;
+  const int p1 = GROUPED ? a.M : min(a.M, p0 + a.chunk);
   const int nslot = (p1 - p0 + WG_BK - 1) / WG_BK;
+  const void* dy_base = a.dy;
+  const void* x_base = a.x;
+  long lddy = a.lddy, ldx = a.ldx;
+  if (GROUPED) {
+    const WgGroupEntry& e = gt->e[split];
+    dy_base = e.dy;
+    x_base = e.x;
+    lddy = e.lddy;
+    ldx = e.ldx;
+  }
 
   const unsigned char* zero = reinterpret_cast<const unsigned char*>(g_gl_zero);
   const int rr = lane >> 4;
@@ -62,10 +72,10 @@
 #pragma unroll
   for (int j = 0; j < 2; ++j) {
     prow[j] = p0 + (wave * 2 + j) * 4 + rr;
-    src[j] = reinterpret_cast<const unsigned char*>(a.dy) +
-             ((long)prow[j] * a.lddy + o0 + c16 * 8) * 2;
-    src[2 + j] = reinterpret_cast<const unsigned char*>(a.x) +
-                 ((long)prow[j] * a.ldx + c0 + c16 * 8) * 2;
+    src[j] = reinterpret_cast<const unsigned char*>(dy_base) +
+             ((long)prow[j] * lddy + o0 + c16 * 8) * 2;
+    src[2 + j] = reinterpret_cast<const unsigned char*>(x_base) +
+                 ((long)prow[j] * ldx + c0 + c16 * 8) * 2;
     if (KXK) {
       pw[j] = prow[j] % a.Wo;
       const int t = prow[j] / a.Wo;
@@ -73,7 +83,7 @@
       pn[j] = t / a.Ho;
     }
   }
-  const long inc_dy = (long)WG_BK * a.lddy * 2, inc_x = (long)WG_BK * a.ldx * 2;
+  const long inc_dy = (long)WG_BK * lddy * 2, inc_x = (long)WG_BK * ldx * 2;
   auto issue = [&](int slot) {
     lds_byte_t* base = lds + (slot & 3) * WG_SLOT + (wave * 2) * 1024;
 #pragma unroll
@@ -164,8 +174,22 @@
   asm volatile("s_waitcnt vmcnt(0) lgkmcnt(0)" ::: "memory");
 #undef WG_WAIT_FRAGS
 
+  const int r32 = lane & 31, hh = lane >> 5;
+  if (GROUPED) {
+    const WgGroupEntry& e = gt->e[split];
+#pragma unroll
+    for (int jb = 0; jb < 2; ++jb) {
+      const int c = c0 + (wc * 2 + jb) * 32 + r32;
+      const float sc = c < a.K ? e.s[c] : 0.f;
+#pragma unroll
+      for (int q = 0; q < 16; ++q) {
+        const int o = o0 + wo * 32 + (q & 3) + 8 * (q >> 2) + 4 * hh;
+        if (o < a.O && c < a.K) e.dw[(long)o * a.K + c] = acc[jb][q] * sc;
+      }
+    }
+    return;
+  }
   float* __restrict__ P = a.partial + (long)split * a.O * a.K;
-  const int r32 = lane & 31, hh = lane >> 5;
 #pragma unroll
   for (int jb = 0; jb < 2; ++jb) {
     const int c = c0 + (wc * 2 + jb) * 32 + r32;
@@ -175,6 +199,16 @@
       if (o < a.O && c < a.K) P[(long)o * a.K + c] = acc[jb][e];
     }
   }
+}
+
+template <bool KXK>
+__global__ __launch_bounds__(WG_THREADS, 2) void conv_wgrad_glds_kernel(const WgradArgs a) {
+  conv_wgrad_glds_body<KXK, false>(a, nullptr);
+}
+
+__global__ __launch_bounds__(WG_THREADS, 2) void conv_wgrad_grouped_kernel(const WgradArgs a,
+                                                                          const WgGroup gt) {
+  conv_wgrad_glds_body<false, true>(a, &gt);
 }
 
 bool conv_wgrad_glds_usable(int dtype, const WgradArgs& a) {
@@ -221,4 +255,50 @@
   return check_launch("conv_gemm_wgrad (glds)");
 }
 
-}
+int launch_conv_wgrad_grouped(WgradArgs a, const WgGroup& gt, hipStream_t stream) {
+  a.tiles_o = (a.O + WG_BM - 1) / WG_BM;
+  a.tiles_k = (a.K + WG_BN - 1) / WG_BN;
+  a.splits = gt.n;
+  a.chunk = 0;
+  static const int once = (int)hipFuncSetAttribute(
+      reinterpret_cast<const void*>(&conv_wgrad_grouped_kernel),
+      hipFuncAttributeMaxDynamicSharedMemorySize, WG_LDS);
+  if (once != 0) {
+    set_error("conv_wgrad_grouped: cannot reserve %d bytes of LDS", WG_LDS);
+    return 2;
+  }
+  const dim3 grid(a.tiles_o * a.tiles_k * gt.n), block(WG_THREADS);
+  hipLaunchKernelGGL(conv_wgrad_grouped_kernel, grid, block, WG_LDS, stream, a, gt);
+  return check_launch("conv_wgrad_grouped");
+}
+
+}
+
+extern "C" int seg_conv_wgrad_grouped(const long* table, int L, int M, int O, int C,
+                                      void* stream) {
+  using namespace seg;
+  SEG_REQUIRE(table != nullptr && L >= 1 && L <= WG_GROUP_MAX,
+              "conv_wgrad_grouped: 1 .. %d layers per launch, got %d", WG_GROUP_MAX, L);
+  SEG_REQUIRE(M >= 1 && O >= 8 && C >= 8 && O % 8 == 0 && C % 8 == 0,
+              "conv_wgrad_grouped: O, C must be multiples of 8 (O=%d C=%d M=%d)", O, C, M);
+  WgGroup gt;
+  gt.n = L;
+  for (int l = 0; l < L; ++l) {
+    const long* r = table + 6L * l;
+    WgGroupEntry& e = gt.e[l];
+    e.dy = reinterpret_cast<const void*>(r[0]);
+    e.x = reinterpret_cast<const void*>(r[1]);
+    e.s = reinterpret_cast<const float*>(r[2]);
+    e.dw = reinterpret_cast<float*>(r[3]);
+    SEG_REQUIRE(e.dy && e.x && e.s && e.dw && r[4] >= O && r[5] >= C && r[4] % 8 == 0 &&
+                    r[5] % 8 == 0 && r[4] < (1L << 31) && r[5] < (1L << 31),
+                "conv_wgrad_grouped: layer %d: null pointer or bad pitch", l);
+    e.lddy = (int)r[4];
+    e.ldx = (int)r[5];
+  }
+  WgradArgs a = {};
+  a.N = 1; a.Hi = a.Ho = 1; a.Wi = a.Wo = M; a.C = C; a.O = O;
+  a.KH = a.KW = a.stride = a.dil = 1; a.pad = 0; a.pro_mode = PRO_NONE;
+  a.M = M; a.K = C;
+  return launch_conv_wgrad_grouped(a, gt, (hipStream_t)stream);
+}
diff --git a/segmentron_amd/csrc/dwconv.hip b/segmentron_amd/csrc/dwconv.hip
--- a/segmentron_amd/csrc/dwconv.hip
+++ b/segmentron_amd/csrc/dwconv.hip
@@ -571,6 +571,25 @@
   return launch_dw_bwd_tiled(dtype, dy, lddy, x, ldx, N, H, W, C, w9c, w_layout, 1, pro_mode,
                              pro_scale, pro_shift, g, ldg, partial_w, partial_bn, grid_y,
                              (hipStream_t)stream, res, ldr);
+}
+
+extern "C" int seg_dwconv3x3_bwd_fused_corr(int dtype, const void* dy, long lddy, const void* x,
+                                            long ldx, int N, int H, int W, int C, const float* w9c,
+                                            int w_layout, int pro_mode, const float* pro_scale,
+                                            const float* pro_shift, const void* res, long ldr,
+                                            const void* d, long ldd, const float* c0,
+                                            const float* c1, void* g, long ldg, float* partial_w,
+                                            float* partial_bn, int grid_y, void* stream) {
+  using namespace seg;
+  SEG_REQUIRE(dtype == DT_BF16 && dw_slide_supported(1, 1, C),
+              "dwconv3x3_bwd_fused_corr: bf16, C %% 4 == 0 (sliding kernel) only");
+  SEG_REQUIRE(((pro_mode & PRO_AFFINE) == 0) || (pro_scale && pro_shift),
+              "dwconv3x3_bwd_fused_corr: affine prologue without scale/shift");
+  SEG_REQUIRE(grid_y >= 1 && partial_w != nullptr && d != nullptr,
+              "dwconv3x3_bwd_fused_corr: bad grid/partials/d");
+  return launch_dw_slide_bwd(dtype, dy, lddy, x, ldx, N, H, W, C, w9c, w_layout, pro_mode,
+                             pro_scale, pro_shift, g, ldg, partial_w, partial_bn, grid_y,
+                             (hipStream_t)stream, res, res ? ldr : 0, d, ldd, c0, c1);
 }
 
 extern "C" int seg_dwconv3x3_bwd_fused(int dtype, const void* dy, long lddy, const void* x,
diff --git a/segmentron_amd/csrc/dwconv_slide.h b/segmentron_amd/csrc/dwconv_slide.h
--- a/segmentron_amd/csrc/dwconv_slide.h
+++ b/segmentron_amd/csrc/dwconv_slide.h
@@ -11,5 +11,7 @@
 int launch_dw_slide_bwd(int dtype, const void* dy, long lddy, const void* x, long ldx, int N, int H,
                         int W, int C, const float* w, int w_layout, int pro_mode, const float* sc,
                         const float* sh, void* g, long ldg, float* partial_w, float* partial_bn,
-                        int rows, hipStream_t st, const void* res = nullptr, long ldr = 0);
+                        int rows, hipStream_t st, const void* res = nullptr, long ldr = 0,
+                        const void* cd = nullptr, long ldd = 0, const float* cc0 = nullptr,
+                        const float* cc1 = nullptr);
 }
diff --git a/segmentron_amd/csrc/dwconv_slide.hip b/segmentron_amd/csrc/dwconv_slide.hip
--- a/segmentron_amd/csrc/dwconv_slide.hip
+++ b/segmentron_amd/csrc/dwconv_slide.hip
@@ -18,7 +18,8 @@
   const float* sc; const float* sh;
   float* partial;
   float* partial_bn;
-  long ldx, lddy, ldy, ldr;
+  const void* cd; const float* cc0; const float* cc1;
+  long ldx, lddy, ldy, ldr, ldd;
   int N, H, W, C, pro_mode, rs, nstrips, nwblk, ncblk;
 };
 
@@ -347,7 +348,7 @@
   }
 }
 
-template <typename T, int MODE, bool RES, bool XCHG>
+template <typename T, int MODE, bool RES, bool XCHG, bool CORR = false>
 __global__ __launch_bounds__(SL_THREADS, 2) void dwconv_slide_bwd_kernel(const DwSlideArgs a) {
   using IO = SlIO<T>;
   using raw_t = typename IO::raw_t;
@@ -357,10 +358,20 @@
   const SlThread t = sl_thread<ES>(a, b, a.lddy);
   const int r0 = t.r0, r1 = t.r1;
 
-  Q4 wt[9], sc, sh;
-  sc = sh = q4_zero();
+  Q4 wt[9], sc, sh, cc0, cc1;
+  sc = sh = cc0 = cc1 = q4_zero();
+  if (CORR) {
+    const float4 u = *reinterpret_cast<const float4*>(a.cc0 + t.c);
+    const float4 v = *reinterpret_cast<const float4*>(a.cc1 + t.c);
+    cc0.lo = (f32x2){u.x, u.y}; cc0.hi = (f32x2){u.z, u.w};
+    cc1.lo = (f32x2){v.x, v.y}; cc1.hi = (f32x2){v.z, v.w};
+  }
+  constexpr int D = SL_DEPTH_B, U = (D % 3 == 0) ? D : 3 * D;
+  raw_t ring[D][3], xring[D], rring[D];
   const long img = (long)b.n * a.H * a.W;
   const unsigned char* __restrict__ Db = reinterpret_cast<const unsigned char*>(a.dy) + img * a.lddy * ES;
+  const unsigned char* __restrict__ Cb =
+      CORR ? reinterpret_cast<const unsigned char*>(a.cd) + img * a.ldd * ES : nullptr;
   const unsigned char* __restrict__ Xb = reinterpret_cast<const unsigned char*>(a.x) + img * a.ldx * ES;
   const unsigned char* __restrict__ Rb =
       RES ? reinterpret_cast<const unsigned char*>(a.res) + img * a.ldr * ES : nullptr;
@@ -371,8 +382,8 @@
   const unsigned xoff = (unsigned)((t.w * a.ldx + t.c) * ES), roff = (unsigned)((t.w * a.ldr + t.c) * ES);
   const unsigned goff = t.live ? (unsigned)((t.w * a.ldy + t.c) * ES) : 0xFFFFFFFFu;
 
-  auto issue = [&](int r, raw_t (&raw)[3]) {
-    const unsigned char* __restrict__ row = Db + (long)min(max(r, 0), t.rlast) * dpitch;
+  auto issue_from = [&](const unsigned char* __restrict__ base, int r, raw_t (&raw)[3]) {
+    const unsigned char* __restrict__ row = base + (long)min(max(r, 0), t.rlast) * dpitch;
     if (XCHG) {
       raw[0] = sl_ld<raw_t>(row, t.off_0);
       raw[1] = sl_ld_edge<raw_t>(row, rowbytes, t.off_e);
@@ -382,15 +393,21 @@
       raw[2] = sl_ld<raw_t>(row, t.off_p);
     }
   };
+  raw_t dring[D][3];
+  auto issue = [&](int r, int j) {
+    issue_from(Db, r, ring[j]);
+    if (CORR) issue_from(Cb, r, dring[j]);
+  };
   auto issue_x = [&](int r, raw_t& xr, raw_t& rr) {
     const int rcl = min(r, r1 - 1);
     xr = sl_ld<raw_t>(Xb + (long)rcl * xpitch, xoff);
     if (RES) rr = sl_ld<raw_t>(Rb + (long)rcl * rpitch, roff);
   };
-  auto commit = [&](int r, const raw_t (&raw)[3], Q4 (&row)[3], auto check) {
+  auto commit = [&](int r, int j, Q4 (&row)[3], auto check) {
     constexpr bool CHECK = decltype(check)::value;
+    const raw_t (&raw)[3] = ring[j];
     const bool rv = !CHECK || (r >= 0 && r < a.H);
-    raw_t r3[3];
+    raw_t r3[3], d3[3];
     r3[1] = raw[0];
     if (XCHG) {
       sl_neighbours<raw_t>(t, raw, r3[0], r3[2]);
@@ -398,9 +415,24 @@
       r3[0] = raw[1];
       r3[2] = raw[2];
     }
+    if (CORR) {
+      const raw_t (&draw)[3] = dring[j];
+      d3[1] = draw[0];
+      if (XCHG) {
+        sl_neighbours<raw_t>(t, draw, d3[0], d3[2]);
+      } else {
+        d3[0] = draw[1];
+        d3[2] = draw[2];
+      }
+    }
 #pragma unroll
     for (int k = 0; k < 3; ++k) {
       row[k] = IO::unpack(r3[k]);
+      if (CORR) {
+        const Q4 dv = IO::unpack(d3[k]);
+        row[k].lo = __builtin_elementwise_fma(-cc1.lo, dv.lo, row[k].lo - cc0.lo);
+        row[k].hi = __builtin_elementwise_fma(-cc1.hi, dv.hi, row[k].hi - cc0.hi);
+      }
       if (CHECK && !rv) row[k] = q4_zero();
     }
   };
@@ -438,12 +470,10 @@
     q4_fma(s2, g, xr);
   };
 
-  constexpr int D = SL_DEPTH_B, U = (D % 3 == 0) ? D : 3 * D;
   Q4 win[3][3];
-  raw_t ring[D][3], xring[D], rring[D];
 #pragma unroll
   for (int j = 0; j < D; ++j) {
-    issue(r0 - 1 + j, ring[j]);
+    issue(r0 - 1 + j, j);
     rring[j] = xring[j] = sl_ld<raw_t>(Xb + (long)min(r0 + j, r1 - 1) * xpitch, xoff);
     if (RES) rring[j] = sl_ld<raw_t>(Rb + (long)min(r0 + j, r1 - 1) * rpitch, roff);
   }
@@ -459,16 +489,16 @@
     if (!t.lm) wt[kh * 3 + 2] = q4_zero();
     if (!t.rm) wt[kh * 3] = q4_zero();
   }
-  commit(r0 - 1, ring[0], win[0], std::true_type{});
-  issue(r0 - 1 + D, ring[0]);
-  commit(r0, ring[1 % D], win[1], std::false_type{});
-  issue(r0 + D, ring[1 % D]);
+  commit(r0 - 1, 0, win[0], std::true_type{});
+  issue(r0 - 1 + D, 0);
+  commit(r0, 1 % D, win[1], std::false_type{});
+  issue(r0 + D, 1 % D);
   int ro = r0;
   for (; ro + U < r1; ro += U) {
 #pragma unroll
     for (int k = 0; k < U; ++k) {
-      commit(ro + k + 1, ring[(k + 2) % D], win[(k + 2) % 3], std::false_type{});
-      issue(ro + k + 1 + D, ring[(k + 2) % D]);
+      commit(ro + k + 1, (k + 2) % D, win[(k + 2) % 3], std::false_type{});
+      issue(ro + k + 1 + D, (k + 2) % D);
       const raw_t xraw = xring[k % D], rraw = rring[k % D];
       issue_x(ro + k + D, xring[k % D], rring[k % D]);
       SL_SCHED_BARRIER();
@@ -479,8 +509,8 @@
 #pragma unroll
   for (int k = 0; k < U; ++k) {
     if (ro + k < r1) {
-      commit(ro + k + 1, ring[(k + 2) % D], win[(k + 2) % 3], std::true_type{});
-      issue(ro + k + 1 + D, ring[(k + 2) % D]);
+      commit(ro + k + 1, (k + 2) % D, win[(k + 2) % 3], std::true_type{});
+      issue(ro + k + 1 + D, (k + 2) % D);
       const raw_t xraw = xring[k % D], rraw = rring[k % D];
       issue_x(ro + k + D, xring[k % D], rring[k % D]);
       compute(ro + k, xraw, rraw, win[k % 3], win[(k + 1) % 3], win[(k + 2) % 3]);
@@ -561,14 +591,14 @@
     default: break;
   }
 }
-template <typename T, bool RES>
+template <typename T, bool RES, bool CORR = false>
 static void slide_launch_bwd(const DwSlideArgs& a, dim3 grid, hipStream_t st) {
   const bool xc = slide_exchange(a, (int)sizeof(T));
   switch (a.pro_mode) {
 #define SL_CASE(M)                                                                                       \
   case M:                                                                                                \
-    if (xc) hipLaunchKernelGGL((dwconv_slide_bwd_kernel<T, M, RES, true>), grid, dim3(SL_THREADS), 0, st, a);  \
-    else hipLaunchKernelGGL((dwconv_slide_bwd_kernel<T, M, RES, false>), grid, dim3(SL_THREADS), 0, st, a);    \
+    if (xc) hipLaunchKernelGGL((dwconv_slide_bwd_kernel<T, M, RES, true, CORR>), grid, dim3(SL_THREADS), 0, st, a);  \
+    else hipLaunchKernelGGL((dwconv_slide_bwd_kernel<T, M, RES, false, CORR>), grid, dim3(SL_THREADS), 0, st, a);    \
     break;
     SL_CASE(0) SL_CASE(1) SL_CASE(2) SL_CASE(3) SL_CASE(5) SL_CASE(7)
 #undef SL_CASE
@@ -583,6 +613,7 @@
                         hipStream_t st) {
   DwSlideArgs a;
   a.x = x; a.dy = nullptr; a.res = nullptr; a.y = y; a.w = w; a.w_layout = w_layout;
+  a.cd = nullptr; a.cc0 = a.cc1 = nullptr; a.ldd = 0;
   a.sc = sc; a.sh = sh; a.partial = stat_partial; a.partial_bn = nullptr;
   a.ldx = ldx; a.lddy = 0; a.ldy = ldy; a.ldr = 0;
   a.N = N; a.H = H; a.W = W; a.C = C; a.pro_mode = pro_mode;
@@ -602,9 +633,11 @@
 int launch_dw_slide_bwd(int dtype, const void* dy, long lddy, const void* x, long ldx, int N, int H,
                         int W, int C, const float* w, int w_layout, int pro_mode, const float* sc,
                         const float* sh, void* g, long ldg, float* partial_w, float* partial_bn,
-                        int rows, hipStream_t st, const void* res, long ldr) {
+                        int rows, hipStream_t st, const void* res, long ldr, const void* cd,
+                        long ldd, const float* cc0, const float* cc1) {
   DwSlideArgs a;
   a.x = x; a.dy = dy; a.res = res; a.y = g; a.w = w; a.w_layout = w_layout & 1;
+  a.cd = cd; a.cc0 = cc0; a.cc1 = cc1; a.ldd = ldd;
   a.sc = sc; a.sh = sh; a.partial = partial_w; a.partial_bn = partial_bn;
   a.ldx = ldx; a.lddy = lddy; a.ldy = ldg; a.ldr = ldr;
   a.N = N; a.H = H; a.W = W; a.C = C; a.pro_mode = pro_mode;
@@ -616,8 +649,13 @@
   SEG_REQUIRE(rows == N * a.nstrips * a.nwblk,
               "dwconv bwd (slide): %d partial rows, the launch writes %d (seg_dwconv_grid_y)", rows,
               N * a.nstrips * a.nwblk);
+  SEG_REQUIRE(cd == nullptr || (dtype == DT_BF16 && ldd == lddy && cc0 && cc1),
+              "dwconv bwd (slide): the dy correction needs bf16, ldd == lddy and c0 / c1");
   const dim3 grid((unsigned)((long)a.ncblk * a.nwblk * a.nstrips * N));
-  if (dtype == DT_BF16) {
+  if (cd != nullptr) {
+    if (res) slide_launch_bwd<bf16_t, true, true>(a, grid, st);
+    else slide_launch_bwd<bf16_t, false, true>(a, grid, st);
+  } else if (dtype == DT_BF16) {
     if (res) slide_launch_bwd<bf16_t, true>(a, grid, st);
     else slide_launch_bwd<bf16_t, false>(a, grid, st);
   } else {
diff --git a/segmentron_amd/functional.py b/segmentron_amd/functional.py
--- a/segmentron_amd/functional.py
+++ b/segmentron_amd/functional.py
@@ -63,6 +63,86 @@
     def take(self):
         g, self.g = self.g, None
         return g
+
+
+class CorrLink:
+    __slots__ = ("ok", "corr")
+
+    def __init__(self):
+        self.ok, self.corr = False, None
+
+    def take(self):
+        c, self.corr = self.corr, None
+        return c
+
+
+WGRAD_GROUP = [os.environ.get("SEG_WGRAD_GROUP") == "1"]
+
+
+class WeightGroup:
+
+    def __init__(self, params):
+        self.params = list(params)
+        self.index = {id(p): i for i, p in enumerate(self.params)}
+        self.jobs = {}
+
+    def put(self, i, d, dy, scale):
+        self.jobs[i] = (d, dy, dy._version, scale)
+
+
+_ACTIVE_GROUP = [None]
+
+
+def _zero_grad_like(w):
+    key = ("zero", str(w.device))
+    if key not in _ONES:
+        _ONES[key] = torch.zeros((), dtype=torch.float32, device=w.device)
+    return _ONES[key].expand(w.shape)
+
+
+class _WeightGroupFn(torch.autograd.Function):
+    @staticmethod
+    def forward(ctx, group, *weights):
+        ctx.group = group
+        return tuple(w.view_as(w) for w in weights)
+
+    @staticmethod
+    def backward(ctx, *grads):
+        group = ctx.group
+        jobs, group.jobs = group.jobs, {}
+        out = list(grads)
+        by_shape = {}
+        for i in sorted(jobs):
+            d, dy, ver, scale = jobs[i]
+            if dy._version != ver:
+                raise RuntimeError("grouped weight gradient: a parked dY was modified in place "
+                                   "before the group's backward")
+            w = group.params[i]
+            dW = torch.empty(w.shape, dtype=torch.float32, device=w.device)
+            out[i] = dW
+            by_shape.setdefault((tuple(dy.shape), tuple(d.shape)), []).append((dy, d, scale, dW))
+        for lst in by_shape.values():
+            for k in range(0, len(lst), 64):
+                K.conv_wgrad_grouped(lst[k:k + 64])
+        return (None,) + tuple(out)
+
+
+@contextlib.contextmanager
+def weight_group(params):
+    from . import compute_dtype
+    params = list(params)
+    if not (WGRAD_GROUP[0] and torch.is_grad_enabled() and compute_dtype() == torch.bfloat16
+            and not _NO_FOLD and any(p.requires_grad for p in params)) \
+            or _ACTIVE_GROUP[0] is not None:
+        yield
+        return
+    group = WeightGroup(params)
+    aliases = _WeightGroupFn.apply(group, *params)
+    _ACTIVE_GROUP[0] = (group, {id(p): a for p, a in zip(params, aliases)})
+    try:
+        yield
+    finally:
+        _ACTIVE_GROUP[0] = None
 
 
 def uses_batch_stats(bn):
@@ -383,6 +463,8 @@
         self.partial = None
         self.drop_bias = False
         self.fork = None
+        self.corr = None
+        self.wgroup = None
 
 
 class _ConvFn(torch.autograd.Function):
@@ -483,8 +565,14 @@
         O, C = weight.shape[0], weight.shape[1]
         bn = spec.bn_in
         w2d = weight.detach().view(O, C)
+        grp = spec.wgroup
+        ctx.grouped = grp is not None and bn.training and bn.group is None and spec.stride == 1 \
+            and spec.drop_const and x.dtype == torch.bfloat16 and spec.corr is not None \
+            and spec.corr.ok and O % 8 == 0 and C % 8 == 0 and K.nhwc(x)[4] % 8 == 0
         wp, wpt, bp = K.fold_weights(w2d, bn.scale, bn.shift, x.dtype,
-                                     want_transpose=ctx.needs_input_grad[0])
+                                     want_transpose=ctx.needs_input_grad[0] and not ctx.grouped)
+        if ctx.grouped:
+            wpt = packed_pointwise(grp[1], True, x.dtype)
         spec.mean_offset = bp
         bias = None if spec.drop_const else bp
         y, spec.partial = K.conv_gemm(x, wp, O, 1, 1, spec.stride, 0, 1, None, bias, spec.out,
@@ -503,6 +591,15 @@
         O, C = weight.shape[0], weight.shape[1]
         if K.nhwc(dy)[4] % K.vec_of(dy.dtype) != 0:
             dy = dy.contiguous()
+        if ctx.grouped:
+            g, dsdt = K.conv_dgrad_sums(dy, ctx.wpt, bn.scale, x)
+            dgamma, dbeta, c0, c1 = K.fold_bwd_finalize(dsdt, bn.count, bn.mean, bn.invstd,
+                                                        bn.gamma, bn.scale)
+            group, index = s.wgroup[0]
+            group.put(index, x, dy, bn.scale)
+            s.corr.corr = (x, c0, c1)
+            dx = g if ctx.needs_input_grad[0] else None
+            return dx, dgamma, dbeta, _zero_grad_like(weight), None
         dwp = K.conv_wgrad(x, dy, O, 1, 1, s.stride, 0, 1, None, raw_partial=True)
         db = None
         if not s.drop_const:
@@ -559,6 +656,41 @@
         if K.nhwc(dy)[4] % K.vec_of(dy.dtype) != 0:
             dy = dy.contiguous()
         dx = dgamma = dbeta = None
+        corr = s.corr.take() if s.corr is not None else None
+        if corr is not None and not (ctx.needs_input_grad[0] and s.stride == 1 and s.dil == 1
+                                     and (s.bn_in is None or s.bn_in.group is None)
+                                     and dy.dtype == torch.bfloat16
+                                     and tuple(corr[0].shape) == tuple(dy.shape)
+                                     and K.nhwc(corr[0])[4] == K.nhwc(dy)[4]):
+            d, c0, c1 = corr
+            ones = _ones(C, dy.device)
+            dy = K.bn_bwd_apply(dy, d, (PRO_AFFINE, ones, ones), c0, c1)
+            corr = None
+        if corr is not None:
+            bn = s.bn_in
+            res = None
+            if bn is None and s.fork is not None and s.fork.g is not None:
+                res = s.fork.take()
+                if res.dtype != x.dtype or tuple(res.shape) != tuple(x.shape):
+                    s.fork.g, res = res, None
+            g, pw, pb = K.dwconv_bwd_fused_corr(x, dy, weight.detach(), s.pro, corr[0], corr[1],
+                                                corr[2], want_bn=bn is not None, res=res)
+            if bn is None:
+                dW, dx = K.dw_wgrad_finalize(pw, C), g
+            elif pb.shape[0] <= 1024:
+                dgamma, dbeta, c0, c1, dW = K.dw_bwd_finalize(pb, pw, bn.count, bn.mean,
+                                                              bn.invstd, bn.gamma)
+            else:
+                dW = K.dw_wgrad_finalize(pw, C)
+                dgamma, dbeta, c0, c1 = K.bn_bwd_finalize_p(pb, bn.count, bn.mean, bn.invstd,
+                                                            bn.gamma)
+            if bn is not None:
+                if not bn.training:
+                    c0 = c1 = None
+                dx = K.bn_bwd_apply(g, x, (PRO_AFFINE, bn.scale, bn.shift), c0, c1, out=g)
+            if s.fork is not None and s.fork.g is not None:
+                dx = dx + s.fork.take()
+            return dx, dgamma, dbeta, dW, None
         tiled = K.dw_tiled(s.stride, s.dil)
         big = x.numel() * x.element_size() >= (40 << 20)
         strided = s.stride == 2 and s.dil == 1 and C % 4 == 0 and weight.dtype == torch.float32
@@ -1134,7 +1266,7 @@
     return Act(_GroupNormFn.apply(y, gn.weight, gn.bias, gn.num_groups, gn.eps, out))
 
 
-def conv_bn(act, conv, bn=None, out=None, fork=None):
+def conv_bn(act, conv, bn=None, out=None, fork=None, corr=None):
     x = act.t
     gn = bn if is_group_norm(bn) else None
     if gn is not None:
@@ -1153,7 +1285,13 @@
         g, b = act.params
     if foldable:
         spec.drop_const = batch_stats
-        y = _FoldConvFn.apply(x, g, b, conv.weight, spec)
+        weight = conv.weight
+        grp = _ACTIVE_GROUP[0]
+        if grp is not None and id(weight) in grp[0].index and corr is not None:
+            spec.corr = corr
+            spec.wgroup = ((grp[0], grp[0].index[id(weight)]), weight)
+            weight = grp[1][id(weight)]
+        y = _FoldConvFn.apply(x, g, b, weight, spec)
         offset = spec.mean_offset if batch_stats else None
     else:
         spec.drop_bias = batch_stats and conv.bias is not None
@@ -1168,12 +1306,15 @@
     return Act(y, finish_bn(bn, spec.partial, N * Ho * Wo, offset, y=y))
 
 
-def dwconv_bn(act, conv, bn, out=None, fork=None):
+def dwconv_bn(act, conv, bn, out=None, fork=None, corr=None):
     gn = bn if is_group_norm(bn) else None
     spec = ConvSpec(act, conv.stride[0], conv.padding[0], conv.dilation[0],
                     None if gn is not None else out,
                     want_stats=gn is None and uses_batch_stats(bn))
     spec.fork = fork
+    if corr is not None:
+        spec.corr = corr
+        corr.ok = gn is None and spec.stride == 1 and spec.dil == 1 and conv.in_channels % 4 == 0
     assert conv.padding[0] == conv.dilation[0] and conv.kernel_size[0] == 3
     g, b = act.params
     y = _DwFn.apply(act.t, g, b, conv.weight, spec)
diff --git a/segmentron_amd/hip_ops.py b/segmentron_amd/hip_ops.py
--- a/segmentron_amd/hip_ops.py
+++ b/segmentron_amd/hip_ops.py
@@ -290,6 +290,24 @@
     return g, colsum(pw, f64=False).view(9, C), pb
 
 
+def dwconv_bwd_fused_corr(x, dy, w, pro, d, c0, c1, want_bn=False, res=None):
+    N, H, W, C, ldx = nhwc(x)
+    lddy = nhwc(dy)[4]
+    ldd = nhwc(d)[4]
+    assert tuple(d.shape) == tuple(dy.shape) == (N, H, W, C) and w.dim() == 4
+    mode, ps, pt = _pro(pro)
+    g = torch.empty((N, H, W, C), dtype=x.dtype, device=x.device)
+    gy = LIB.query("seg_dwconv_grid_y", _DT[x.dtype], C, N, H, W, 1, 1, 1)
+    pw = torch.empty((gy, 9 * C), dtype=torch.float32, device=x.device)
+    pb = torch.empty((gy, 2 * C), dtype=torch.float32, device=x.device) if want_bn else None
+    if res is not None:
+        assert tuple(res.shape) == (N, H, W, C) and res.dtype == x.dtype
+    LIB.call("seg_dwconv3x3_bwd_fused_corr", _DT[x.dtype], _p(dy), lddy, _p(x), ldx, N, H, W, C,
+             _p(w), 1, mode, _p(ps), _p(pt), _p(res), nhwc(res)[4] if res is not None else 0,
+             _p(d), ldd, _p(c0), _p(c1), _p(g), C, _p(pw), _p(pb), gy, _stream())
+    return g, pw, pb
+
+
 def dwconv_bwd_fused_s2(x, dy, w, pro=None, want_bn=False, raw_dw=False):
     N, H, W, C, ldx = nhwc(x)
     Nd, Ho, Wo, Cd, lddy = nhwc(dy)
@@ -570,6 +588,34 @@
     return dW, dsdt
 
 
+def conv_dgrad_sums(dy, wt, scale, x, want_dt=False):
+    N, H, W, O, lddy = nhwc(dy)
+    C = wt.shape[0]
+    ldx = nhwc(x)[4]
+    assert tuple(x.shape) == (N, H, W, C) and wt.shape == (C, O) and wt.dtype == dy.dtype
+    M = N * H * W
+    g = torch.empty((N, H, W, C), dtype=dy.dtype, device=dy.device)
+    R = LIB.query("seg_conv_gemm_dgrad_sums_rows", M, C)
+    dsdt = torch.empty((R, 2 * C), dtype=torch.float32, device=dy.device)
+    LIB.call("seg_conv_gemm_dgrad_sums", _p(dy), lddy, M, O, _p(wt), C, _p(scale), _p(x), ldx,
+             _p(g), C, _p(dsdt), R, int(bool(want_dt)), _stream())
+    return g, dsdt
+
+
+def conv_wgrad_grouped(jobs):
+    import numpy as np
+    dy0, x0 = jobs[0][0], jobs[0][1]
+    N, H, W, O, _ = nhwc(dy0)
+    C = x0.shape[-1]
+    table = np.empty((len(jobs), 6), dtype=np.int64)
+    for i, (dy, x, scale, dW) in enumerate(jobs):
+        assert tuple(dy.shape) == (N, H, W, O) and tuple(x.shape) == (N, H, W, C)
+        assert dW.is_contiguous() and dW.numel() == O * C and dW.dtype == torch.float32
+        table[i] = (dy.data_ptr(), x.data_ptr(), scale.data_ptr(), dW.data_ptr(), nhwc(dy)[4],
+                    nhwc(x)[4])
+    LIB.call("seg_conv_wgrad_grouped", table.ctypes.data, len(jobs), N * H * W, O, C, _stream())
+
+
 def fold_bwd_finalize(dsdt, count, mean, invstd, gamma, scale, grad_scale=1.0):
     C = mean.numel()
     out = torch.empty((4, C), dtype=torch.float32, device=mean.device)
diff --git a/segmentron_amd/models/backbones/xception.py b/segmentron_amd/models/backbones/xception.py
--- a/segmentron_amd/models/backbones/xception.py
+++ b/segmentron_amd/models/backbones/xception.py
@@ -101,8 +101,11 @@
         a = self.block1(a)
         a, c1 = self.block2(a)
         a, c2 = self.block3(a)
-        for i in range(4, 20):
-            a = getattr(self, "block%d" % i)(a)
+        mid = [getattr(self, "block%d" % i) for i in range(4, 20)]
+        with F.weight_group(getattr(blk, "sep_conv%d" % j).block.pointwise.weight
+                            for blk in mid for j in (1, 2, 3)):
+            for blk in mid:
+                a = blk(a)
         c3 = a
         a = self.block20(c3)
         c4 = self.block21(a)
diff --git a/segmentron_amd/modules/basic.py b/segmentron_amd/modules/basic.py
--- a/segmentron_amd/modules/basic.py
+++ b/segmentron_amd/modules/basic.py
@@ -32,8 +32,9 @@
     def forward(self, act, fork=None):
         b = self.block
         if self.relu_first:
-            d = F.dwconv_bn(act.with_relu(), b.depthwise, b.bn_depth, fork=fork)
-            return F.conv_bn(d, b.pointwise, b.bn_point)
+            link = F.CorrLink()
+            d = F.dwconv_bn(act.with_relu(), b.depthwise, b.bn_depth, fork=fork, corr=link)
+            return F.conv_bn(d, b.pointwise, b.bn_point, corr=link)
         assert fork is None
         d = F.dwconv_bn(act, b.depthwise, b.bn_depth)
         d.relu = True
```
